# BlueFisher/Advanced-Soft-Actor-Critic

Measured on AMD Instinct MI355X. Metric: SAC train steps/sec (PER sample + grad step), batch 256, higher is better.
Workload: dtype f32; 1 GPU; cfg2: TEST vector obs(6) c_action(2) stock MLP, PER capacity 524288, n_step=4 V-trace; per_gpu_batch=256, global_batch=256, rows_resident=262144, replay_capacity=524288, n_step=4, burn_in_step=0, parallelism=single, ranks=1, hipgraph=True

## Files before the change

advanced-soft-actor-critic_amd/algorithm/fused.py:

```python
import numpy as np
import contextlib

import torch

from asac_amd import native

__all__ = ['FlatParamGroup', 'FlatAdam', 'squash_sample', 'squash_sample_ls', 'clipped_q_loss', 'DeviceNoise',
           'RecordedNoise']


class FlatParamGroup:

    def __init__(self, named_params: list[tuple[str, list[torch.nn.Parameter]]], device, with_grad=True):
        self.segments: dict[str, tuple[int, int]] = {}
        self.params: dict[str, list[torch.nn.Parameter]] = {}
        total = 0
        for name, ps in named_params:
            start = total
            for p in ps:
                total += p.numel()
            total = (total + 3) // 4 * 4
            self.segments[name] = (start, total)
            self.params[name] = list(ps)
        self.numel = total
# ... 305 lines not shown
        F.mse_loss = orig


def scaled_mse(pred: torch.Tensor, target: torch.Tensor, divisor: float) -> torch.Tensor:
    from asac_amd import native
    if (pred.is_cuda and pred.dim() == 3 and pred.dtype == torch.float32 and pred.is_contiguous() and target.shape == pred.shape
            and target.dtype == torch.float32 and target.stride(-1) == 1 and not target.requires_grad
            and 0 < pred.numel() <= native.MASKED_MSE_MAX):
        return _ScaledMseFn.apply(pred, target, divisor)
    return torch.nn.functional.mse_loss(pred, target) / divisor


class DeviceNoise:

    def __init__(self, seed: int | None = None):
        self.seed = torch.initial_seed() if seed is None else seed
        self._prefilled = []

    def _covered(self, buf: torch.Tensor) -> bool:
        return any(lo <= buf.data_ptr() < hi for lo, hi in self._prefilled)

    def begin_step(self, step_counter: torch.Tensor, u: torch.Tensor | None, flat: torch.Tensor | None,
                   subsets: torch.Tensor | None = None, ensemble: int = 0, polyak=None, zero=None) -> None:
        if subsets is not None and subsets.shape[1] == ensemble:
            subsets = None
        if polyak is not None or zero is not None:
            native.step_prologue(polyak, zero, self.seed, step_counter, u, flat, subsets, ensemble)
        else:
            native.noise_fill(self.seed, step_counter, u, flat, subsets, ensemble)
        self._prefilled = [(t.data_ptr(), t.data_ptr() + t.numel() * t.element_size())
                           for t in (u, flat, subsets) if t is not None]

    def begin_step_with_sample(self, step_counter, rb, flat, subsets=None, ensemble: int = 0, polyak=None,
                               zero=None, defer_weights: bool = False) -> int:
        if (rb.uniform_source is not self or rb.sharded is not None
                or rb.batch_size > native.PROLOGUE_SAMPLE_MAX_BATCH):
            return 0
        if subsets is not None and subsets.shape[1] == ensemble:
            subsets = None
        if defer_weights and rb.min_ratio_reducer is None and rb.batch_size > 256 and rb._gather_keys is not None:
            native.step_prologue_sample_partial(polyak, zero, self.seed, step_counter, rb._u, flat, subsets, ensemble, rb._tree,
                                                rb.capacity, rb.batch_size, rb._slot_ids, rb._leaf, rb._p, rb._ids, rb._min_p)
            self._prefilled = [(t.data_ptr(), t.data_ptr() + t.numel() * t.element_size())
                               for t in (rb._u, flat, subsets) if t is not None]
            return 3
        native.step_prologue_sample(polyak, zero, self.seed, step_counter, rb._u, flat, subsets, ensemble, rb._tree,
                                    rb.capacity, rb.batch_size, rb._slot_ids, rb._beta, rb.beta_increment_per_sampling,
                                    rb._leaf, rb._p, rb._ids, rb._w if rb.min_ratio_reducer is None else None,
                                    rb._min_p)
        self._prefilled = [(t.data_ptr(), t.data_ptr() + t.numel() * t.element_size())
                           for t in (rb._u, flat, subsets) if t is not None]
        return 1

    def uniform_(self, buf: torch.Tensor) -> None:
        if not self._covered(buf):
            buf.uniform_()

    def prefill(self, flat: torch.Tensor) -> None:
        if not self._covered(flat):
            flat.normal_()
            self._prefilled.append((flat.data_ptr(), flat.data_ptr() + flat.numel() * flat.element_size()))

    def normal_(self, buf: torch.Tensor) -> None:
        if not self._covered(buf):
            buf.normal_()

    def subset_(self, buf: torch.Tensor, ensemble: int) -> None:
        k = buf.numel()
        if k == ensemble or self._covered(buf):
            return
        keys = torch.rand(ensemble, device=buf.device)
        buf.copy_(torch.topk(keys, k).indices.to(torch.int32))

# ... 40 lines not shown
```

advanced-soft-actor-critic_amd/algorithm/replay_buffer.py:

```python
import logging
import math
from pathlib import Path

import numpy as np
import torch

from asac_amd import native

_NP_DTYPES = {torch.float32: np.dtype(np.float32), torch.float64: np.dtype(np.float64), torch.float16: np.dtype(np.float16),
              torch.int64: np.dtype(np.int64), torch.int32: np.dtype(np.int32), torch.int16: np.dtype(np.int16),
              torch.int8: np.dtype(np.int8), torch.uint8: np.dtype(np.uint8), torch.bool: np.dtype(np.bool_)}

__all__ = ['PrioritizedReplayBuffer']


def _f32_bits(x: float) -> int:
    return int(np.float32(x).view(np.uint32))


class _DeviceUniform:

    def fill(self, u: torch.Tensor) -> None:
        u.uniform_()

# ... 35 lines not shown

        C, dev = self.capacity, self.device
        with torch.cuda.device(dev):
            self._tree = torch.zeros(2 * C - 1, dtype=torch.float32, device=dev)
            self._slot_ids = torch.zeros(C, dtype=torch.int64, device=dev)
            self._winner = torch.full((C + 2 * max(4096, batch_size),), -1, dtype=torch.int32, device=dev)
            self._winner_rows = torch.full((C,), -1, dtype=torch.int32, device=dev)
            self._winner_rows_side = None
            self._nan_flag = torch.zeros(1, dtype=torch.int32, device=dev)
            self._beta = torch.tensor([beta], dtype=torch.float64, device=dev)
            self._max_p = torch.zeros(1, dtype=torch.float32, device=dev)
            self._min_p = torch.zeros(528, dtype=torch.float32, device=dev)
            B = batch_size
            self._u = torch.zeros(B, dtype=torch.float64, device=dev)
            self._leaf = torch.zeros(B, dtype=torch.int32, device=dev)
            self._p = torch.zeros(B, dtype=torch.float32, device=dev)
            self._ids = torch.zeros(B, dtype=torch.int64, device=dev)
            self._w = torch.ones(B, dtype=torch.float32, device=dev)
        self._init_beta = beta

        self._columns: dict[str, torch.Tensor] | None = None
        self._batch: dict[str, torch.Tensor] | None = None
        self._gather_keys = None
        self._join_action_width, self.joint_pre_action, self.derived = None, None, None
        self._size = 0
        self._next_id = 0

        self._pad_action: torch.Tensor | None = None
        self.uniform_source = _DeviceUniform()
        self.min_ratio_reducer = None
        self.sharded = None
        self.lookahead, self.next_valid, self.parity, self._alt = False, False, 0, None
        self._gather_sidecar = None
        self._closed = False

    def set_window_padding(self, padding_action: torch.Tensor) -> None:
        self._pad_action = padding_action.to(self.device, torch.float32).contiguous()
        self._gather_keys = None

    @property
    def beta(self) -> float:
        return float(self._beta.item())

    def _to_device(self, v) -> torch.Tensor:
        if isinstance(v, torch.Tensor):
            return v.to(self.device, non_blocking=True)
        return torch.from_numpy(np.ascontiguousarray(v)).to(self.device, non_blocking=True)

    def _store_rows(self, transitions: dict) -> tuple[int, int]:
        if (self.packed_ingress and len(transitions) <= native.MAX_GATHER_KEYS
                and all(isinstance(v, np.ndarray) for v in transitions.values())):
            return self._store_rows_packed(transitions)
        rows = {k: self._to_device(v) for k, v in transitions.items()}
        count = next(iter(rows.values())).shape[0]
        C = self.capacity
        if self._columns is None:
            self._columns = {k: torch.zeros((C, *v.shape[1:]), dtype=v.dtype, device=self.device)
                             for k, v in rows.items()}
            self._batch, self._gather_keys = None, None
        first_id = self._next_id
        skip = max(0, count - C)
        start = (first_id + skip) % C
        n1 = min(count - skip, C - start)
        for k, v in rows.items():
            col = self._columns[k]
            col[start:start + n1].copy_(v[skip:skip + n1], non_blocking=True)
# ... 173 lines not shown
    def _build_batch(self) -> None:
        self._batch, specs = self._window_specs(self.batch_size, joined=True)
        self._gather_keys = native.make_gather_keys(specs)
        self._gather_refs = specs
        if self.lookahead:
            self._build_second_set()

    _SET_ATTRS = ('_u', '_leaf', '_p', '_ids', '_w', '_min_p', '_batch', '_gather_keys', '_gather_refs',
                  'joint_pre_action', 'derived', '_gather_sidecar')

    def enable_lookahead(self) -> None:
        assert self.sharded is None and self.min_ratio_reducer is None, 'one batch in flight: single-shard replay only'
        self.lookahead, self.next_valid, self.parity = True, False, 0
        self._alt = None
        if self._gather_keys is not None:
            self._build_second_set()

    def _build_second_set(self) -> None:
        first = {a: getattr(self, a) for a in self._SET_ATTRS}
        with torch.cuda.device(self.device):
            for a in ('_u', '_leaf', '_p', '_ids', '_w', '_min_p'):
                setattr(self, a, first[a].clone())
            self._batch, specs = self._window_specs(self.batch_size, joined=True)
            self._gather_keys = native.make_gather_keys(specs)
            self._gather_refs = specs
            self._gather_sidecar = self._make_gather_sidecar()
        self._alt = {a: getattr(self, a) for a in self._SET_ATTRS}
        for a, v in first.items():
            setattr(self, a, v)
        with torch.cuda.device(self.device):
            self._gather_sidecar = self._make_gather_sidecar()
        self.next_valid = False

    def _make_gather_sidecar(self):
        return native.sidecar_window_gather(self._gather_keys, self._ids, self.batch_size, self.prev_n, self.post_n,
                                            self.capacity, self._index_ring())

    def next_gather_sidecar(self):
        self.next_valid = True
        return self._alt['_gather_sidecar']

    def gather_next_now(self) -> None:
        self.swap_sets()
        try:
            self.sample_into_static(sampled=True)
        finally:
            self.swap_sets()

    def swap_sets(self) -> None:
        for a in self._SET_ATTRS:
            mine = getattr(self, a)
            setattr(self, a, self._alt[a])
            self._alt[a] = mine
        self.parity ^= 1

    def next_uniforms(self) -> torch.Tensor:
        return self._alt['_u']

    def sample_next_into_static(self, sampled: bool = False) -> None:
        self.swap_sets()
        try:
            self.sample_into_static(sampled=sampled)
        finally:
            self.swap_sets()
        self.next_valid = True

    def _index_ring(self):
        index_ring = self._columns.get('index') if self._pad_action is not None else None
        if self._pad_action is not None and index_ring is None:
            raise KeyError("window padding needs an 'index' column")
        return self._leaf if index_ring is None else index_ring

    def gather_windows(self, ids: torch.Tensor) -> dict:
        ids = ids.reshape(-1).to(self.device, torch.int64).contiguous()
        out, specs = self._window_specs(ids.numel())
        if ids.numel():
            with torch.cuda.device(self.device):
                native.window_gather_pad(native.make_gather_keys(specs), ids, ids.numel(), self.prev_n, self.post_n,
                                         self.capacity, self._index_ring())
        return out

    def sample(self):
        if not self.is_lg_batch_size:
            return None
        if self._gather_keys is None:
            self._build_batch()
        self.sample_into_static()
        return self._ids, self._batch, self._w.unsqueeze(-1)

    def sample_into_static(self, sampled: int = 0) -> None:
        B, C = self.batch_size, self.capacity
        if self.sharded is not None:
            self.sharded.sample_into(self)
            return
        reducer = self.min_ratio_reducer
        if not sampled:
            self.uniform_source.fill(self._u)
            native.sumtree_sample(self._tree, C, B, self._u, self._slot_ids, self._beta,
                                  self.beta_increment_per_sampling, self._leaf, self._p, self._ids,
                                  self._w if reducer is None else None, self._min_p)
        if reducer is not None:
            if not sampled:
                torch.div(self._min_p[0:1], self._tree[0:1], out=self._min_p[1:2])
            reducer(self._min_p[1:2])
            native.per_is_weights(self._p, B, self._tree, self._min_p[1:2], self._beta,
                                  self.beta_increment_per_sampling, self._w)
        if sampled == 3:
            native.window_gather_pad_w(self._gather_keys, self._ids, B, self.prev_n, self.post_n, C, self._index_ring(),
                                       self._p, self._tree, self._beta, self.beta_increment_per_sampling, self._w, self._min_p)
        elif sampled != 2:
            native.window_gather_pad(self._gather_keys, self._ids, B, self.prev_n, self.post_n, C, self._index_ring())

    def _update_ids(self, ids: torch.Tensor, td: torch.Tensor, stale_check=True, mode=0, sidecars=None) -> None:
        k = ids.numel()
        if k == 0:
            return
        piece = (self._winner.numel() - self.capacity) // 2
        for s in range(0, k, piece):
            native.sumtree_update(self._tree, self.capacity, ids[s:s + piece], self._slot_ids if stale_check else None,
                                  td[s:s + piece], self.alpha, self.td_error_min, self.td_error_max, mode,
                                  self._winner, self._nan_flag, sidecars=sidecars if s == 0 else None)

    def update(self, data_ids, td_error, sidecars=None) -> None:
# ... 163 lines not shown
```

advanced-soft-actor-critic_amd/algorithm/sac_base.py:

```python
import contextlib
import logging
import random
from collections import defaultdict, namedtuple
from pathlib import Path

import numpy as np
import torch
from torch import distributions, nn
from torch.nn import functional

from asac_amd import native

from . import fused_gru, fused_linear
from .fused import DeviceNoise, FlatAdam, FlatParamGroup, squash_sample, squash_sample_ls, time_slice
from .fused_mlp import DeferredPartialSums, StockMLP, describe_policy, describe_q, direct_param_grads
from .nn_models import *
from .nn_models.layers.seq_layers import step_mask_cache
from .nn_models.representation import ModelSimpleRep
from .batch_buffer import BatchBuffer
from .captured_step import CapturedStep
from .replay_buffer import PrioritizedReplayBuffer
from .sac_aux import AuxHeadsMixin
from .utils import *
from .utils.enums import CURIOSITY, SEQ_ENCODER, SIAMESE
# ... 182 lines not shown

        hip_config = dict(hip_config or {})
        self._use_graph = bool(hip_config.get('use_graph', True))
        self._graph_warmup = int(hip_config.get('graph_warmup', 3))
        self._direct_graph_launch = bool(hip_config.get('direct_graph_launch', True))
        self._dist = hip_config.get('dist')
        self._use_fused_mlp = bool(hip_config.get('fused_mlp', True))
        self._graph_collectives = bool(hip_config.get('graph_collectives', True))
        self._twin_rep = bool(hip_config.get('twin_rep', True))
        self._fuse_linear_tanh = bool(hip_config.get('fused_linear_tanh', True))
        self._use_sidecars = bool(hip_config.get('sidecars', True))
        self._defer_is_weights = bool(hip_config.get('defer_is_weights', True))
        self._fused_policy_step = bool(hip_config.get('fused_policy_step', True))
        self._fused_forward_chain = bool(hip_config.get('fused_forward_chain', True))
        self._fused_td_chain = bool(hip_config.get('fused_td_chain', True))
        self._fused_td_update = bool(hip_config.get('fused_td_update', True))
        self._fused_q_return = bool(hip_config.get('fused_q_return', True))
        self._fused_q_state_grads = bool(hip_config.get('fused_q_state_grads', True))
        self._gru_backward_at = bool(hip_config.get('gru_backward_at', True))
        self._adjacent_cat = bool(hip_config.get('adjacent_cat', True))
        self._fold_rep_q_adam = bool(hip_config.get('fold_rep_q_adam', True))
        self._rep_grad_one_position = bool(hip_config.get('rep_grad_one_position', True))
        self._deferred_cat = bool(hip_config.get('deferred_cat', True))
        self._rep_from_burn_in = bool(hip_config.get('rep_from_burn_in', True))
        self._fused_curiosity = bool(hip_config.get('fused_curiosity', True))
        self._fused_discrete = bool(hip_config.get('fused_discrete', True))
        self._fused_rpm_loss = bool(hip_config.get('fused_rpm_loss', True))
        self._rpm_single_backward = bool(hip_config.get('rpm_single_backward', True))
        self._fused_gating = bool(hip_config.get('fused_gating', True))
        self._rpm_conv_one_launch = bool(hip_config.get('rpm_conv_one_launch', True))
        self._lookahead = int(hip_config.get('lookahead', 0))
        assert self._lookahead in (0, 1), 'hip_config lookahead: 0 (synchronous sampling) or 1 (one batch in flight)'
        self._la_gather_sidecar = bool(hip_config.get('lookahead_gather_sidecar', True)) and self._use_sidecars
        self._la_gather = None
        self._fuse_prediction_dense = bool(hip_config.get('fuse_prediction_dense', True))
        self._fused_q_loss_with_aux = bool(hip_config.get('fused_q_loss_with_aux', True))
        self._head_sums_members = bool(hip_config.get('head_sums_members', True))
        self._rep_epilogue, self._rep_epilogue_hp = False, None
        self._cat_mode = None
        self._g_state_base = None
        self._dist_sampling = hip_config.get('dist_sampling', 'throughput')
        self._dist_ready = False
        assert self._dist_sampling in ('throughput', 'parity')

        self._set_logger()

        if not use_replay_buffer:
            if self._dist is not None:
                raise ValueError('use_replay_buffer=False (the episode batch queue) is single-GPU: a data-parallel '
                                 "context (hip_config['dist']) is not supported with it")
            if self._lookahead:
                self._logger.info("hip_config['lookahead'] does not apply without a replay buffer: forced to 0")
                self._lookahead = 0

        if self.use_n_step_is and c_action_size == 0 and len(d_action_sizes) != 0 and discrete_dqn_like:
            self.use_n_step_is = False

        if device is None:
            if not torch.cuda.is_available():
                raise native.AsacNativeError('SAC_Base needs an MI355X (cuda/ROCm device); there is no CPU path')
            self.device = torch.device(f'cuda:{random.randint(0, torch.cuda.device_count() - 1)}')
        else:
            self.device = torch.device(device)
        if self.device.type != 'cuda':
            raise native.AsacNativeError(f'SAC_Base needs a cuda/ROCm device, got {self.device}; no CPU fallback')
        if self.device.index is None:
# ... 854 lines not shown
        else:
            self._launch_return(ret)
            g0 = self._fq.backward_qloss(x0, a0, t_q, c_y.reshape(-1), w, self.clip_epsilon, self._loss_q_e,
                                         defer=fold, state_grads=state_grads)
        if fold:
            self._fq.adam_partials(self.optimizer_q_list[0], loss_out=self._loss_q_e)
        return g0

    @torch.no_grad()
    def _train_rep_q_stock(self, n_last_masks, n_padding_masks, nx_obses_list, nx_states, nx_actions, n_rewards,
                           n_dones, n_mu_probs, priority_is, policy_sample):
        E, B = self.ensemble_q_num, nx_states.shape[0]
        x0 = StockMLP._rows(nx_states[:, 0], self.state_size)
        a0 = StockMLP._rows(nx_actions[:, 0], self.c_action_size)
        xs = StockMLP._rows(nx_states, self.state_size)
        job_tq, _ = self._ftq.job(x0, a0, out=self._tq_buf)
        job_pi, ls = self._fpi.job(xs, None)
        T, A = nx_states.shape[1], self.c_action_size
        window = (n_last_masks, n_padding_masks, nx_obses_list, nx_states, nx_actions, n_rewards, n_dones,
                  n_mu_probs if self.use_n_step_is else None)
        fused = None
        if self._fused_forward_chain and self.curiosity is None:
            f32 = dict(dtype=torch.float32, device=self.device)
            a_y, logp_y = torch.empty((B, T, A), **f32), torch.empty((B, T), **f32)
            c_pi = torch.empty((B, T, A), **f32) if self.use_n_step_is else None
            job_q, q_tab = self._ftq.job(xs, a_y.view(-1, A))
            fused = native.pi_q_job(job_pi, job_q, self._eps_y, a_y, logp_y, T,
                                    action=nx_actions if self.use_n_step_is else None,
                                    action_offset=self.d_action_summed_size, prob_out=c_pi,
                                    eps2=self._eps_pi if policy_sample else None, t2=0,
                                    a2_out=self._pi_a, logp2_out=self._pi_logp)
            if not native.policy_sample_q_forward_ok(fused):
                fused = None
        if fused is not None:
            self.noise.normal_(self._eps_y)
            if policy_sample:
                self.noise.normal_(self._eps_pi)
                self._pi_sampled = True
            native.policy_sample_q_forward(fused, [job_tq], sidecars=self._take_la_gather())
            _, c_y, ret = self._get_y(*window, eps_buf=self._eps_y, subset_prefix='y', y_out=self._y_buf,
                                      ls=ls[0].view(B, T, 2 * A), sample=(a_y, logp_y), stored_pi=c_pi,
                                      q_table=q_tab.view(E, B, T), launch=False)
        else:
            c_y, ret = self._stock_q_targets(job_tq, job_pi, ls, window, policy_sample)
        opt = self.optimizer_q_list[0]
        fold = self._dist is None and opt.start == self._fq._start and self._params.span('rep')[0] == self._params.span('rep')[1]
        self._stock_q_backward(x0, a0, ret, c_y, priority_is, fold, fused_return=fused is not None and self._fused_q_return)
        if not fold:
            self._finish_rep_q(None, None)

    def _train_rep_q(self, n_last_masks, n_padding_masks, nx_obses_list, nx_states, nx_actions, n_rewards,
                     n_dones, n_mu_probs, priority_is, aux=None, policy_sample=False, state_base=None):
        if (self._stock_c_only() and aux is None and self.clip_epsilon > 0 and not nx_states.requires_grad
                and self.optimizer_rep is None):
            return self._train_rep_q_stock(n_last_masks, n_padding_masks, nx_obses_list, nx_states, nx_actions,
                                           n_rewards, n_dones, n_mu_probs, priority_is, policy_sample)
        dsum = self.d_action_summed_size
        obs_list = [o[:, 0] for o in nx_obses_list]
        state, action = nx_states[:, 0], nx_actions[:, 0]
        if state_base is not None and not nx_states.requires_grad:
            state = state_base[0][:, state_base[1]]
        d_action, c_action = action[..., :dsum], action[..., dsum:]

        if (self._fused_q_state_grads and self._fq is not None and self._ftq is not None and not self.d_action_sizes
                and self.c_action_size and self.clip_epsilon > 0 and aux is None and state_base is not None
                and state_base[0].dim() == 3 and state.requires_grad):
            base, t = state_base
            with torch.no_grad():
                x0 = StockMLP._rows(base.detach()[:, t], self.state_size)
                a0 = StockMLP._rows(c_action, self.c_action_size)
                states_y = nx_states.detach()
                job_tq, _ = self._ftq.job(x0, a0, out=self._tq_buf)
                job_pi, ls_y = self._fpi.job(StockMLP._rows_in_place(states_y, self.state_size), None)
                c_y, ret = self._stock_q_targets(
                    job_tq, job_pi, ls_y, (n_last_masks, n_padding_masks, nx_obses_list, states_y, nx_actions, n_rewards,
                                           n_dones, n_mu_probs if self.use_n_step_is else None), policy_sample)
                fold = self._dist is None and self._fold_rep_q_adam and self._rep_q_adam_alike()
                g0 = self._stock_q_backward(x0, a0, ret, c_y, priority_is, fold, fused_return=self._fused_q_return,
                                            state_grads=True)
                g_base = self._g_state_base
                if g_base is None or g_base.shape != base.shape:
                    g_base = self._g_state_base = torch.zeros_like(base)
                at_position = self._gru_backward_at and fused_gru.is_fused_top(base)
                from_head = not at_position and self._head_sums_members and fused_linear.is_fused_head_output(base)
                if not (at_position or from_head):
                    torch.sum(g0, dim=0, out=g_base[:, t])
            rep_stepped = False
            with direct_param_grads(), DeferredPartialSums() as sums_later:
                if at_position:
# ... 411 lines not shown
            return
        if isinstance(ep_indexes, torch.Tensor):
            assert ep_indexes.dtype == torch.int32
            last = ep_indexes == -1
            last[:, -1] = True
            obs_dev = [o[0] for o in ep_obses_list]
        else:
            assert ep_indexes.dtype == np.int32
            last = np.zeros_like(ep_indexes, dtype=bool)
            last[:, -1] = True
            last[ep_indexes == -1] = True
            obs_dev = None
        if not self.use_replay_buffer:
            self.batch_buffer.put_episode(ep_indexes, last, ep_obses_list, ep_actions, ep_rewards, ep_dones, ep_probs,
                                          ep_pre_seq_hidden_states)
            return
        rows = {'index': ep_indexes[0], 'last_mask': last[0],
                **{f'obs_{name}': o[0] for name, o in zip(self.obs_names, ep_obses_list)},
                'action': ep_actions[0], 'reward': ep_rewards[0], 'done': ep_dones[0],
                'mu_prob': ep_probs[0], 'pre_seq_hidden_state': ep_pre_seq_hidden_states[0]}
        if self.use_normalization:
            self._update_normalizer(obs_dev if obs_dev is not None
                                    else [torch.from_numpy(o[0]).to(self.device) for o in ep_obses_list])
        self.replay_buffer.add(rows, ignore_size=1)

    def _device_step(self) -> None:
        with step_mask_cache() if self.seq_encoder == SEQ_ENCODER.ATTN else contextlib.nullcontext():
            self._device_step_body()

    def _device_step_body(self) -> None:
        self._counter_advanced = False
        w = self._step_sample()
        self._step_rep_and_q(w)
        self._step_policy(w)
        post = _AfterPolicy()
        if not self.use_replay_buffer:
            self._step_temperature_and_aux(w, post)
            if not self._counter_advanced:
                self._opt_steps.add_(1)
            self.batch_buffer.advance_head()
            return
        self._join_lookahead()
        if w.stock and self.use_n_step_is:
            with torch.no_grad():
                if not self._step_after_policy_one_launch(w, post):
                    self._step_after_policy_chain(w, post)
        self._step_temperature_and_aux(w, post)
        self._step_write_backs(w, post)
        if not self._counter_advanced:
            self._opt_steps.add_(1)

    def _join_lookahead(self) -> None:
        if self._la_gather is not None:
            self._la_gather = None
            self.replay_buffer.gather_next_now()

    def _take_la_gather(self):
        sc, self._la_gather = self._la_gather, None
        return None if sc is None else [sc]

    def _step_sample(self):
        rb, b = getattr(self, 'replay_buffer', None), self.burn_in_step
        polyak = None
        if self.update_target_per_step == 1 and self._polyak_len > 0:
            polyak = (self._target_params.flat[:self._polyak_len], self._params.flat[:self._polyak_len], self.tau)
        zero = None if self._grads_overwrite else self._params.grad
        if not self.use_replay_buffer:
            self.noise.begin_step(self._opt_steps, None, self._eps_all, self._subsets_all, self.ensemble_q_num,
                                  polyak=polyak, zero=zero)
            self.batch_buffer.gather_into_static()
            return self._window_views(self.batch_buffer._batch, None, None, None)
        if self._lookahead:
            sampled = False
            if self._use_sidecars:
                rb.swap_sets()
                try:
                    sampled = self.noise.begin_step_with_sample(self._opt_steps, rb, self._eps_all, self._subsets_all,
                                                                self.ensemble_q_num, polyak=polyak, zero=zero)
                finally:
                    rb.swap_sets()
            if not sampled:
                self.noise.begin_step(self._opt_steps, rb.next_uniforms() if rb.uniform_source is self.noise else None,
                                      self._eps_all, self._subsets_all, self.ensemble_q_num, polyak=polyak, zero=zero)
            if sampled and self._la_gather_sidecar:
                self._la_gather = rb.next_gather_sidecar()
            else:
                rb.sample_next_into_static(sampled=sampled)
        else:
            sampled = self._use_sidecars and self.noise.begin_step_with_sample(
                self._opt_steps, rb, self._eps_all, self._subsets_all, self.ensemble_q_num, polyak=polyak, zero=zero,
                defer_weights=self._defer_is_weights)
            if not sampled:
                self.noise.begin_step(self._opt_steps, rb._u if rb.uniform_source is self.noise else None, self._eps_all,
                                      self._subsets_all, self.ensemble_q_num, polyak=polyak, zero=zero)
            rb.sample_into_static(sampled=sampled)
        derived = rb.derived if rb.derived is not None and rb.sharded is None else None
        return self._window_views(rb._batch, rb._ids, rb._w.unsqueeze(-1) if self.use_priority else None, derived,
                                  rb.joint_pre_action)

    def _window_views(self, batch, ids, priority_is, derived, joint_pre_action=None):
        b = self.burn_in_step
        w = _Window()
        w.ids = ids
        w.priority_is = priority_is
        w.bnx_obses_list = [batch[f'obs_{name}'] for name in self.obs_names]
        w.bnx_actions, w.bnx_pad = batch['action'], batch['padding_mask']
        w.bn_indexes, w.bn_last, w.bn_pad = batch['index'][:, :-1], batch['last_mask'][:, :-1], w.bnx_pad[:, :-1]
        w.bn_actions, w.bn_rewards, w.bn_dones = w.bnx_actions[:, :-1], batch['reward'][:, :-1], batch['done'][:, :-1]
        w.bn_mu_probs = batch['mu_prob'][:, :-1]
        w.bnx_hidden = batch['pre_seq_hidden_state']
        w.nx_obs = [o[:, b:] for o in w.bnx_obses_list]
        w.obs_b = [o[:, b] for o in w.bnx_obses_list]
        w.stock = self._stock_c_only()
        w.rep_trainable = self.optimizer_rep is not None
        self.noise.prefill(self._eps_all)
        if type(self.model_rep) is ModelSimpleRep:
            w.rep_in = (None, None, w.bnx_obses_list, None, w.bnx_hidden)
        else:
            if derived is not None:
                d = derived
                bnx_indexes, bnx_padding_masks, bnx_pre_actions = d['index_x'], d['padding_mask_x'], d['pre_action']
            else:
                bnx_indexes, bnx_padding_masks, bnx_pre_actions = self.get_bnx_data(
                    w.bn_indexes, w.bn_pad, w.bn_actions, pre_action_out=joint_pre_action)
            w.rep_in = (bnx_indexes, bnx_padding_masks, w.bnx_obses_list, bnx_pre_actions, w.bnx_hidden)
        return w

    def _step_rep_and_q(self, w) -> None:
# ... 269 lines not shown
    def _optimizer_hp(self) -> tuple:
        opts = self._all_optimizers
        if opts is None:
            opts = self._all_optimizers = [o for o in vars(self).values() if isinstance(o, FlatAdam)] + \
                [o for o in self.optimizer_q_list if o is not None]
        return tuple((o.lr, o.betas, o.eps) for o in opts)

    def _drop_graphs(self) -> None:
        self._graph, self._la_graphs, self._graph_runs = None, {}, {}

    def _drop_graphs_if_hp_changed(self) -> None:
        hp = self._optimizer_hp()
        if hp != self._graph_hp:
            if self._graph_hp is not None and (self._graph is not None or self._la_graphs or self._graph_runs):
                self._logger.info('optimizer hyper-parameters changed: the captured step is dropped and captured again')
                self._drop_graphs()
            self._graph_hp = hp

    @unified_elapsed_timer('train a step', 10)
    def train(self) -> int:
        step = self.get_global_step()
        rb = getattr(self, 'replay_buffer', None)
        if not self._ready_to_train():
            self._profiler('train a step').ignore()
            return step
        self._drop_graphs_if_hp_changed()
        if rb is None:
            if self.batch_buffer._batch is None:
                self.batch_buffer.build_static()
                self._drop_graphs()
        elif rb._gather_keys is None:
            rb._build_batch()
            self._drop_graphs()

        if self._lookahead:
            if not rb.lookahead:
                rb.enable_lookahead()
            if not rb.next_valid:
                with torch.cuda.device(self.device):
                    rb.sample_next_into_static()
            rb.swap_sets()
            self._graph = self._la_graphs.get(rb.parity)
            rb.next_valid = False

        with self._profiler('train', repeat=10):
            if self.update_target_per_step != 1 and step % self.update_target_per_step == 0:
                self._update_target_variables(tau=self.tau)
            graph_ok = (self._use_graph and not self._graph_failed and isinstance(self.noise, DeviceNoise)
                        and (self._dist is None or self._graph_collectives))
            if graph_ok and self._graph is None and self._eager_steps >= self._graph_warmup:
                self._try_capture()
            if graph_ok and self._graph is not None:
                self._replay_graph()
            else:
                self._device_step()
                self._eager_steps += 1
        if rb is None:
            self.batch_buffer.pop_host()
        if self._lookahead:
            self._la_graphs[rb.parity] = self._graph
            rb.next_valid = True

        if step % self.write_summary_per_step == 0:
            if rb is not None:
                rb.check_health()
            if self.summary_writer is not None:
# ... 89 lines not shown
```

advanced-soft-actor-critic_amd/csrc/asac_gather.h:

```cpp
#pragma once
#include "asac_common.h"

namespace asac {

constexpr int kGatherBlock = 256;
#ifndef ASAC_GATHER_UNROLL
#define ASAC_GATHER_UNROLL 2
#endif
constexpr int kUnrollLarge = ASAC_GATHER_UNROLL;
constexpr int64_t kSmallGatherBlocks = 8192;

struct GatherKeyDev {
    const uint8_t* src;
    uint8_t* dst;
    const uint8_t* pad_row;
    int32_t row_bytes;
    int32_t pad_mode;
    uint32_t pad_word;
    int32_t convert;
    int32_t unit_log2;
    int32_t units_per_row;
    uint32_t first_block;
    int32_t dst_pitch;
    int32_t derive;
};

struct GatherArgs {
    int32_t n_keys;
    const int64_t* ids;
    const int32_t* index_ring;
    int32_t batch, prev_n, L, capacity;
};
template <int NK>
struct GatherLaunch {
    GatherKeyDev key[NK];
    GatherArgs c;
};

__device__ __forceinline__ int64_t load_id(const int64_t* ids, int s) { return ids[s]; }

__device__ __forceinline__ bool row_valid(const GatherArgs& a, int64_t id, int j) {
    if (j == a.prev_n) return true;
    const int idx_j = a.index_ring[ring_slot(id + (j - a.prev_n), a.capacity)];
    const int idx_c = a.index_ring[ring_slot(id, a.capacity)];
    return (idx_j - idx_c) == (j - a.prev_n);
}

template <typename Unit>
__device__ __forceinline__ Unit pad_value(const GatherKeyDev& k, int w);

template <>
__device__ __forceinline__ uint4 pad_value<uint4>(const GatherKeyDev& k, int w) {
    if (k.pad_mode == ASAC_PAD_ROW) return reinterpret_cast<const uint4*>(k.pad_row)[w];
    uint32_t x = k.pad_word;
    if (k.pad_mode == ASAC_PAD_BYTE) x = (x & 0xff) * 0x01010101u;
    return make_uint4(x, x, x, x);
}
template <>
__device__ __forceinline__ uint32_t pad_value<uint32_t>(const GatherKeyDev& k, int w) {
    if (k.pad_mode == ASAC_PAD_ROW) return reinterpret_cast<const uint32_t*>(k.pad_row)[w];
    uint32_t x = k.pad_word;
    if (k.pad_mode == ASAC_PAD_BYTE) x = (x & 0xff) * 0x01010101u;
    return x;
}
template <>
__device__ __forceinline__ uint8_t pad_value<uint8_t>(const GatherKeyDev& k, int w) {
    if (k.pad_mode == ASAC_PAD_ROW) return k.pad_row[w];
    if (k.pad_mode == ASAC_PAD_WORD) return (uint8_t)(k.pad_word >> (8 * (w & 3)));
    return (uint8_t)(k.pad_word & 0xff);
}

__device__ __forceinline__ int derived_row(int derive, int j, int L) {
    if (derive == ASAC_DERIVE_PREVIOUS) return j > 0 ? j - 1 : 0;
    if (derive >= ASAC_DERIVE_HOLD_LAST) return min(j, L - 2);
    return j;
}
template <typename Unit> __device__ __forceinline__ Unit zero_unit() { return Unit(0); }
template <> __device__ __forceinline__ uint4 zero_unit<uint4>() { return make_uint4(0, 0, 0, 0); }
template <typename Unit> __device__ __forceinline__ Unit next_index(Unit v) { return v; }
template <> __device__ __forceinline__ uint32_t next_index<uint32_t>(uint32_t v) { return v + (v != 0xffffffffu ? 1u : 0u); }

template <typename Unit, int kUnroll>
__device__ __forceinline__ void copy_units(const GatherArgs& a, const GatherKeyDev& k, int64_t g0,
                                           int64_t total_units) {
    int64_t g[kUnroll], at[kUnroll];
    Unit val[kUnroll];
    bool live[kUnroll];
#pragma unroll
    for (int r = 0; r < kUnroll; ++r) {
        g[r] = g0 + (int64_t)r * kGatherBlock;
        live[r] = g[r] < total_units;
        if (!live[r]) continue;
        const int64_t row = g[r] / k.units_per_row;
        const int w = (int)(g[r] - row * k.units_per_row);
        at[r] = row * k.dst_pitch + (int64_t)w * (int)sizeof(Unit);
        const int sample = (int)(row / a.L);
        const int j = (int)(row - (int64_t)sample * a.L);
        const int64_t id = load_id(a.ids, sample);
        const int js = derived_row(k.derive, j, a.L);
        const int slot = ring_slot(id + (js - a.prev_n), a.capacity);
        const Unit data = reinterpret_cast<const Unit*>(k.src + (int64_t)slot * k.row_bytes)[w];
        const bool valid = (k.pad_mode == ASAC_PAD_KEEP) || row_valid(a, id, js);
// ... 83 lines not shown
```

advanced-soft-actor-critic_amd/csrc/asac_sidecar.h:

```cpp
#pragma once
#include "asac_common.h"
#include "asac_gather.h"

#include <cmath>

namespace asac {

struct AdamScalars {
    float w1, b2, one_m_b2, eps;
    double lr, b1, b2d;
};

inline AdamScalars adam_scalars(float lr, float beta1, float beta2, float eps) {
    AdamScalars c;
    c.w1 = (float)(1.0 - (double)beta1);
    c.b2 = beta2;
    c.one_m_b2 = (float)(1.0 - (double)beta2);
    c.eps = eps;
    c.lr = (double)lr;
    c.b1 = (double)beta1;
    c.b2d = (double)beta2;
    return c;
}

// ... 115 lines not shown
    if (a.padding_mask && a.padding_mask[(int64_t)s * a.mask_sample_stride + j]) return false;
    if (a.ids[s] < 0) return false;
    const int64_t tid = a.ids[s] + a.first_off + j;
    const int slot = ring_slot(tid, a.capacity);
    *slot_out = slot;
    return a.slot_ids[slot] == tid;
}

__device__ __forceinline__ void scatter_elect_row(const ScatterArgs& a, int flat) {
    if (flat >= a.batch * a.count) return;
    int slot;
    if (scatter_target(a, flat, &slot)) atomicMax(&a.winner[slot], flat);
}

__device__ __forceinline__ void scatter_write_row(const ScatterArgs& a, int flat, int lane, int lanes) {
    if (flat >= a.batch * a.count) return;
    int slot;
    if (!scatter_target(a, flat, &slot)) return;
    if (__hip_atomic_load(&a.winner[slot], __ATOMIC_RELAXED, __HIP_MEMORY_SCOPE_AGENT) != flat) return;
    const int s = flat / a.count;
    const int j = flat - s * a.count;
    const uint8_t* src = a.rows + (int64_t)s * a.rows_sample_stride + (int64_t)j * a.rows_row_stride;
    uint8_t* dst = a.ring + (int64_t)slot * a.row_bytes;
    if (((a.row_bytes | (int)(reinterpret_cast<uintptr_t>(src) & 3) |
          (int)(reinterpret_cast<uintptr_t>(dst) & 3)) & 3) == 0) {
        for (int w = lane; w < a.row_bytes / 4; w += lanes)
            reinterpret_cast<uint32_t*>(dst)[w] = reinterpret_cast<const uint32_t*>(src)[w];
    } else {
        for (int w = lane; w < a.row_bytes; w += lanes) dst[w] = src[w];
    }
    if (lane == 0) __hip_atomic_store(&a.winner[slot], -1, __ATOMIC_RELAXED, __HIP_MEMORY_SCOPE_AGENT);
}

struct SidecarDev {
    int32_t kind, first_block;
    AlphaAdamArgs alpha;
    ScatterArgs scatter;
    const void* gather;
};
template <int NSC>
struct SidecarsT {
    SidecarDev j[NSC];
    int32_t n, blocks;
};
using SidecarsDev = SidecarsT<ASAC_MAX_SIDECARS>;

template <int NSC>
inline SidecarsT<NSC> sidecars_first(const SidecarsDev& full) {
    SidecarsT<NSC> out{};
    for (int k = 0; k < NSC && k < full.n; ++k) out.j[k] = full.j[k];
    out.n = full.n < NSC ? full.n : NSC;
    out.blocks = full.blocks;
    return out;
}

constexpr int kSidecarRowsPerWg = 256;
inline int scatter_write_rows_per_wg(int row_bytes) { return row_bytes <= 32 ? kSidecarRowsPerWg : 4; }

inline int sidecars_prepare(const asac_sidecar_t* jobs, int n, SidecarsDev& out) {
    out.n = 0;
    out.blocks = 0;
    if (n < 0 || n > ASAC_MAX_SIDECARS || (n > 0 && !jobs)) return 1;
    for (int k = 0; k < n; ++k) {
        const asac_sidecar_t& h = jobs[k];
        SidecarDev& d = out.j[k];
        d.kind = h.kind;
        d.first_block = out.blocks;
        if (h.kind == ASAC_SIDECAR_ALPHA_ADAM) {
            if (h.B <= 0 || h.n <= 0 || h.slot < 0 || h.slot >= h.n || !h.logp || !h.steps_done) return 1;
            d.alpha = AlphaAdamArgs{h.logp, h.B, h.target, h.slot, h.param, h.grad, h.exp_avg, h.exp_avg_sq, h.n,
                                    adam_scalars(h.lr, h.beta1, h.beta2, h.eps), h.steps_done, h.advance_counter};
            out.blocks += 1;
        } else if (h.kind == ASAC_SIDECAR_SCATTER_ELECT || h.kind == ASAC_SIDECAR_SCATTER_WRITE) {
            if (h.row_bytes <= 0 || h.capacity <= 0 || h.batch <= 0 || h.count <= 0 || !h.winner || !h.slot_ids) return 1;
            d.scatter = ScatterArgs{static_cast<uint8_t*>(h.ring), h.row_bytes, h.capacity, h.ids, h.batch, h.first_off,
                                    h.count, h.slot_ids, h.padding_mask, h.mask_sample_stride,
                                    static_cast<const uint8_t*>(h.rows), h.rows_sample_stride_bytes,
                                    h.rows_row_stride_bytes, h.winner};
            const int total = h.batch * h.count;
            const int per = h.kind == ASAC_SIDECAR_SCATTER_ELECT ? kSidecarRowsPerWg : scatter_write_rows_per_wg(h.row_bytes);
            out.blocks += (total + per - 1) / per;
        } else if (h.kind == ASAC_SIDECAR_WINDOW_GATHER) {
            if (!h.gather_plan || h.gather_blocks <= 0) return 1;
            d.gather = h.gather_plan;
            out.blocks += h.gather_blocks;
        } else {
            return 1;
        }
    }
    out.n = n;
    return 0;
}

template <int NSC, bool GATHER = false>
__device__ __forceinline__ void sidecar_run(const SidecarsT<NSC>& sc, int block, float* lds256) {
    int k = 0;
#pragma unroll
    for (int q = 1; q < NSC; ++q)
        if (q < sc.n && block >= sc.j[q].first_block) k = q;
    const SidecarDev& job = sc.j[k];
    const int local = block - job.first_block;
    if (job.kind == ASAC_SIDECAR_ALPHA_ADAM) {
        alpha_adam_block(job.alpha, lds256);
    } else if (GATHER && job.kind == ASAC_SIDECAR_WINDOW_GATHER) {
        if (threadIdx.x < kGatherBlock)
            gather_block<ASAC_MAX_GATHER_KEYS, 1>(*static_cast<const GatherLaunch<ASAC_MAX_GATHER_KEYS>*>(job.gather),
                                                  (unsigned)local);
    } else if (threadIdx.x < 256) {
        if (job.kind == ASAC_SIDECAR_SCATTER_ELECT) {
            scatter_elect_row(job.scatter, local * kSidecarRowsPerWg + (int)threadIdx.x);
        } else if (job.scatter.row_bytes <= 32) {
            scatter_write_row(job.scatter, local * kSidecarRowsPerWg + (int)threadIdx.x, 0, 1);
        } else {
            scatter_write_row(job.scatter, local * 4 + (int)(threadIdx.x >> 6), (int)(threadIdx.x & 63), kWave);
        }
    }
}

}
```

advanced-soft-actor-critic_amd/csrc/gather.hip:

```cpp
#include "asac_common.h"
#include "asac_gather.h"
#include "asac_sidecar.h"

namespace asac {

template <int NK, int kUnroll>
__global__ __launch_bounds__(kGatherBlock) void k_window_gather_pad(const GatherLaunch<NK> m) {
    gather_block<NK, kUnroll>(m, blockIdx.x);
}

struct WeightsJob {
    const float* p;
    const float* tree;
    double* beta_state;
    double beta_increment;
    float* w_out;
    float* min_p_out;
    int32_t batch, parts;
};

__device__ __forceinline__ void weights_job(const WeightsJob& j) {
    float bm = j.min_p_out[2];
    for (int k = 1; k < j.parts; ++k) bm = fminf(bm, j.min_p_out[2 + k]);
    const float root = j.tree[0];
    const double b = fmin(1.0, *j.beta_state + j.beta_increment);
    const float min_ratio = bm / root;
    __syncthreads();
    for (int i = threadIdx.x; i < j.batch; i += kGatherBlock) j.w_out[i] = is_weight(j.p[i], root, min_ratio, b);
    if (threadIdx.x == 0) {
        *j.beta_state = b;
        j.min_p_out[0] = bm;
    }
}

template <int NK, int kUnroll>
__global__ __launch_bounds__(kGatherBlock) void k_window_gather_pad_w(const GatherLaunch<NK> m, unsigned gather_blocks,
                                                                      const WeightsJob j) {
    if (blockIdx.x == 0) {
        weights_job(j);
        return;
    }
    gather_block<NK, kUnroll>(m, blockIdx.x - 1);
}

__global__ __launch_bounds__(256) void k_scatter_elect(const ScatterArgs a) {
    scatter_elect_row(a, blockIdx.x * blockDim.x + threadIdx.x);
}

__global__ __launch_bounds__(256) void k_scatter_write(const ScatterArgs a) {
    scatter_write_row(a, blockIdx.x * (blockDim.x / kWave) + threadIdx.x / kWave, threadIdx.x & (kWave - 1), kWave);
}

__global__ __launch_bounds__(256) void k_window_aux(const int32_t* __restrict__ index, int64_t index_sb,
                                                    const uint8_t* __restrict__ pad, int64_t pad_sb,
                                                    const float* __restrict__ action, int64_t action_sb,
                                                    int64_t action_st, int B, int L, int A,
                                                    int32_t* __restrict__ index_x, uint8_t* __restrict__ pad_x,
                                                    float* __restrict__ pre_action, int64_t pre_action_st) {
    const int i = blockIdx.x * blockDim.x + threadIdx.x;
    if (i >= B * L) return;
    const int b = i / L, t = i - b * L;
    const int ts = t < L - 1 ? t : L - 2;
    const int32_t iv = index[(int64_t)b * index_sb + ts];
    index_x[i] = t < L - 1 ? iv : iv + (iv != -1 ? 1 : 0);
    pad_x[i] = pad[(int64_t)b * pad_sb + ts];
// ... 101 lines not shown
    return finish_launch("asac_window_aux");
}

int asac_window_gather_pad(const asac_gather_key_t* keys_host, int n_keys, const int64_t* ids,
                           int batch, int prev_n, int post_n, int capacity,
                           const int32_t* index_ring, void* stream) {
    GatherLaunch<ASAC_MAX_GATHER_KEYS> m{};
    uint64_t blocks = 0;
    int unroll = 0;
    if (const int rc = gather_fill(keys_host, n_keys, ids, batch, prev_n, post_n, capacity, index_ring, 0, m, &blocks, &unroll))
        return rc;
    if (n_keys <= 8) {
        GatherLaunch<8> m8{};
        for (int q = 0; q < n_keys; ++q) m8.key[q] = m.key[q];
        m8.c = m.c;
        if (unroll == 1)
            ASAC_LAUNCH((k_window_gather_pad<8, 1>), dim3((unsigned)blocks), dim3(kGatherBlock), 0, as_stream(stream), m8);
        else
            ASAC_LAUNCH((k_window_gather_pad<8, kUnrollLarge>), dim3((unsigned)blocks), dim3(kGatherBlock), 0, as_stream(stream), m8);
    } else if (unroll == 1) {
        ASAC_LAUNCH((k_window_gather_pad<ASAC_MAX_GATHER_KEYS, 1>), dim3((unsigned)blocks), dim3(kGatherBlock), 0,
                    as_stream(stream), m);
    } else {
        ASAC_LAUNCH((k_window_gather_pad<ASAC_MAX_GATHER_KEYS, kUnrollLarge>), dim3((unsigned)blocks), dim3(kGatherBlock), 0,
                    as_stream(stream), m);
    }
    return finish_launch("asac_window_gather_pad");
}

int asac_window_gather_pad_w(const asac_gather_key_t* keys_host, int n_keys, const int64_t* ids, int batch, int prev_n,
                             int post_n, int capacity, const int32_t* index_ring, const float* p, const float* tree,
                             double* beta_state, double beta_increment, float* is_weights_out, float* min_p_out,
                             void* stream) {
    if (!p || !tree || !beta_state || !is_weights_out || !min_p_out || batch <= 256 || batch > 1024)
        return bad_arg("asac_window_gather_pad_w");
    GatherLaunch<ASAC_MAX_GATHER_KEYS> m{};
    uint64_t blocks = 0;
    int unroll = 0;
    if (const int rc = gather_fill(keys_host, n_keys, ids, batch, prev_n, post_n, capacity, index_ring, 0, m, &blocks, &unroll))
        return rc;
    const dim3 grid((unsigned)blocks + 1u);
    for (int rep = 0; rep < g_launch_repeat; ++rep) {
        const WeightsJob j{p, tree, beta_state, rep == 0 ? beta_increment : 0.0, is_weights_out, min_p_out, batch,
                           (batch + 255) / 256};
        if (n_keys <= 8) {
            GatherLaunch<8> m8{};
            for (int q = 0; q < n_keys; ++q) m8.key[q] = m.key[q];
            m8.c = m.c;
            if (unroll == 1)
                hipLaunchKernelGGL((k_window_gather_pad_w<8, 1>), grid, dim3(kGatherBlock), 0, as_stream(stream), m8,
                                   (unsigned)blocks, j);
            else
                hipLaunchKernelGGL((k_window_gather_pad_w<8, kUnrollLarge>), grid, dim3(kGatherBlock), 0, as_stream(stream),
                                   m8, (unsigned)blocks, j);
        } else if (unroll == 1) {
            hipLaunchKernelGGL((k_window_gather_pad_w<ASAC_MAX_GATHER_KEYS, 1>), grid, dim3(kGatherBlock), 0,
                               as_stream(stream), m, (unsigned)blocks, j);
        } else {
            hipLaunchKernelGGL((k_window_gather_pad_w<ASAC_MAX_GATHER_KEYS, kUnrollLarge>), grid, dim3(kGatherBlock), 0,
                               as_stream(stream), m, (unsigned)blocks, j);
        }
    }
    return finish_launch("asac_window_gather_pad_w");
}

int64_t asac_window_gather_plan_bytes(void) { return (int64_t)sizeof(GatherLaunch<ASAC_MAX_GATHER_KEYS>); }

int asac_window_gather_plan(const asac_gather_key_t* keys_host, int n_keys, const int64_t* ids, int batch, int prev_n,
                            int post_n, int capacity, const int32_t* index_ring, void* plan_dev, int* blocks_out) {
    if (!plan_dev || !blocks_out) return bad_arg("asac_window_gather_plan");
    GatherLaunch<ASAC_MAX_GATHER_KEYS> m{};
    uint64_t blocks = 0;
    int unroll = 0;
    if (const int rc = gather_fill(keys_host, n_keys, ids, batch, prev_n, post_n, capacity, index_ring, 1, m, &blocks, &unroll))
        return rc;
    const hipError_t e = hipMemcpy(plan_dev, &m, sizeof(m), hipMemcpyHostToDevice);
    if (e != hipSuccess) {
        set_error(e, "asac_window_gather_plan");
        return (int)e;
    }
    *blocks_out = (int)blocks;
    return 0;
}

int asac_gather_rows(const asac_gather_key_t* keys_host, int n_keys, const int64_t* ids, int n_rows, int capacity,
                     void* stream) {
    if (n_keys <= 0 || n_keys > ASAC_MAX_GATHER_KEYS || !keys_host) return bad_arg("asac_gather_rows");
    for (int q = 0; q < n_keys; ++q)
        if (keys_host[q].pad_mode != ASAC_PAD_KEEP || keys_host[q].convert != ASAC_CVT_NONE)
            return bad_arg("asac_gather_rows: key");
    return asac_window_gather_pad(keys_host, n_keys, ids, n_rows, 0, 0, capacity, nullptr, stream);
}

int asac_scatter_rows_if_id_match(void* ring, int row_bytes, int capacity, const int64_t* ids,
                                  int batch, int first_off, int count, const int64_t* slot_ids,
                                  const uint8_t* padding_mask, int mask_sample_stride,
                                  const void* rows, int64_t rows_sample_stride_bytes,
                                  int64_t rows_row_stride_bytes, int32_t* winner, void* stream) {
    if (row_bytes <= 0 || capacity <= 0 || batch <= 0 || count <= 0 || !winner || !slot_ids)
        return bad_arg("asac_scatter_rows_if_id_match");
    ScatterArgs a{static_cast<uint8_t*>(ring), row_bytes, capacity, ids, batch, first_off, count,
                  slot_ids, padding_mask, mask_sample_stride, static_cast<const uint8_t*>(rows),
                  rows_sample_stride_bytes, rows_row_stride_bytes, winner};
    const int total = batch * count;
    hipStream_t s = as_stream(stream);
    ASAC_LAUNCH(k_scatter_elect, dim3((total + 255) / 256), dim3(256), 0, s, a);
    ASAC_LAUNCH(k_scatter_write, dim3((total + 3) / 4), dim3(256), 0, s, a);
    return finish_launch("asac_scatter_rows_if_id_match");
}

}
```

advanced-soft-actor-critic_amd/csrc/mlp.hip:

```cpp
#include "asac_common.h"
#include "asac_gelu.h"
#include "asac_sidecar.h"
#include "asac_squash.h"
#include "asac_vtrace.h"

#include <cmath>

namespace asac {

constexpr int kP = 66;
constexpr int kMaxW = 64;
constexpr int kMaxB = ASAC_MLP_MAX_BLOCKS;
constexpr int kHeadPad = 16;
#ifndef ASAC_PS_WAVES
#define ASAC_PS_WAVES 16
#endif
#ifndef ASAC_PIQ_WAVES
#define ASAC_PIQ_WAVES 8
#endif
constexpr int kPiQThreads = 64 * ASAC_PIQ_WAVES;
template <int TM> constexpr int threads_of() { return TM * 16; }

inline int mlp_tile_rows(int64_t N, int E) { return ((N + 15) / 16) * (int64_t)(E > 0 ? E : 1) <= 256 ? 16 : 32; }

// ... 364 lines not shown
}

using rsrc_t = __amdgpu_buffer_rsrc_t;
constexpr unsigned kOob = 0x80000000u;
__device__ __forceinline__ rsrc_t make_rsrc(const void* p, unsigned bytes = 0x7fffffffu) {
    return __builtin_amdgcn_make_buffer_rsrc(const_cast<void*>(p), 0, (int)bytes, 0x00020000);
}
__device__ __forceinline__ int buf_ld(rsrc_t r, unsigned byte_off) {
    return __builtin_amdgcn_raw_buffer_load_b32(r, (int)byte_off, 0, 0);
}

template <int THREADS, bool WINDOW, int SLOTS = 4>
__device__ __forceinline__ void fetch_input_tile_fixed(const StageScalars& q, int e, int64_t row0, float (&v)[SLOTS]) {
    const int in0 = q.in0, in1 = q.in1;
    const rsrc_t r0 = make_rsrc(q.x0 + e * q.x0_ms);
    const rsrc_t r1 = make_rsrc(q.x1 + e * q.x1_ms, in1 > 0 ? 0x7fffffffu : 0u);
#pragma unroll
    for (int u = 0; u < SLOTS; ++u) {
        const int i = threadIdx.x + u * THREADS;
        const int r = i >> 6, c = i & 63;
        const uint32_t row = (uint32_t)row0 + (uint32_t)r;
        const bool live = (int64_t)row0 + r < q.N;
        uint32_t off = row * (uint32_t)q.x0_rs;
        if (WINDOW) {
            const uint32_t smp = row / (uint32_t)q.x0_T;
            off = smp * (uint32_t)q.x0_sb + (row - smp * (uint32_t)q.x0_T) * (uint32_t)q.x0_rs;
        }
        const unsigned o0 = (live && c < in0) ? (off + (uint32_t)c) * 4u : kOob;
        const unsigned o1 = (live && c >= in0 && c < in0 + in1) ? (row * (uint32_t)q.x1_rs + (uint32_t)(c - in0)) * 4u : kOob;
        v[u] = __builtin_bit_cast(float, buf_ld(r0, o0) | buf_ld(r1, o1));
    }
}

template <int THREADS, int NB>
__device__ __forceinline__ void net_fetch_fixed(const StageScalars& q, StagedNet<THREADS>& r) {
    constexpr int U = 4096 / THREADS;
    const rsrc_t rp = make_rsrc(q.P);
    const int K0 = q.in0 + q.in1;
#pragma unroll
    for (int u = 0; u < U; ++u) {
        const int i = threadIdx.x + u * THREADS;
        const int rr = i >> 6, c = i & 63;
        r.w[0][u] = __builtin_bit_cast(float, buf_ld(rp, c < K0 ? (unsigned)(q.w_off[0] + rr * K0 + c) * 4u : kOob));
    }
#pragma unroll
    for (int l = 1; l < NB; ++l) {
#pragma unroll
        for (int u = 0; u < U / 4; ++u) {
            const auto t = __builtin_amdgcn_raw_buffer_load_b128(rp, (q.w_off[l] + 4 * (int)(threadIdx.x + u * THREADS)) * 4, 0, 0);
#pragma unroll
            for (int k = 0; k < 4; ++k) r.w[l][4 * u + k] = __builtin_bit_cast(float, (int)t[k]);
        }
    }
#pragma unroll
    for (int l = 0; l < NB; ++l) r.bias[l] = __builtin_bit_cast(float, buf_ld(rp, (unsigned)(q.b_off[l] + (threadIdx.x & 63)) * 4u));
    const int h0 = q.h0, h1 = q.h1;
#pragma unroll
    for (int u = 0; u < 1024 / THREADS; ++u) {
        const int i = threadIdx.x + u * THREADS;
        const int o = i >> 6, c = i & 63;
        const bool first = o < h0, second = !first && o < h0 + h1;
        const int idx = second ? q.hw1 + (o - h0) * kMaxW + c : q.hw0 + o * kMaxW + c;
        r.head[u] = __builtin_bit_cast(float, buf_ld(rp, (first || second) ? (unsigned)idx * 4u : kOob));
    }
    {
        const int o = threadIdx.x & 15;
// ... 18 lines not shown
            const int q = threadIdx.x + u * THREADS;
            float2* o2 = reinterpret_cast<float2*>(L.w[l] + (q >> 4) * kP + ((q & 15) << 2));
            o2[0] = make_float2(r.w[l][4 * u], r.w[l][4 * u + 1]);
            o2[1] = make_float2(r.w[l][4 * u + 2], r.w[l][4 * u + 3]);
        }
    }
    if (threadIdx.x < kMaxW) {
#pragma unroll
        for (int l = 0; l < NB; ++l) L.bias[l][threadIdx.x] = r.bias[l];
    }
#pragma unroll
    for (int u = 0; u < 1024 / THREADS; ++u) {
        const int i = threadIdx.x + u * THREADS;
        L.head[(i >> 6) * kP + (i & 63)] = r.head[u];
    }
    if (threadIdx.x < kHeadPad) L.head_bias[threadIdx.x] = r.head_bias;
}

template <int TM>
struct MlpLds {
    float head[kHeadPad * kP];
    float bias[kMaxB][kMaxW];
    float head_bias[kHeadPad];
    float xs[2][TM * kP];
    float w[kMaxB][kMaxW * kP];
};

inline size_t mlp_fwd_lds_bytes(int n_blocks, bool wide = false, int TM = 32) {
    const size_t head = TM == 16 ? offsetof(MlpLds<16>, w) : offsetof(MlpLds<32>, w);
    return head + (size_t)(n_blocks + (wide ? 1 : 0)) * kMaxW * kP * sizeof(float) +
           (wide ? (size_t)TM * kP * sizeof(float) : 0);
}

template <int TM, bool WINDOW, bool WIDE = false, int NB = 0, bool EPI = false>
__device__ __forceinline__ void mlp_fwd_tiles(const MlpFwdArgs& a, const int e, const int tile0, const int tile_stride,
                                              MlpLds<TM>& L, const SampleEpi* epi = nullptr) {
    constexpr int THREADS = threads_of<TM>();
    constexpr int RT = TM / 16;
    constexpr bool fixed = NB > 0;
    static_assert(!(fixed && WIDE), "the fixed-shape path has a first layer of <= 64 inputs");
    const float* P = a.params + e * a.member_stride;
    const int wave = threadIdx.x >> 6, lane = threadIdx.x & 63;
    const int rt = wave % RT, ct = wave / RT;
    const int nb = fixed ? NB : a.d.n_blocks;
    const int K0 = a.d.in0 + a.d.in1;
    const int n_tiles = (int)((a.N + TM - 1) / TM);

    constexpr bool wide = WIDE;
    float* w_hi = &L.w[0][0] + nb * kMaxW * kP;
    float* x_hi = w_hi + kMaxW * kP;
    StageScalars q;
    if constexpr (fixed) {
        q = stage_scalars<NB>(a, e);
        float in_lo[4];
        fetch_input_tile_fixed<THREADS, WINDOW>(q, e, (int64_t)tile0 * TM, in_lo);
        StagedNet<THREADS> regs;
        net_fetch_fixed<THREADS, NB>(q, regs);
        put_input_tile<THREADS>(in_lo, L.xs[0]);
        net_put_fixed<THREADS, NB>(regs, L);
    } else {
        float in_lo[4], in_hi[4];
        fetch_input_tile<THREADS, WINDOW>(a, e, (int64_t)tile0 * TM, in_lo);
        if (wide) fetch_input_tile<THREADS, WINDOW>(a, e, (int64_t)tile0 * TM, in_hi, kMaxW);
        StagedNet<THREADS> regs;
        net_fetch<THREADS>(a.d, P, K0, wide, regs);
        put_input_tile<THREADS>(in_lo, L.xs[0]);
        if (wide) {
            put_input_tile<THREADS>(in_hi, x_hi);
            stage_matrix_part<THREADS>(L.w[0], P + a.d.w_off[0], a.d.width[0], K0, 0, kMaxW);
            stage_matrix_part<THREADS>(w_hi, P + a.d.w_off[0], a.d.width[0], K0, kMaxW, K0 - kMaxW);
        }
        net_put<THREADS>(a.d, P, K0, wide, regs, L);
    }
    const int K_last = fixed ? kMaxW : a.d.width[nb - 1];
    __syncthreads();

    const int O = a.d.head_cols[0] + a.d.head_cols[1];
    int cur = 0;
    for (int tile = tile0; tile < n_tiles; tile += tile_stride) {
        const int64_t row0 = (int64_t)tile * TM;
        const bool more = tile + tile_stride < n_tiles;
        float nxt[4], nxt_hi[4];
        if (more) {
            if constexpr (fixed) fetch_input_tile_fixed<THREADS, WINDOW>(q, e, (int64_t)(tile + tile_stride) * TM, nxt);
            else fetch_input_tile<THREADS, WINDOW>(a, e, (int64_t)(tile + tile_stride) * TM, nxt);
        }
        if (more && wide) fetch_input_tile<THREADS, WINDOW>(a, e, (int64_t)(tile + tile_stride) * TM, nxt_hi, kMaxW);
        SampleEpiIn epi_in{};
        bool epi_on = false;
        if constexpr (EPI) {
            epi_on = epi->on != 0;
            if (epi_on)
                epi_in = sample_epilogue_fetch(*epi, row0 + (wave % RT) * 16 + 4 * (lane >> 4) + wave / RT, a.N, lane & 15);
        }
        int K = K0;
#pragma unroll
        for (int l = 0; l < (fixed ? NB : kMaxB); ++l) {
            if (l >= nb) break;
            const int W = fixed ? kMaxW : a.d.width[l];
            const float* xin = L.xs[cur];
            float* xout = L.xs[cur ^ 1];
            f32x4 acc = (fixed && l > 0) ? gemm_tile(xin, L.w[l], kMaxW, rt, ct)
                                         : gemm_tile(xin, L.w[l], (l == 0 && wide) ? kMaxW : round4(K), rt, ct);
            if (l == 0 && wide) acc += gemm_tile(x_hi, w_hi, round4(K0 - kMaxW), rt, ct);
            const int col = ct * 16 + (lane & 15);
            const float bias = L.bias[l][col];
            const bool res = a.d.residual[l] != 0;
            f32x2_g ya, yb, unused;
            gelu_parts2((f32x2_g){acc[0] + bias, acc[1] + bias}, ya, unused);
            gelu_parts2((f32x2_g){acc[2] + bias, acc[3] + bias}, yb, unused);
            const float yv[4] = {ya.x, ya.y, yb.x, yb.y};
#pragma unroll
            for (int r = 0; r < 4; ++r) {
                const int row = rt * 16 + 4 * (lane >> 4) + r;
                float y = yv[r];
                if (res) y += xin[row * kP + col];
                xout[row * kP + col] = col < W ? y : 0.f;
// ... 948 lines not shown
    q.in0 = j.in0, q.in1 = j.in1, q.x0_T = j.x0_T;
    q.h0 = j.h0, q.h1 = j.h1;
    q.hw0 = j.hw0, q.hw1 = j.hw1, q.hb0 = j.hb0, q.hb1 = j.hb1;
#pragma unroll
    for (int l = 0; l < 3; ++l) q.w_off[l] = j.w_off[l], q.b_off[l] = j.b_off[l];
    ASAC_PIN(q.P); ASAC_PIN(q.x0); ASAC_PIN(q.x1);
    ASAC_PIN(q.N); ASAC_PIN(q.x0_rs); ASAC_PIN(q.x0_ms); ASAC_PIN(q.x1_rs); ASAC_PIN(q.x1_ms); ASAC_PIN(q.x0_sb);
    ASAC_PIN(q.in0); ASAC_PIN(q.in1); ASAC_PIN(q.x0_T); ASAC_PIN(q.h0); ASAC_PIN(q.h1);
    ASAC_PIN(q.hw0); ASAC_PIN(q.hw1); ASAC_PIN(q.hb0); ASAC_PIN(q.hb1);
#pragma unroll
    for (int l = 0; l < 3; ++l) { ASAC_PIN(q.w_off[l]); ASAC_PIN(q.b_off[l]); }
    return q;
}

__device__ __forceinline__ StageScalars stage_scalars_stock_like(const ASAC_KARG StockJobArg& j, int e, const StageScalars& rows) {
    StageScalars q = rows;
    q.P = j.P + e * j.member_stride;
    q.in1 = j.in1;
    q.h0 = j.h0, q.h1 = j.h1;
    q.hw0 = j.hw0, q.hw1 = j.hw1, q.hb0 = j.hb0, q.hb1 = j.hb1;
#pragma unroll
    for (int l = 0; l < 3; ++l) q.w_off[l] = j.w_off[l], q.b_off[l] = j.b_off[l];
    ASAC_PIN(q.P); ASAC_PIN(q.in1); ASAC_PIN(q.h0); ASAC_PIN(q.h1);
    ASAC_PIN(q.hw0); ASAC_PIN(q.hw1); ASAC_PIN(q.hb0); ASAC_PIN(q.hb1);
#pragma unroll
    for (int l = 0; l < 3; ++l) { ASAC_PIN(q.w_off[l]); ASAC_PIN(q.b_off[l]); }
    return q;
}

__device__ __forceinline__ float gauss_head_value(bool location, float raw) {
    return location ? tanhf(raw / 5.f) * 5.f : expf(fminf(fmaxf(raw, -20.f), 0.5f));
}

template <bool WINDOW>
__device__ __forceinline__ void pi_q_tiles(const ASAC_KARG PiQLaunch& a, PiQLds& L) {
    constexpr int THREADS = kPiQThreads;
    constexpr int SLOTS = 1024 / kPiQThreads;
    const bool comp = (threadIdx.x >> 6) < 4;
    const int e = (int)blockIdx.x % a.E, group = (int)blockIdx.x / a.E;
    const int wave = threadIdx.x >> 6, lane = threadIdx.x & 63;
    const int col = wave * 16 + (lane & 15);
    const int A = a.pi.h0, S = a.q.in0;
    const int K0p = a.pi.in0, K0q = a.q.in0 + a.q.in1;
    const int N = a.pi.N;
    const int n_tiles = (int)((N + 15) / 16);
    const bool writer = e == 0;
    MLP_STAMP(0);

    const StageScalars sp = stage_scalars_stock(a.pi, 0);
    const StageScalars sq = stage_scalars_stock_like(a.q, e, sp);
    float in_lo[SLOTS];
    fetch_input_tile_fixed<THREADS, WINDOW, SLOTS>(sp, 0, (int64_t)group * 16, in_lo);
    StagedNet<THREADS> rp, rq;
    net_fetch_fixed<THREADS, 3>(sp, rp);
    net_fetch_fixed<THREADS, 3>(sq, rq);
    put_input_tile<THREADS, SLOTS>(in_lo, L.xs[0]);
    net_put_fixed<THREADS, 3>(rp, L);
    PiQCritic C{L.qw, L.qhead, L.qbias, L.qhead_bias};
    __syncthreads();
    MLP_STAMP(1);

    for (int tile = group; tile < n_tiles; tile += a.tile_groups) {
        const int row0 = tile * 16;
        if (tile != group) {
            fetch_input_tile_fixed<THREADS, WINDOW, SLOTS>(sp, 0, row0, in_lo);
            __syncthreads();
            put_input_tile<THREADS, SLOTS>(in_lo, L.xs[0]);
            __syncthreads();
        }
        int cur = 0;
#pragma unroll
        for (int l = 0; l < 3; ++l) {
            if (comp) {
                const float* xin = L.xs[cur];
                float* xout = L.xs[cur ^ 1];
                const f32x4 acc = l > 0 ? gemm_tile(xin, L.w[l], kMaxW, 0, wave) : gemm_tile(xin, L.w[l], round4(K0p), 0, wave);
                const float bias = L.bias[l][col];
                const bool res = (a.pi.residual_bits >> l) & 1;
                f32x2_g ya, yb, unused;
                gelu_parts2((f32x2_g){acc[0] + bias, acc[1] + bias}, ya, unused);
                gelu_parts2((f32x2_g){acc[2] + bias, acc[3] + bias}, yb, unused);
                const float yv[4] = {ya.x, ya.y, yb.x, yb.y};
#pragma unroll
                for (int r = 0; r < 4; ++r) {
                    const int row = 4 * (lane >> 4) + r;
                    float y = yv[r];
                    if (res) y += xin[row * kP + col];
                    xout[row * kP + col] = y;
                }
            }
            __syncthreads();
            cur ^= 1;
        }
        MLP_STAMP(2);
        if (comp) {
            const f32x4 acc = gemm_tile(L.xs[cur], L.head, kMaxW, 0, 0);
            const int hc = lane & 15;
            const float mine = wave == 0 ? acc[0] : wave == 1 ? acc[1] : wave == 2 ? acc[2] : acc[3];
            const int lrow = 4 * (lane >> 4) + wave;
            const float v = gauss_head_value(hc < A, mine + L.head_bias[hc]);
            L.ls[lrow * 2 * kHeadPad + hc] = v;
            if (writer && a.pi.out && row0 + lrow < N && hc < 2 * A) a.pi.out[(row0 + lrow) * (2 * A) + hc] = v;
        }
        __syncthreads();
        MLP_STAMP(3);
        {
            float* scr = L.xs[1];
            const int job = wave;
            const bool job_on = job == 0 || (writer && ((job == 1 && a.sp.action) || (job == 2 && a.eps2)));
            float* s0 = scr + job * 256;
            float* s1 = s0 + 128;
            if (job < 3 && job_on) {
                for (int it = lane; it < 16 * A; it += 64) {
                    const int lrow = it / A, d = it - lrow * A;
                    const int r = row0 + lrow;
                    if (r >= N) continue;
                    const float l = L.ls[lrow * 2 * kHeadPad + d], sc = L.ls[lrow * 2 * kHeadPad + A + d];
                    if (job == 1) {
                        const int spT = a.sp.T;
                        const int sb = (int)((unsigned)r / (unsigned)spT), st = r - sb * spT;
                        const float av = a.sp.action[sb * a.sp.a_sb + st * a.sp.a_st + a.sp.a_off + d];
                        const float x = atanhf(fminf(fmaxf(av, -0.999f), 0.999f));
                        s0[lrow * 8 + d] = squash_jac(x);
                        s1[lrow * 8 + d] = expf(normal_log_prob(x, l, sc));
                    } else {
                        float ev;
                        const int smp = (int)((unsigned)r / (unsigned)a.T);
                        if (job == 0) {
                            ev = a.eps[r * A + d];
                        } else {
                            if (r - smp * a.T != a.t2) continue;
                            ev = a.eps2[smp * A + d];
                        }
                        const float x = l + ev * sc;
                        const float t = tanhf(x);
                        s0[lrow * 8 + d] = logf(fmaxf(1.f - t * t, kSquashFloor));
                        s1[lrow * 8 + d] = normal_log_prob(x, l, sc);
                        if (job == 0) {
                            L.act[lrow * kHeadPad + d] = t;
                            if (writer) a.a_out[r * A + d] = t;
                        } else {
                            a.a2_out[smp * A + d] = t;
                        }
                    }
                }
                __builtin_amdgcn_fence(__ATOMIC_RELEASE, "wavefront");
                __builtin_amdgcn_wave_barrier();
                __builtin_amdgcn_fence(__ATOMIC_ACQUIRE, "wavefront");
                if (lane < 16) {
                    const int lrow = lane;
                    const int r = row0 + lrow;
                    if (r < N) {
                        if (job == 1) {
                            float jac = 1.f;
// ... 77 lines not shown

template <int NSC>
__global__ __launch_bounds__(kPiQThreads) void k_pi_sample_q(const PiQLaunch m_by_value, const SidecarsT<NSC> sc) {
    extern __shared__ __attribute__((aligned(16))) unsigned char smem_raw[];
    const ASAC_KARG PiQLaunch& m = *static_cast<const ASAC_KARG PiQLaunch*>(kernarg_base());
    const int blk = (int)blockIdx.x;
    const int fused_blocks = m.blocks;
    if (blk >= fused_blocks && threadIdx.x >= 256) return;
    if (blk < fused_blocks) {
        PiQLds& L = *reinterpret_cast<PiQLds*>(smem_raw);
        if (m.pi.x0_T > 0) pi_q_tiles<true>(m, L);
        else pi_q_tiles<false>(m, L);
        return;
    }
    const int xb = blk - fused_blocks;
    if (xb >= m.x_blocks) {
        sidecar_run<NSC, true>(sc, xb - m.x_blocks, reinterpret_cast<float*>(smem_raw));
        return;
    }
    int k = 0;
#pragma unroll
    for (int q = 1; q < ASAC_MLP_MAX_JOBS; ++q)
        if (q < m.x_n && xb >= m.x_first_block[q]) k = q;
    const int local = xb - m.x_first_block[k];
    const int E = m.x_E[k];
    MlpLds<16>& L = *reinterpret_cast<MlpLds<16>*>(smem_raw);
    const MlpFwdArgs job = expand_stock(m.x_job[k]);
    if (job.x0_T > 0)
        mlp_fwd_tiles<16, true, false, 3>(job, local % E, local / E, m.x_tile_stride[k], L);
    else
        mlp_fwd_tiles<16, false, false, 3>(job, local % E, local / E, m.x_tile_stride[k], L);
}

__global__ __launch_bounds__(256) void k_mlp_reduce_partials(const float* __restrict__ partial, int tiles, int E,
                                                             int64_t member_stride, int64_t used,
                                                             float* __restrict__ grad, int accumulate,
                                                             const float* __restrict__ loss_partial,
                                                             float* __restrict__ loss_out, float inv_n) {
    const int64_t i = (int64_t)blockIdx.x * blockDim.x + threadIdx.x;
    const int e = blockIdx.y;
    if (loss_partial && i == 0) {
        float l = 0.f;
        for (int t = 0; t < tiles; ++t) l += loss_partial[(int64_t)t * E + e];
        loss_out[e] = l * inv_n;
    }
    if (i >= used) return;
    float s = 0.f;
    for (int t0 = 0; t0 < tiles; t0 += 8) {
        float v[8];
#pragma unroll
        for (int w = 0; w < 8; ++w) {
            const int t = t0 + w < tiles ? t0 + w : tiles - 1;
            v[w] = partial[((int64_t)t * E + e) * member_stride + i];
        }
#pragma unroll
        for (int w = 0; w < 8; ++w) s += t0 + w < tiles ? v[w] : 0.f;
    }
    grad[e * member_stride + i] = accumulate ? grad[e * member_stride + i] + s : s;
}

constexpr int kReduceSlices = 16;
constexpr int kSlicedFrom = 64;
__global__ __launch_bounds__(64 * kReduceSlices) void k_mlp_reduce_partials_sliced(
    const float* __restrict__ partial, int tiles, int E, int64_t member_stride, int64_t used, float* __restrict__ grad,
    int accumulate, const float* __restrict__ loss_partial, float* __restrict__ loss_out, float inv_n) {
    __shared__ float part[kReduceSlices][64];
// ... 443 lines not shown
    ASAC_LAUNCH(k_policy_step, dim3((unsigned)tiles), dim3(kPsThreads), sizeof(PsLds), s, a);
    if (reduce_mode != ASAC_MLP_REDUCE_DEFER)
        reduce_partials(pi_desc, workspace, tiles, 1, pi_member_stride, pi_grad_params, reduce_mode, nullptr, nullptr, 0.f, s);
    return finish_launch("asac_policy_step_fused");
}

static bool fits32(int64_t v) { return v >= 0 && v < 0x1fffffffLL; }

static StockJobArg stock_job_arg(const asac_mlp_job_t& p) {
    const asac_mlp_desc_t* d = p.desc;
    StockJobArg j{};
    j.P = p.params, j.x0 = p.x0, j.x1 = p.x1, j.out = p.out;
    j.member_stride = (int32_t)p.member_stride, j.N = (int32_t)p.N;
    j.x0_rs = (int32_t)p.x0_row_stride, j.x0_ms = (int32_t)p.x0_member_stride;
    j.x1_rs = (int32_t)p.x1_row_stride, j.x1_ms = (int32_t)p.x1_member_stride;
    j.x0_sb = (int32_t)p.x0_sample_stride, j.x0_T = (int32_t)p.x0_window_T;
    j.in0 = d->in0, j.in1 = d->in1, j.h0 = d->head_cols[0], j.h1 = d->head_cols[1];
    j.hw0 = (int32_t)d->head_w_off[0], j.hw1 = (int32_t)d->head_w_off[1];
    j.hb0 = (int32_t)d->head_b_off[0], j.hb1 = (int32_t)d->head_b_off[1];
    for (int l = 0; l < 3; ++l) {
        j.w_off[l] = (int32_t)d->w_off[l], j.b_off[l] = (int32_t)d->b_off[l];
        j.residual_bits |= (d->residual[l] ? 1 : 0) << l;
    }
    j.head_transform = d->head_transform;
    return j;
}

static asac_mlp_job_t pi_rows(const asac_mlp_job_t& p) {
    asac_mlp_job_t r = p;
    r.x1 = nullptr, r.x1_row_stride = r.x1_member_stride = 0;
    return r;
}

static bool pi_q_job_ok(const asac_pi_q_job_t& j) {
    const asac_mlp_job_t &p = j.pi, &q = j.q;
    if (!p.desc || !q.desc || !desc_ok(*p.desc) || !desc_ok(*q.desc) || p.N <= 0 || q.N != p.N || p.E != 1 || q.E < 1) return false;
    if (!stock3(*p.desc, p.params, p.member_stride) || !stock3(*q.desc, q.params, q.member_stride)) return false;
    if (!scalar_head(*q.desc) || !gauss_head(*p.desc) || p.desc->in1 != 0) return false;
    const int A = p.desc->head_cols[0];
    if (q.desc->in0 != p.desc->in0 || q.desc->in1 != A || 2 * A > kHeadPad || A > 8) return false;
    if (!p.x0 || q.x0 != p.x0 || q.x0_row_stride != p.x0_row_stride || q.x0_window_T != p.x0_window_T ||
        q.x0_sample_stride != p.x0_sample_stride || p.x0_member_stride != 0 || q.x0_member_stride != 0 || !q.out)
        return false;
    const asac_squash_job_t& s = j.sample;
    if (!s.eps || !s.a_tanh_out || !s.logp_out || s.A != A || s.rows != p.N) return false;
    if (s.action && (!s.prob_out || s.T <= 0)) return false;
    if (j.eps2 && (!j.a2_out || !j.logp2_out || s.T <= 0 || j.t2 < 0 || j.t2 >= s.T)) return false;
    if (!fits32(p.member_stride) || !fits32(q.member_stride * q.E)) return false;
    if (s.action && (!fits32((p.N / s.T + 1) * s.action_stride_b) || !fits32((p.N / s.T + 1) * s.prob_stride_b) ||
                     !fits32(s.T * s.action_stride_t) || !fits32(s.T * s.prob_stride_t)))
        return false;
    return job_fits32(pi_rows(p));
}

int asac_policy_sample_q_forward_ok(const asac_pi_q_job_t* job) { return job && pi_q_job_ok(*job) ? 1 : 0; }

int asac_policy_sample_q_forward(const asac_pi_q_job_t* job, const asac_mlp_job_t* extra_jobs, int n_extra,
                                 const asac_sidecar_t* sidecars_host, int n_sidecars, void* stream) {
    if (!job || !pi_q_job_ok(*job) || n_extra < 0 || n_extra > ASAC_MLP_MAX_JOBS || (n_extra > 0 && !extra_jobs))
        return bad_arg("asac_policy_sample_q_forward");
    SidecarsDev sc{};
    if (sidecars_prepare(sidecars_host, n_sidecars, sc)) return bad_arg("asac_policy_sample_q_forward: sidecar");
    PiQLaunch m{};
    const asac_mlp_job_t p = pi_rows(job->pi);
    asac_mlp_job_t q = pi_rows(job->q);
    q.x1 = p.x0;
    m.pi = stock_job_arg(p);
    m.q = stock_job_arg(q);
    m.E = q.E;
    const int tiles = (int)((p.N + 15) / 16);
    const int cap = 256 / q.E > 0 ? 256 / q.E : 1;
    m.tile_groups = tiles <= cap ? tiles : cap;
    m.blocks = m.tile_groups * q.E;
    const asac_squash_job_t& sj = job->sample;
    m.eps = sj.eps;
    m.a_out = sj.a_tanh_out;
    m.logp_out = sj.logp_out;
    m.sp = StoredProbArg{sj.action, sj.prob_out, sj.T, (int32_t)sj.action_stride_b, (int32_t)sj.action_stride_t, sj.action_offset,
                         (int32_t)sj.prob_stride_b, (int32_t)sj.prob_stride_t, sj.prob_offset, 0};
    m.eps2 = job->eps2;
    m.T = sj.T > 0 ? sj.T : 1;
    m.t2 = job->t2;
    m.a2_out = job->a2_out;
    m.logp2_out = job->logp2_out;
    m.x_n = n_extra;
    int blocks = 0;
    for (int k = 0; k < n_extra; ++k) {
        const asac_mlp_job_t& j = extra_jobs[k];
        if (!job_ok(j, true) || !stock3(*j.desc, j.params, j.member_stride) || j.x0_window_T < 0 || !job_fits32(j) ||
            !fits32(j.member_stride) || !fits32(j.x0_member_stride) || !fits32(j.x1_member_stride))
            return bad_arg("asac_policy_sample_q_forward: extra job");
        m.x_job[k] = stock_job_arg(j);
        m.x_E[k] = j.E;
        m.x_first_block[k] = blocks;
        m.x_tile_stride[k] = mlp_tile_groups(j.N, j.E, 1, 16);
        blocks += m.x_tile_stride[k] * j.E;
    }
    m.x_blocks = blocks;
    static bool attr_done = false;
    static bool attr_done1 = false;
    if (int rc = set_lds_limit(reinterpret_cast<const void*>(k_pi_sample_q<ASAC_MAX_SIDECARS>), sizeof(PiQLds), attr_done,
                               "asac_policy_sample_q_forward: hipFuncSetAttribute"))
        return rc;
    if (int rc = set_lds_limit(reinterpret_cast<const void*>(k_pi_sample_q<1>), sizeof(PiQLds), attr_done1,
                               "asac_policy_sample_q_forward: hipFuncSetAttribute"))
        return rc;
    const SidecarsDev none{};
    for (int rep = 0; rep < g_launch_repeat; ++rep) {
        const bool last = rep == g_launch_repeat - 1;
        const dim3 grid((unsigned)(m.blocks + blocks + (last ? sc.blocks : 0)));
        if (sc.n <= 1)
            hipLaunchKernelGGL(k_pi_sample_q<1>, grid, dim3(kPiQThreads), sizeof(PiQLds), as_stream(stream), m,
                               sidecars_first<1>(last ? sc : none));
        else
            hipLaunchKernelGGL(k_pi_sample_q<ASAC_MAX_SIDECARS>, grid, dim3(kPiQThreads), sizeof(PiQLds), as_stream(stream), m,
                               last ? sc : none);
    }
    return finish_launch("asac_policy_sample_q_forward");
}

int asac_mlp_backward_qloss_return_ok(const asac_mlp_job_t* job, const asac_vtrace_args_t* ret) {
    if (!job || !job->desc || !desc_ok(*job->desc) || !ret || job->E <= 0 || job->N <= 0 || ret->B != job->N || ret->n <= 0 ||
        !ret->q || !ret->y_out || ret->E_sample <= 0 || ret->E_sample > ASAC_MAX_ENSEMBLE || ret->td_error_out)
        return 0;
    if (wide_input(*job->desc) || !stock3(*job->desc, job->params, job->member_stride)) return 0;
    const int tm = mlp_tile_rows(job->N, job->E);
    const size_t lds = (tm == 16 ? sizeof(MlpBwdLds<16>) : sizeof(MlpBwdLds<32>)) +
                       (size_t)(2 * ((ret->n + 1) | 1) + 2) * tm * sizeof(float);
    const int threads = tm == 16 ? 64 * ASAC_BWD_WAVES : 32 * 16;
    return tm * ret->n <= threads && lds <= 128 * 1024;
}
// ... 41 lines not shown
```

advanced-soft-actor-critic_amd/csrc/sumtree.hip:

```cpp
#include "asac_common.h"
#include "asac_gather.h"
#include "asac_noise.h"
#include "asac_sidecar.h"
#include "asac_tree_update.h"

#include <cmath>
#include <cstdio>
#include <cstring>
#include <mutex>

namespace asac {

int g_launch_repeat = 1;
static char g_err[256] = "";
static std::mutex g_err_mu;

void set_error(hipError_t e, const char* where) {
    std::lock_guard<std::mutex> lk(g_err_mu);
    snprintf(g_err, sizeof(g_err), "%s: %s", where, hipGetErrorString(e));
}

constexpr int kSampleBlock = 256;
constexpr int kLdsLevels = 12;
constexpr int kLdsNodes = (1 << kLdsLevels) - 1;
// ... 148 lines not shown
            node_[t] = 4 * node_[t] + 3 + 2 * i1 + step(t, i1 ? a2[t].z : a2[t].x, i1 ? a2[t].w : a2[t].y);
        }
    }
    for (; l < levels; ++l) {
        float ab[kTrips][2];
#pragma unroll
        for (int t = 0; t < kTrips; ++t) {
            const int left = live_[t] ? 2 * node_[t] + 1 : 1;
            ab[t][0] = tree[left], ab[t][1] = tree[left + 1];
        }
#pragma unroll
        for (int t = 0; t < kTrips; ++t) node_[t] = 2 * node_[t] + 1 + step(t, ab[t][0], ab[t][1]);
    }
    int64_t id_reg[kTrips];
#pragma unroll
    for (int trip = 0; trip < kTrips; ++trip) {
        const int i = first + trip * kSampleBlock;
        id_reg[trip] = -1;
        if (!live_[trip]) {
            p_reg[trip] = 0.f;
            continue;
        }
        const float p = levels == 0 ? tree[0] : p_reg[trip];
        leaf_out[i] = node_[trip];
        p_out[i] = p;
        id_reg[trip] = slot_ids[node_[trip] - (capacity - 1)];
        pmin = fminf(pmin, p);
        p_reg[trip] = p;
    }

    float m = wave_min(pmin);
    if ((threadIdx.x & (kWave - 1)) == 0) red[threadIdx.x / kWave] = m;
    __syncthreads();
    SampleSync* const sync = MULTI ? reinterpret_cast<SampleSync*>(min_p_out + 2) : nullptr;
    const unsigned n_wg = MULTI ? (unsigned)((batch + kSampleBlock - 1) / kSampleBlock) : 1u;
    if (PARTIAL) {
        if (threadIdx.x == 0) {
            float bm = red[0];
            for (int w = 1; w < kSampleBlock / kWave; ++w) bm = fminf(bm, red[w]);
            sync->part[blockIdx.x] = bm;
        }
#pragma unroll
        for (int trip = 0; trip < kTrips; ++trip) {
            const int i = first + trip * kSampleBlock;
            if (live_[trip]) ids_out[i] = id_reg[trip];
        }
        return;
    }
    if (MULTI) {
        if (threadIdx.x == 0) {
            float bm = red[0];
            for (int w = 1; w < kSampleBlock / kWave; ++w) bm = fminf(bm, red[w]);
            sync_store(&sync->part[blockIdx.x], bm);
            sync_complete();
            __hip_atomic_fetch_add(&sync->arrived, 1u, __ATOMIC_RELAXED, __HIP_MEMORY_SCOPE_AGENT);
            while (__hip_atomic_load(&sync->arrived, __ATOMIC_RELAXED, __HIP_MEMORY_SCOPE_AGENT) < n_wg)
                __builtin_amdgcn_s_sleep(1);
            bm = sync_load(&sync->part[0]);
            for (unsigned w = 1; w < n_wg; ++w) bm = fminf(bm, sync_load(&sync->part[w]));
            red[0] = bm;
        }
    } else if (threadIdx.x == 0) {
        float bm = red[0];
        for (int w = 1; w < kSampleBlock / kWave; ++w) bm = fminf(bm, red[w]);
        red[0] = bm;
        if (FUSE_WEIGHTS && !w_out) {
            min_p_out[0] = bm;
// ... 27 lines not shown
        const double b = fmin(1.0, beta_old + beta_increment);
#pragma unroll
        for (int trip = 0; trip < kTrips; ++trip) {
            const int i = first + trip * kSampleBlock;
            if (i < batch) w_out[i] = is_weight(p_reg[trip], root, min_ratio, b);
        }
    }
#pragma unroll
    for (int trip = 0; trip < kTrips; ++trip) {
        const int i = first + trip * kSampleBlock;
        if (live_[trip]) ids_out[i] = id_reg[trip];
    }
}

template <bool FUSE_WEIGHTS, bool STAGE_TOP>
__global__ __launch_bounds__(kSampleBlock) void k_sumtree_sample(
    const float* __restrict__ tree, int capacity, int levels, int batch,
    const double* __restrict__ u, const int64_t* __restrict__ slot_ids, double* beta_state,
    double beta_increment, int32_t* __restrict__ leaf_out, float* __restrict__ p_out,
    int64_t* __restrict__ ids_out, float* __restrict__ w_out, float* min_p_out) {
    sumtree_sample_body<FUSE_WEIGHTS, STAGE_TOP>(tree, capacity, levels, batch, const_cast<double*>(u), slot_ids, beta_state,
                                                 beta_increment, leaf_out, p_out, ids_out, w_out, min_p_out);
}

template <bool PARTIAL>
__global__ __launch_bounds__(kSampleBlock) void k_prologue_sample(
    const PrologueArgs pa, const float* __restrict__ tree, int capacity, int levels, int batch,
    const int64_t* __restrict__ slot_ids, double* beta_state, double beta_increment, int32_t* __restrict__ leaf_out,
    float* __restrict__ p_out, int64_t* __restrict__ ids_out, float* __restrict__ w_out, float* min_p_out) {
    const int n_s = (batch + kSampleBlock - 1) / kSampleBlock;
    if ((int)blockIdx.x < n_s) {
        const SampleDraw dr{pa.seed, pa.step, pa.n_normal};
        if (n_s == 1)
            sumtree_sample_body<true, true, true, false, 1, false, 13>(
                tree, capacity, levels, batch, pa.u, slot_ids, beta_state, beta_increment, leaf_out, p_out, ids_out, w_out,
                min_p_out, dr);
        else
            sumtree_sample_body<true, true, true, false, 1, true, 13, PARTIAL>(
                tree, capacity, levels, batch, pa.u, slot_ids, beta_state, beta_increment, leaf_out, p_out, ids_out, w_out,
                min_p_out, dr);
    } else {
        prologue_block(pa, (int)blockIdx.x - n_s, true);
    }
}

__global__ __launch_bounds__(kSampleBlock) void k_sumtree_descend(
    const float* __restrict__ tree, int capacity, int levels, int n, const double* __restrict__ v,
    const int64_t* __restrict__ slot_ids, int32_t* __restrict__ leaf_out, float* __restrict__ p_out,
    int64_t* __restrict__ ids_out, float* scratch_min) {
    sumtree_sample_body<false, false, false, true>(tree, capacity, levels, n, const_cast<double*>(v), slot_ids, nullptr, 0.0,
                                                   leaf_out, p_out, ids_out, nullptr, scratch_min);
}

__global__ __launch_bounds__(kSampleBlock) void k_sumtree_descend_owned(
    const float* __restrict__ tree, int capacity, int levels, int n, const double* __restrict__ v,
    const int32_t* __restrict__ owner, int rank, const int64_t* __restrict__ slot_ids, int32_t* __restrict__ leaf_out,
    float* __restrict__ p_out, int64_t* __restrict__ ids_out, float* scratch_min) {
    sumtree_sample_body<false, false, false, true>(tree, capacity, levels, n, const_cast<double*>(v), slot_ids, nullptr, 0.0,
                                                   leaf_out, p_out, ids_out, nullptr, scratch_min, SampleDraw{}, owner, rank);
}

constexpr int kMaxShards = 64;
__global__ __launch_bounds__(kSampleBlock) void k_sumtree_plan_top(const float* __restrict__ roots, int G, int levels_top,
                                                                   int batch, const double* __restrict__ u,
                                                                   int32_t* __restrict__ owner_out, double* __restrict__ v_out,
                                                                   float* __restrict__ total_out) {
    __shared__ float heap[2 * kMaxShards];
// ... 305 lines not shown
    for (int rep = 0; rep < g_launch_repeat; ++rep) {
        const int blocks_p = rep == 0 ? (int)pb : 0;
        const PrologueArgs a{seed, step_counter, uniform_out, batch, normal_out, n_normal, subsets_out, n_subsets, E_sample,
                             E, blocks_p, target, source, n_polyak, one_m_tau, tau, (int)zb, zero_out, n_zero};
        const dim3 grid((unsigned)((batch + kSampleBlock - 1) / kSampleBlock + blocks_p + zb + (lanes + 255) / 256));
        if (partial)
            hipLaunchKernelGGL(k_prologue_sample<true>, grid, dim3(kSampleBlock), 0, as_stream(stream), a, tree, capacity,
                               ilog2(capacity), batch, slot_ids, beta_state, 0.0, leaf_out, p_out, ids_out, is_weights_out,
                               min_p_out);
        else
            hipLaunchKernelGGL(k_prologue_sample<false>, grid, dim3(kSampleBlock), 0, as_stream(stream), a, tree, capacity,
                               ilog2(capacity), batch, slot_ids, beta_state, rep == 0 ? beta_increment : 0.0, leaf_out, p_out,
                               ids_out, is_weights_out, min_p_out);
    }
    return finish_launch("asac_step_prologue_sample");
}

int asac_step_prologue_sample(float* target, const float* source, int64_t n_polyak, float tau, float* zero_out,
                              int64_t n_zero, uint64_t seed, const int64_t* step_counter, double* uniform_out,
                              float* normal_out, int64_t n_normal, int32_t* subsets_out, int n_subsets, int E_sample,
                              int E, const float* tree, int capacity, int batch, const int64_t* slot_ids,
                              double* beta_state, double beta_increment, int32_t* leaf_out, float* p_out,
                              int64_t* ids_out, float* is_weights_out, float* min_p_out, void* stream) {
    return prologue_sample_launch(target, source, n_polyak, tau, zero_out, n_zero, seed, step_counter, uniform_out, normal_out,
                                  n_normal, subsets_out, n_subsets, E_sample, E, tree, capacity, batch, slot_ids, beta_state,
                                  beta_increment, leaf_out, p_out, ids_out, is_weights_out, min_p_out, false, stream);
}

int asac_step_prologue_sample_partial(float* target, const float* source, int64_t n_polyak, float tau, float* zero_out,
                                      int64_t n_zero, uint64_t seed, const int64_t* step_counter, double* uniform_out,
                                      float* normal_out, int64_t n_normal, int32_t* subsets_out, int n_subsets, int E_sample,
                                      int E, const float* tree, int capacity, int batch, const int64_t* slot_ids,
                                      int32_t* leaf_out, float* p_out, int64_t* ids_out, float* min_p_out, void* stream) {
    if (batch <= kSampleBlock) return bad_arg("asac_step_prologue_sample_partial: one workgroup samples such a batch whole");
    static double unused_beta = 0.0;
    return prologue_sample_launch(target, source, n_polyak, tau, zero_out, n_zero, seed, step_counter, uniform_out, normal_out,
                                  n_normal, subsets_out, n_subsets, E_sample, E, tree, capacity, batch, slot_ids, &unused_beta,
                                  0.0, leaf_out, p_out, ids_out, nullptr, min_p_out, true, stream);
}

int asac_per_is_weights(const float* p, int batch, const float* total, const float* min_ratio,
                        double* beta_state, double beta_increment, float* is_weights_out,
                        void* stream) {
    if (batch <= 0) return bad_arg("asac_per_is_weights");
    hipStream_t s = as_stream(stream);
    const int blocks = (batch + 255) / 256;
    if (batch <= kFusedSampleMax && g_launch_repeat == 1) {
        ASAC_LAUNCH(k_is_weights_advance, dim3(1), dim3(256), 0, s, p, batch, total, min_ratio, beta_state, beta_increment,
                    is_weights_out);
        return finish_launch("asac_per_is_weights");
    }
    ASAC_LAUNCH(k_is_weights, dim3(blocks), dim3(256), 0, s, p, batch, total, min_ratio,
                       beta_state, beta_increment, is_weights_out, 1);
    ASAC_LAUNCH(k_advance_beta, dim3(1), dim3(1), 0, s, beta_state, beta_increment);
    return finish_launch("asac_per_is_weights");
}

int asac_sumtree_update(float* tree, int capacity, int k, const int64_t* ids,
                        const int64_t* slot_ids, const float* td_error, float alpha, float td_min,
                        float td_max, int mode, int32_t* winner, int32_t* nan_flag, void* stream) {
    return asac_sumtree_update_sc(tree, capacity, k, ids, slot_ids, td_error, alpha, td_min, td_max, mode, winner, nan_flag,
                                  nullptr, 0, stream);
}

int asac_sumtree_update_sc(float* tree, int capacity, int k, const int64_t* ids,
                           const int64_t* slot_ids, const float* td_error, float alpha, float td_min,
                           float td_max, int mode, int32_t* winner, int32_t* nan_flag,
// ... 59 lines not shown
```

advanced-soft-actor-critic_amd/native.py:

```python
import ctypes as C
from pathlib import Path

import torch

PKG_DIR = Path(__file__).resolve().parent
import os as _os

LIB_PATH = Path(_os.environ.get('ASAC_HIP_LIB', PKG_DIR / 'lib' / 'libasac_hip.so'))
ABI_VERSION = 88

MAX_GATHER_KEYS = 16
PAD_KEEP, PAD_WORD, PAD_BYTE, PAD_ROW, PAD_EMIT_MASK = 0, 1, 2, 3, 4
CVT_NONE, CVT_U8_TO_F32_UNIT, CVT_BOOL_TO_F32 = 0, 1, 2


class AsacNativeError(RuntimeError):
    pass


class GatherKey(C.Structure):
    _fields_ = [('src', C.c_void_p), ('dst', C.c_void_p), ('pad_row', C.c_void_p),
                ('row_bytes', C.c_int32), ('pad_mode', C.c_int32), ('pad_word', C.c_uint32),
                ('convert', C.c_int32), ('dst_row_pitch', C.c_int32), ('derive', C.c_int32)]


class AdamEpilogue(C.Structure):
    _fields_ = [('param_base', C.c_void_p), ('grad_base', C.c_void_p), ('exp_avg_base', C.c_void_p),
                ('exp_avg_sq_base', C.c_void_p), ('lr', C.c_float), ('beta1', C.c_float), ('beta2', C.c_float),
                ('eps', C.c_float), ('steps_done', C.c_void_p)]


def adam_epilogue(param_flat, grad_flat, exp_avg, exp_avg_sq, lr, beta1, beta2, eps, steps_done) -> AdamEpilogue:
    for t in (param_flat, grad_flat, exp_avg, exp_avg_sq):
        assert t.is_cuda and t.is_contiguous() and t.dtype == torch.float32 and t.numel() == param_flat.numel()
    assert steps_done.dtype == torch.int64 and steps_done.is_cuda
    ep = AdamEpilogue(param_flat.data_ptr(), grad_flat.data_ptr(), exp_avg.data_ptr(), exp_avg_sq.data_ptr(),
                      float(lr), float(beta1), float(beta2), float(eps), steps_done.data_ptr())
    ep._keep = (param_flat, grad_flat, exp_avg, exp_avg_sq, steps_done)
    ep._span = (grad_flat.data_ptr(), grad_flat.data_ptr() + 4 * grad_flat.numel())
    return ep


# ... 56 lines not shown
    _fields_ = [('in0', C.c_int32), ('in1', C.c_int32), ('n_blocks', C.c_int32),
                ('width', C.c_int32 * 4), ('residual', C.c_int32 * 4), ('head_cols', C.c_int32 * 2),
                ('w_off', C.c_int64 * 4), ('b_off', C.c_int64 * 4),
                ('head_w_off', C.c_int64 * 2), ('head_b_off', C.c_int64 * 2),
                ('head_transform', C.c_int32), ('reserved_', C.c_int32)]


class MlpJob(C.Structure):
    _fields_ = [('desc', C.POINTER(MlpDesc)), ('params', C.c_void_p), ('member_stride', C.c_int64),
                ('x0', C.c_void_p), ('x0_row_stride', C.c_int64), ('x0_member_stride', C.c_int64),
                ('x1', C.c_void_p), ('x1_row_stride', C.c_int64), ('x1_member_stride', C.c_int64),
                ('N', C.c_int64), ('out', C.c_void_p), ('E', C.c_int32), ('x0_window_T', C.c_int32),
                ('x0_sample_stride', C.c_int64)]


MLP_MAX_JOBS = 2
SAMPLE_EPILOGUE = _os.environ.get('ASAC_SAMPLE_EPILOGUE', '1') != '0'


class Sidecar(C.Structure):
    _fields_ = [('kind', C.c_int32),
                ('logp', C.c_void_p), ('B', C.c_int32), ('target', C.c_float), ('slot', C.c_int32),
                ('param', C.c_void_p), ('grad', C.c_void_p), ('exp_avg', C.c_void_p), ('exp_avg_sq', C.c_void_p),
                ('n', C.c_int32), ('lr', C.c_float), ('beta1', C.c_float), ('beta2', C.c_float), ('eps', C.c_float),
                ('steps_done', C.c_void_p), ('advance_counter', C.c_int32),
                ('ring', C.c_void_p), ('row_bytes', C.c_int32), ('capacity', C.c_int32), ('ids', C.c_void_p),
                ('batch', C.c_int32), ('first_off', C.c_int32), ('count', C.c_int32), ('slot_ids', C.c_void_p),
                ('padding_mask', C.c_void_p), ('mask_sample_stride', C.c_int32), ('rows', C.c_void_p),
                ('rows_sample_stride_bytes', C.c_int64), ('rows_row_stride_bytes', C.c_int64), ('winner', C.c_void_p),
                ('gather_plan', C.c_void_p), ('gather_blocks', C.c_int32)]


SIDECAR_ALPHA_ADAM, SIDECAR_SCATTER_ELECT, SIDECAR_SCATTER_WRITE, SIDECAR_WINDOW_GATHER, MAX_SIDECARS = 1, 2, 3, 4, 4


class SquashJob(C.Structure):
    _fields_ = [('loc', C.c_void_p), ('scale', C.c_void_p), ('ls_row_stride', C.c_int64), ('eps', C.c_void_p),
                ('rows', C.c_int64), ('A', C.c_int32), ('T', C.c_int32), ('a_tanh_out', C.c_void_p),
                ('logp_out', C.c_void_p), ('x_out', C.c_void_p), ('action', C.c_void_p),
                ('action_stride_b', C.c_int64), ('action_stride_t', C.c_int64), ('prob_out', C.c_void_p),
                ('prob_stride_b', C.c_int64), ('prob_stride_t', C.c_int64), ('action_offset', C.c_int32),
                ('prob_offset', C.c_int32)]


SQUASH_MAX_JOBS = 4


class PiQJob(C.Structure):
    _fields_ = [('pi', MlpJob), ('sample', SquashJob), ('eps2', C.c_void_p), ('t2', C.c_int32), ('reserved_', C.c_int32),
                ('a2_out', C.c_void_p), ('logp2_out', C.c_void_p), ('q', MlpJob)]


class SampleEpilogue(C.Structure):
    _fields_ = [('sample', SquashJob), ('eps2', C.c_void_p), ('t2', C.c_int32), ('reserved_', C.c_int32),
                ('a2_out', C.c_void_p), ('logp2_out', C.c_void_p)]


class PartialSum(C.Structure):
    _fields_ = [('partial', C.c_void_p), ('out', C.c_void_p), ('slab_stride', C.c_int64), ('n', C.c_int64),
                ('slabs', C.c_int32), ('slices', C.c_int32), ('accumulate', C.c_int32), ('pad_', C.c_int32)]


class GruDesc(C.Structure):
    _fields_ = [('input', C.c_int32), ('hidden', C.c_int32), ('hidden_pow2', C.c_int32), ('layers', C.c_int32)]


class Conv2Desc(C.Structure):
    _fields_ = [(n, C.c_int32) for n in ('channels', 'height', 'width', 'out1', 'kernel1', 'stride1',
                                         'out2', 'kernel2', 'stride2')]


GRU_MAX_LAYERS, GRU_MAX_DIM = 2, 16
_PtrArray = C.c_void_p * GRU_MAX_LAYERS

class ObsDecoderParams(C.Structure):
    _fields_ = [(n, C.c_void_p) for n in ('dense1_w', 'dense1_b', 'dense2_w', 'dense2_b', 'ct1_w', 'ct1_b', 'ct2_w',
                                          'ct2_b', 'ct3_w', 'ct3_b')]


_SIGNATURES = {
    'asac_version': (C.c_int, []),
    'asac_last_error': (C.c_char_p, []),
    'asac_set_launch_repeat': (C.c_int, [C.c_int]),
    'asac_sumtree_sample': (C.c_int, [C.c_void_p, C.c_int, C.c_int, C.c_void_p, C.c_void_p, C.c_void_p,
                                      C.c_double, C.c_void_p, C.c_void_p, C.c_void_p, C.c_void_p,
                                      C.c_void_p, C.c_void_p]),
    'asac_per_is_weights': (C.c_int, [C.c_void_p, C.c_int, C.c_void_p, C.c_void_p, C.c_void_p, C.c_double,
                                      C.c_void_p, C.c_void_p]),
    'asac_sumtree_update': (C.c_int, [C.c_void_p, C.c_int, C.c_int, C.c_void_p, C.c_void_p, C.c_void_p,
                                      C.c_float, C.c_float, C.c_float, C.c_int, C.c_void_p, C.c_void_p,
                                      C.c_void_p]),
    'asac_per_add': (C.c_int, [C.c_void_p, C.c_int, C.c_int64, C.c_int, C.c_int, C.c_void_p, C.c_float,
                               C.c_void_p, C.c_void_p]),
    'asac_sumtree_leaf_max': (C.c_int, [C.c_void_p, C.c_int, C.c_void_p, C.c_void_p]),
    'asac_sumtree_check': (C.c_int, [C.c_void_p, C.c_int, C.c_void_p, C.c_void_p]),
    'asac_gelu_eval': (C.c_int, [C.c_void_p, C.c_void_p, C.c_void_p, C.c_int64, C.c_void_p]),
    'asac_sumtree_plan_top': (C.c_int, [C.c_void_p, C.c_int, C.c_int, C.c_void_p, C.c_void_p, C.c_void_p, C.c_void_p, C.c_void_p]),
    'asac_sumtree_descend_owned': (C.c_int, [C.c_void_p, C.c_int, C.c_int, C.c_void_p, C.c_void_p, C.c_int, C.c_void_p,
                                             C.c_void_p, C.c_void_p, C.c_void_p, C.c_void_p]),
    'asac_per_is_weights_slice': (C.c_int, [C.c_void_p, C.c_int, C.c_int, C.c_int, C.c_void_p, C.c_void_p, C.c_double,
                                            C.c_void_p, C.c_void_p]),
    'asac_window_gather_pad': (C.c_int, [C.POINTER(GatherKey), C.c_int, C.c_void_p, C.c_int, C.c_int,
                                         C.c_int, C.c_int, C.c_void_p, C.c_void_p]),
    'asac_window_gather_plan_bytes': (C.c_int64, []),
    'asac_window_gather_plan': (C.c_int, [C.POINTER(GatherKey), C.c_int, C.c_void_p, C.c_int, C.c_int, C.c_int, C.c_int,
                                          C.c_void_p, C.c_void_p, C.POINTER(C.c_int)]),
    'asac_sumtree_descend': (C.c_int, [C.c_void_p, C.c_int, C.c_int, C.c_void_p, C.c_void_p, C.c_void_p, C.c_void_p,
                                       C.c_void_p, C.c_void_p]),
    'asac_gather_rows': (C.c_int, [C.POINTER(GatherKey), C.c_int, C.c_void_p, C.c_int, C.c_int, C.c_void_p]),
    'asac_rows_move': (C.c_int, [C.POINTER(RowMove), C.c_int, C.c_void_p, C.c_void_p, C.c_void_p, C.c_int,
                                 C.c_void_p]),
    'asac_batch_put': (C.c_int, [C.POINTER(BatchPutKey), C.c_int, C.c_int, C.c_int, C.c_int, C.c_void_p, C.c_void_p,
                                 C.c_int, C.c_int, C.c_void_p, C.c_void_p, C.c_int, C.c_int, C.c_void_p, C.c_int,
                                 C.c_void_p, C.c_int32, C.c_void_p]),
    'asac_batch_pop_gather': (C.c_int, [C.POINTER(BatchGatherKey), C.c_int, C.c_void_p, C.c_void_p, C.c_int, C.c_int,
                                        C.c_int, C.c_int, C.c_void_p]),
    'asac_window_aux': (C.c_int, [C.c_void_p, C.c_int64, C.c_void_p, C.c_int64, C.c_void_p, C.c_int64, C.c_int64,
                                  C.c_int, C.c_int, C.c_int, C.c_void_p, C.c_void_p, C.c_void_p, C.c_int64, C.c_void_p]),
    'asac_scatter_rows_if_id_match': (C.c_int, [C.c_void_p, C.c_int, C.c_int, C.c_void_p, C.c_int, C.c_int,
                                                C.c_int, C.c_void_p, C.c_void_p, C.c_int, C.c_void_p,
                                                C.c_int64, C.c_int64, C.c_void_p, C.c_void_p]),
    'asac_squash_sample_fwd': (C.c_int, [C.c_void_p, C.c_void_p, C.c_int64, C.c_void_p, C.c_int64, C.c_int,
                                         C.c_void_p, C.c_void_p, C.c_void_p,
                                         C.c_void_p, C.c_int, C.c_int64, C.c_int64, C.c_int,
                                         C.c_void_p, C.c_int64, C.c_int64, C.c_int, C.c_void_p]),
    'asac_squash_sample_bwd': (C.c_int, [C.c_void_p, C.c_void_p, C.c_int64, C.c_void_p, C.c_void_p, C.c_int,
                                         C.c_int64, C.c_void_p, C.c_void_p, C.c_int64, C.c_int, C.c_void_p,
                                         C.c_void_p, C.c_int64, C.c_void_p]),
    'asac_squash_multi': (C.c_int, [C.POINTER(SquashJob), C.c_int, C.POINTER(Sidecar), C.c_int, C.c_void_p]),
    'asac_squash_prob': (C.c_int, [C.c_void_p, C.c_void_p, C.c_int64, C.c_void_p, C.c_int, C.c_int64, C.c_int64,
                                   C.c_int, C.c_int64, C.c_int, C.c_void_p, C.c_int64, C.c_int64, C.c_int,
                                   C.c_void_p]),
    'asac_vtrace_return_min': (C.c_int, [C.POINTER(VtraceArgs), C.c_void_p]),
    'asac_vtrace_return_min_sc': (C.c_int, [C.POINTER(VtraceArgs), C.POINTER(Sidecar), C.c_int, C.POINTER(Sidecar),
                                            C.c_void_p]),
    'asac_td_update': (C.c_int, [C.POINTER(VtraceArgs), C.c_void_p, C.c_int, C.c_void_p, C.c_void_p, C.c_float, C.c_float,
                                 C.c_float, C.c_void_p, C.c_void_p, C.POINTER(Sidecar), C.c_int, C.POINTER(Sidecar),
                                 C.c_void_p]),
    'asac_sumtree_update_sc': (C.c_int, [C.c_void_p, C.c_int, C.c_int, C.c_void_p, C.c_void_p, C.c_void_p, C.c_float,
                                         C.c_float, C.c_float, C.c_int, C.c_void_p, C.c_void_p, C.POINTER(Sidecar), C.c_int,
                                         C.c_void_p]),
    'asac_vtrace_return_direct': (C.c_int, [C.POINTER(VtraceArgs), C.c_void_p, C.c_void_p, C.c_void_p,
                                            C.c_void_p, C.c_void_p]),
    'asac_q_loss_fwd_bwd': (C.c_int, [C.c_void_p, C.c_void_p, C.c_void_p, C.c_void_p, C.c_int, C.c_int,
                                      C.c_float, C.c_void_p, C.c_void_p, C.c_void_p]),
    'asac_mlp_forward': (C.c_int, [C.POINTER(MlpJob), C.c_void_p]),
    'asac_mlp_forward_multi': (C.c_int, [C.POINTER(MlpJob), C.c_int, C.POINTER(Sidecar), C.c_int, C.c_void_p]),
    'asac_mlp_forward_multi_sampled_ok': (C.c_int, [C.POINTER(MlpJob), C.c_int, C.POINTER(SampleEpilogue)]),
    'asac_mlp_forward_multi_sampled': (C.c_int, [C.POINTER(MlpJob), C.c_int, C.POINTER(SampleEpilogue), C.POINTER(Sidecar),
                                                 C.c_int, C.c_void_p]),
    'asac_mlp_backward_workspace': (C.c_int64, [C.c_int64, C.c_int, C.c_int64]),
    'asac_mlp_backward_tiles': (C.c_int64, [C.c_int64, C.c_int]),
    'asac_mlp_backward': (C.c_int, [C.POINTER(MlpJob), C.c_void_p, C.c_void_p, C.c_void_p, C.c_void_p, C.c_void_p, C.c_int,
                                    C.c_void_p]),
    'asac_mlp_backward_qloss': (C.c_int, [C.POINTER(MlpJob), C.c_void_p, C.c_void_p, C.c_void_p, C.c_float, C.c_void_p,
                                          C.c_void_p, C.c_void_p, C.c_void_p, C.c_int, C.c_void_p]),
    'asac_mlp_backward_qloss_return_ok': (C.c_int, [C.POINTER(MlpJob), C.POINTER(VtraceArgs)]),
    'asac_mlp_backward_qloss_return': (C.c_int, [C.POINTER(MlpJob), C.c_void_p, C.POINTER(VtraceArgs), C.c_void_p, C.c_float,
                                                 C.c_void_p, C.c_void_p, C.c_void_p, C.c_void_p, C.c_int, C.c_void_p]),
    'asac_mlp_backward_policy_q': (C.c_int, [C.POINTER(MlpJob), C.c_void_p, C.c_void_p, C.c_int, C.c_void_p, C.c_void_p]),
    'asac_mlp_backward_policy_sample': (C.c_int, [C.POINTER(MlpJob), C.c_void_p, C.c_void_p, C.c_int, C.c_void_p,
                                                  C.c_void_p, C.c_void_p, C.c_int, C.c_void_p]),
    'asac_struct_size': (C.c_int64, [C.c_char_p]),
    'asac_policy_sample_q_forward_ok': (C.c_int, [C.POINTER(PiQJob)]),
    'asac_policy_sample_q_forward': (C.c_int, [C.POINTER(PiQJob), C.POINTER(MlpJob), C.c_int, C.POINTER(Sidecar), C.c_int,
                                               C.c_void_p]),
    'asac_policy_step_fused_ok': (C.c_int, [C.POINTER(MlpDesc), C.c_void_p, C.c_int64, C.POINTER(MlpDesc), C.c_void_p,
                                            C.c_int64, C.c_int64]),
    'asac_policy_step_fused': (C.c_int, [C.POINTER(MlpDesc), C.c_void_p, C.c_int64, C.POINTER(MlpDesc), C.c_void_p,
                                         C.c_int64, C.c_void_p, C.c_int64, C.c_int64, C.c_void_p, C.c_void_p,
                                         C.c_void_p, C.c_void_p, C.c_void_p, C.c_void_p, C.c_void_p, C.c_void_p,
                                         C.c_void_p, C.c_void_p, C.c_int, C.c_void_p]),
    'asac_mlp_param_extent': (C.c_int64, [C.POINTER(MlpDesc)]),
    'asac_adam_step_partials': (C.c_int, [C.c_void_p, C.c_void_p, C.c_void_p, C.c_void_p, C.c_float, C.c_float,
                                          C.c_float, C.c_float, C.c_void_p, C.c_void_p, C.c_int64, C.c_int,
                                          C.c_int64, C.c_int64, C.c_int, C.c_void_p, C.c_int64, C.c_void_p]),
    'asac_gauss_head_fwd': (C.c_int, [C.c_void_p, C.c_int64, C.c_int, C.c_void_p, C.c_void_p, C.c_void_p]),
    'asac_gauss_head_bwd': (C.c_int, [C.c_void_p, C.c_void_p, C.c_void_p, C.c_int64, C.c_int, C.c_void_p,
                                      C.c_void_p]),
    'asac_attention_supported': (C.c_int, [C.c_int, C.c_int, C.c_int]),
    'asac_attention_forward': (C.c_int, [C.c_void_p, C.c_void_p, C.c_void_p, C.c_void_p, C.c_int64, C.c_int64, C.c_int64,
                                         C.c_int, C.c_int, C.c_int, C.c_int, C.c_void_p, C.c_void_p, C.c_void_p,
                                         C.c_void_p]),
    'asac_attention_backward': (C.c_int, [C.c_void_p, C.c_void_p, C.c_void_p, C.c_void_p, C.c_void_p, C.c_void_p, C.c_int,
                                          C.c_int, C.c_int, C.c_int, C.c_void_p, C.c_void_p, C.c_void_p, C.c_void_p]),
    'asac_attention_proj_workspace': (C.c_int64, [C.c_int, C.c_int, C.c_int, C.c_int]),
    'asac_attention_proj_forward': (C.c_int, [C.c_void_p, C.c_int64, C.c_int64, C.c_void_p, C.c_int64, C.c_int64,
                                              C.c_void_p * 8, C.c_void_p, C.c_int64, C.c_int64, C.c_int64, C.c_int,
                                              C.c_int, C.c_int, C.c_int, C.c_void_p, C.c_void_p, C.c_void_p, C.c_void_p,
                                              C.c_void_p, C.c_int64, C.c_int64, C.c_void_p]),
    'asac_attention_proj_backward': (C.c_int, [C.c_void_p, C.c_int64, C.c_int64, C.c_void_p, C.c_int64, C.c_int64,
                                               C.c_void_p * 8, C.c_void_p, C.c_void_p, C.c_void_p, C.c_void_p, C.c_int64,
                                               C.c_int64, C.c_void_p, C.c_void_p, C.c_int64, C.c_int64,
                                               C.c_int, C.c_int, C.c_int, C.c_int, C.c_void_p, C.c_void_p, C.c_void_p,
                                               C.c_int, C.c_void_p, C.c_void_p]),
    'asac_linear_tanh_workspace': (C.c_int64, [C.c_int64, C.c_int, C.c_int]),
    'asac_linear_tanh_forward': (C.c_int, [C.c_void_p, C.c_int64, C.c_void_p, C.c_void_p, C.c_int64, C.c_int, C.c_int,
# ... 360 lines not shown
def sumtree_descend_owned(tree, capacity, values, owner, rank, slot_ids, leaf_out, p_out, ids_out):
    assert values.dtype == torch.float64 and owner.dtype == torch.int32 and ids_out.dtype == torch.int64
    _check(load().asac_sumtree_descend_owned(_p(tree), capacity, values.numel(), _p(values), _p(owner), int(rank),
                                             _p(slot_ids), _p(leaf_out), _p(p_out), _p(ids_out), _stream()),
           'asac_sumtree_descend_owned')


def per_is_weights_slice(p_all, first, count, total, beta_state, beta_increment, w_out):
    _check(load().asac_per_is_weights_slice(_p(p_all), p_all.numel(), first, count, _p(total), _p(beta_state),
                                            float(beta_increment), _p(w_out), _stream()), 'asac_per_is_weights_slice')


def gelu_eval(z, value, deriv):
    _check(load().asac_gelu_eval(_p(z), _p(value), _p(deriv), z.numel(), _stream()), 'asac_gelu_eval')


@_profiled
def window_gather_pad(keys, ids, batch, prev_n, post_n, capacity, index_ring):
    _check(load().asac_window_gather_pad(keys, len(keys), _p(ids), batch, prev_n, post_n, capacity,
                                         _p(index_ring), _stream()), 'asac_window_gather_pad')


def sidecar_window_gather(keys, ids, batch, prev_n, post_n, capacity, index_ring) -> Sidecar:
    import torch
    plan = torch.empty(int(load().asac_window_gather_plan_bytes()), dtype=torch.uint8, device=ids.device)
    blocks = C.c_int(0)
    _check(load().asac_window_gather_plan(keys, len(keys), _p(ids), batch, prev_n, post_n, capacity, _p(index_ring), _p(plan),
                                          C.byref(blocks)), 'asac_window_gather_plan')
    sc = Sidecar(kind=SIDECAR_WINDOW_GATHER, gather_plan=_p(plan), gather_blocks=blocks.value)
    sc._keep = (plan, keys, ids, index_ring)
    return sc


@_profiled
def gather_rows(keys, ids, capacity):
    _check(load().asac_gather_rows(keys, len(keys), _p(ids), ids.numel(), capacity, _stream()), 'asac_gather_rows')


def make_row_moves(specs):
    assert 0 < len(specs) <= MAX_GATHER_KEYS
    arr = (RowMove * len(specs))()
    for k, s in zip(arr, specs):
        k.src, k.dst = s['src'].data_ptr(), s['dst'].data_ptr()
        k.row_bytes = int(s['row_bytes'])
        k.src_mode, k.dst_mode = int(s['src_mode']), int(s['dst_mode'])
        k.src_stride0, k.src_stride1 = int(s.get('src_stride0', 0)), int(s.get('src_stride1', 0))
        k.dst_stride0, k.dst_stride1 = int(s.get('dst_stride0', 0)), int(s.get('dst_stride1', 0))
        k.src_row_offset = int(s.get('src_row_offset', 0))
        k.pad_word = int(s.get('pad_word', 0)) & 0xffffffff
    return arr


@_profiled
def rows_move(keys, slot, src_row, dst_row, n_items):
    _check(load().asac_rows_move(keys, len(keys), _p(slot), _p(src_row), _p(dst_row), int(n_items), _stream()),
           'asac_rows_move')


def make_batch_put_keys(specs):
    assert 0 < len(specs) <= MAX_GATHER_KEYS
    arr = (BatchPutKey * len(specs))()
    for k, s in zip(arr, specs):
        k.src = s['src'].data_ptr() if s.get('src') is not None else None
        k.pool = s['pool'].data_ptr()
        k.pad_row = s['pad_row'].data_ptr() if s.get('pad_row') is not None else None
        k.src_stride = int(s.get('src_stride', 0))
# ... 308 lines not shown
    assert len(jobs) == len(epilogues) and 1 <= len(jobs) <= MLP_MAX_JOBS
    return bool(load().asac_mlp_forward_multi_sampled_ok((MlpJob * len(jobs))(*jobs), len(jobs),
                                                         (SampleEpilogue * len(jobs))(*epilogues)))


@_profiled
def mlp_forward_multi_sampled(jobs, epilogues, sidecars=None):
    global _last_work
    _last_work = sum(mlp_flops(j.desc.contents, j.E, j.N) for j in jobs)
    assert len(jobs) == len(epilogues) and 1 <= len(jobs) <= MLP_MAX_JOBS
    arr = (MlpJob * len(jobs))(*jobs)
    epi = (SampleEpilogue * len(jobs))(*epilogues)
    sc, n_sc = _sidecar_array(sidecars)
    _check(load().asac_mlp_forward_multi_sampled(arr, len(jobs), epi, sc, n_sc, _stream()), 'asac_mlp_forward_multi_sampled')


def pi_q_job(pi_job: MlpJob, q_job: MlpJob, eps, a_out, logp_out, T, action=None, action_offset=0, prob_out=None,
             prob_offset=0, eps2=None, t2=0, a2_out=None, logp2_out=None) -> PiQJob:
    j = PiQJob()
    j.pi, j.q = pi_job, q_job
    A = pi_job.desc.contents.head_cols[0]
    N = pi_job.N
    assert eps.is_contiguous() and a_out.is_contiguous() and eps.numel() == N * A and logp_out.numel() == N
    s = j.sample
    s.eps, s.a_tanh_out, s.logp_out, s.rows, s.A, s.T = eps.data_ptr(), a_out.data_ptr(), logp_out.data_ptr(), N, A, T
    if action is not None:
        assert action.dim() == 3 and action.shape[1] == T
        _stored_action(s, N, action, action_offset, prob_out, prob_offset)
    if eps2 is not None:
        _second_sample(j, N // T, A, eps2, t2, a2_out, logp2_out)
    return j


def policy_sample_q_forward_ok(job: PiQJob) -> bool:
    return bool(load().asac_policy_sample_q_forward_ok(C.byref(job)))


@_profiled
def policy_sample_q_forward(job: PiQJob, extra_jobs=(), sidecars=None):
    global _last_work
    _last_work = (mlp_flops(job.pi.desc.contents, 1, job.pi.N) + mlp_flops(job.q.desc.contents, job.q.E, job.q.N)
                  + sum(mlp_flops(j.desc.contents, j.E, j.N) for j in extra_jobs))
    extra_jobs = list(extra_jobs)
    assert len(extra_jobs) <= MLP_MAX_JOBS
    arr = (MlpJob * len(extra_jobs))(*extra_jobs) if extra_jobs else None
    sc, n_sc = _sidecar_array(sidecars)
    _check(load().asac_policy_sample_q_forward(C.byref(job), arr, len(extra_jobs), sc, n_sc, _stream()),
           'asac_policy_sample_q_forward')


def mlp_backward_workspace(member_stride, E, N) -> int:
    return int(load().asac_mlp_backward_workspace(member_stride, E, N))


def mlp_backward_tiles(N, E) -> int:
    return int(load().asac_mlp_backward_tiles(N, E))


MLP_REDUCE_OVERWRITE, MLP_REDUCE_ACCUMULATE, MLP_REDUCE_DEFER = 0, 1, 2


def mlp_param_extent(desc) -> int:
    return int(load().asac_mlp_param_extent(C.byref(desc)))


@_profiled
def mlp_backward_qloss(job: MlpJob, target_q, y, weights, clip_eps, loss_out, grad_params, workspace, reduce_mode,
                       grad_x0=None):
# ... 643 lines not shown
                                     C.c_uint64(int(seed) & (2 ** 64 - 1)), _p(step_counter), _p(uniform_out), nu,
                                     _p(normal_out), nn_, _p(subsets_out), ns, es, int(ensemble), _stream()),
           'asac_step_prologue')


PROLOGUE_SAMPLE_MAX_BATCH = 1024


@_profiled
def step_prologue_sample(polyak, zero, seed, step_counter, uniform_out, normal_out, subsets_out, ensemble, tree,
                         capacity, batch, slot_ids, beta_state, beta_increment, leaf_out, p_out, ids_out, is_weights_out,
                         min_p_out):
    target_flat, source_flat, tau = polyak if polyak is not None else (None, None, 0.0)
    assert uniform_out.numel() == batch and uniform_out.dtype == torch.float64 and batch <= PROLOGUE_SAMPLE_MAX_BATCH
    assert min_p_out.numel() >= 528 and min_p_out.dtype == torch.float32
    assert zero is None or (zero.is_contiguous() and zero.dtype == torch.float32)
    nn_ = 0 if normal_out is None else normal_out.numel()
    ns = es = 0
    if subsets_out is not None:
        assert subsets_out.dtype == torch.int32 and subsets_out.is_contiguous() and subsets_out.dim() == 2
        ns, es = subsets_out.shape
    _check(load().asac_step_prologue_sample(
        _p(target_flat), _p(source_flat), 0 if polyak is None else target_flat.numel(), float(tau), _p(zero),
        0 if zero is None else zero.numel(), C.c_uint64(int(seed) & (2 ** 64 - 1)), _p(step_counter), _p(uniform_out),
        _p(normal_out), nn_, _p(subsets_out), ns, es, int(ensemble), _p(tree), capacity, batch, _p(slot_ids),
        _p(beta_state), float(beta_increment), _p(leaf_out), _p(p_out), _p(ids_out), _p(is_weights_out), _p(min_p_out),
        _stream()), 'asac_step_prologue_sample')


@_profiled
def step_prologue_sample_partial(polyak, zero, seed, step_counter, uniform_out, normal_out, subsets_out, ensemble, tree,
                                 capacity, batch, slot_ids, leaf_out, p_out, ids_out, min_p_out):
    target_flat, source_flat, tau = polyak if polyak is not None else (None, None, 0.0)
    assert uniform_out.numel() == batch and uniform_out.dtype == torch.float64 and 256 < batch <= PROLOGUE_SAMPLE_MAX_BATCH
    assert min_p_out.numel() >= 528 and min_p_out.dtype == torch.float32
    assert zero is None or (zero.is_contiguous() and zero.dtype == torch.float32)
    nn_ = 0 if normal_out is None else normal_out.numel()
    ns = es = 0
    if subsets_out is not None:
        assert subsets_out.dtype == torch.int32 and subsets_out.is_contiguous() and subsets_out.dim() == 2
        ns, es = subsets_out.shape
    _check(load().asac_step_prologue_sample_partial(
        _p(target_flat), _p(source_flat), 0 if polyak is None else target_flat.numel(), float(tau), _p(zero),
        0 if zero is None else zero.numel(), C.c_uint64(int(seed) & (2 ** 64 - 1)), _p(step_counter), _p(uniform_out),
        _p(normal_out), nn_, _p(subsets_out), ns, es, int(ensemble), _p(tree), capacity, batch, _p(slot_ids),
        _p(leaf_out), _p(p_out), _p(ids_out), _p(min_p_out), _stream()), 'asac_step_prologue_sample_partial')


@_profiled
def window_gather_pad_w(keys, ids, batch, prev_n, post_n, capacity, index_ring, p, tree, beta_state, beta_increment,
                        is_weights_out, min_p_out):
    _check(load().asac_window_gather_pad_w(keys, len(keys), _p(ids), batch, prev_n, post_n, capacity, _p(index_ring), _p(p),
                                           _p(tree), _p(beta_state), float(beta_increment), _p(is_weights_out),
                                           _p(min_p_out), _stream()), 'asac_window_gather_pad_w')


def graph_launch(graph_exec: int):
    _check(load().asac_graph_launch(C.c_void_p(int(graph_exec)), _stream()), 'asac_graph_launch')


def graph_replace_memset_nodes(graph: int):
    rep, kept = C.c_int(0), C.c_int(0)
    _check(load().asac_graph_replace_memset_nodes(C.c_void_p(int(graph)), C.byref(rep), C.byref(kept)),
           'asac_graph_replace_memset_nodes')
    return rep.value, kept.value


# ... 684 lines not shown
```

include/asac_hip.h:

```cpp
#ifndef ASAC_HIP_H
#define ASAC_HIP_H

#include <stdint.h>

#ifdef __cplusplus
extern "C" {
#endif

#define ASAC_ABI_VERSION 88
#define ASAC_MAX_GATHER_KEYS 16
#define ASAC_MAX_ENSEMBLE 16
#define ASAC_MAX_ACTION 64
#define ASAC_MLP_MAX_BLOCKS 4

int asac_version(void);
int64_t asac_struct_size(const char* name);
const char* asac_last_error(void);

int asac_set_launch_repeat(int repeat);


int asac_sumtree_sample(const float* tree, int capacity, int batch, const double* u,
                        const int64_t* slot_ids, double* beta_state, double beta_increment,
                        int32_t* leaf_out, float* p_out, int64_t* ids_out, float* is_weights_out,
                        float* min_p_out, void* stream);

int asac_sumtree_descend(const float* tree, int capacity, int n, const double* values, const int64_t* slot_ids,
                         int32_t* leaf_out, float* p_out, int64_t* ids_out, void* stream);

int asac_sumtree_plan_top(const float* shard_roots, int n_shards, int batch, const double* u, int32_t* owner_out,
                          double* value_out, float* total_out, void* stream);
int asac_sumtree_descend_owned(const float* tree, int capacity, int n, const double* values, const int32_t* owner,
                               int rank, const int64_t* slot_ids, int32_t* leaf_out, float* p_out, int64_t* ids_out,
                               void* stream);
int asac_per_is_weights_slice(const float* p_all, int n_all, int first, int count, const float* total, double* beta_state,
                              double beta_increment, float* is_weights_out, void* stream);

int asac_per_is_weights(const float* p, int batch, const float* total, const float* min_ratio,
                        double* beta_state, double beta_increment, float* is_weights_out,
                        void* stream);

int asac_sumtree_update(float* tree, int capacity, int k, const int64_t* ids,
// ... 12 lines not shown
enum {
    ASAC_PAD_KEEP = 0,
    ASAC_PAD_WORD = 1,
    ASAC_PAD_BYTE = 2,
    ASAC_PAD_ROW = 3,
    ASAC_PAD_EMIT_MASK = 4
};
enum {
    ASAC_CVT_NONE = 0,
    ASAC_CVT_U8_TO_F32_UNIT = 1,
    ASAC_CVT_BOOL_TO_F32 = 2
};
enum { ASAC_DERIVE_NONE = 0, ASAC_DERIVE_PREVIOUS = 1, ASAC_DERIVE_HOLD_LAST = 2, ASAC_DERIVE_HOLD_LAST_NEXT = 3 };
typedef struct {
    const void* src;
    void* dst;
    const void* pad_row;
    int32_t row_bytes;
    int32_t pad_mode;
    uint32_t pad_word;
    int32_t convert;
    int32_t dst_row_pitch;
    int32_t derive;
} asac_gather_key_t;

int asac_window_gather_pad(const asac_gather_key_t* keys_host, int n_keys, const int64_t* ids,
                           int batch, int prev_n, int post_n, int capacity,
                           const int32_t* index_ring, void* stream);

int64_t asac_window_gather_plan_bytes(void);
int asac_window_gather_plan(const asac_gather_key_t* keys_host, int n_keys, const int64_t* ids, int batch, int prev_n,
                            int post_n, int capacity, const int32_t* index_ring, void* plan_dev, int* blocks_out);

int asac_gather_rows(const asac_gather_key_t* keys_host, int n_keys, const int64_t* ids, int n_rows, int capacity,
                     void* stream);

enum { ASAC_ROW_ITEM = 0, ASAC_ROW_SLOT = 1, ASAC_ROW_SLOT_ROW = 2, ASAC_ROW_BROADCAST = 3 };
typedef struct {
    const void* src;
    void* dst;
    int64_t src_stride0, src_stride1;
    int64_t dst_stride0, dst_stride1;
    int32_t row_bytes;
    int32_t src_mode, dst_mode;
    int32_t src_row_offset;
    uint32_t pad_word;
    int32_t reserved_;
} asac_row_move_t;

int asac_rows_move(const asac_row_move_t* keys_host, int n_keys, const int32_t* slot, const int32_t* src_row,
                   const int32_t* dst_row, int n_items, void* stream);

int asac_window_aux(const int32_t* index, int64_t index_stride_b, const uint8_t* padding_mask,
                    int64_t mask_stride_b, const float* action, int64_t action_stride_b, int64_t action_stride_t,
                    int B, int L, int A, int32_t* index_x_out, uint8_t* padding_mask_x_out,
                    float* pre_action_out, int64_t pre_action_stride_t, void* stream);

int asac_scatter_rows_if_id_match(void* ring, int row_bytes, int capacity, const int64_t* ids,
                                  int batch, int first_off, int count, const int64_t* slot_ids,
                                  const uint8_t* padding_mask, int mask_sample_stride,
                                  const void* rows, int64_t rows_sample_stride_bytes,
                                  int64_t rows_row_stride_bytes, int32_t* winner, void* stream);


int asac_squash_sample_fwd(const float* loc, const float* scale, int64_t ls_row_stride, const float* eps,
                           int64_t rows, int A, float* a_tanh_out, float* logp_out, float* x_out,
                           const float* action, int T, int64_t action_stride_b, int64_t action_stride_t,
                           int action_offset, float* prob_out, int64_t prob_stride_b, int64_t prob_stride_t,
                           int prob_offset, void* stream);

int asac_squash_sample_bwd(const float* loc, const float* scale, int64_t ls_row_stride, const float* eps,
                           const float* grad_a, int grad_a_members, int64_t grad_a_member_stride,
                           const float* grad_logp, const float* log_alpha, int64_t rows, int A,
                           float* grad_loc, float* grad_scale, int64_t grad_row_stride, void* stream);

#define ASAC_SIDECAR_ALPHA_ADAM 1
#define ASAC_SIDECAR_SCATTER_ELECT 2
#define ASAC_SIDECAR_SCATTER_WRITE 3
#define ASAC_SIDECAR_WINDOW_GATHER 4
#define ASAC_MAX_SIDECARS 4
typedef struct {
    int32_t kind;
    const float* logp;
    int32_t B;
    float target;
    int32_t slot;
    float *param, *grad, *exp_avg, *exp_avg_sq;
    int32_t n;
    float lr, beta1, beta2, eps;
    int64_t* steps_done;
    int32_t advance_counter;
    void* ring;
    int32_t row_bytes, capacity;
    const int64_t* ids;
    int32_t batch, first_off, count;
    const int64_t* slot_ids;
    const uint8_t* padding_mask;
    int32_t mask_sample_stride;
    const void* rows;
    int64_t rows_sample_stride_bytes, rows_row_stride_bytes;
    int32_t* winner;
    const void* gather_plan;
    int32_t gather_blocks;
} asac_sidecar_t;

#define ASAC_SQUASH_MAX_JOBS 4
typedef struct {
    const float* loc;
    const float* scale;
    int64_t ls_row_stride;
    const float* eps;
    int64_t rows;
// ... 87 lines not shown
    const asac_mlp_desc_t* desc;
    const float* params;
    int64_t member_stride;
    const float* x0;
    int64_t x0_row_stride, x0_member_stride;
    const float* x1;
    int64_t x1_row_stride, x1_member_stride;
    int64_t N;
    float* out;
    int32_t E;
    int32_t x0_window_T;
    int64_t x0_sample_stride;
} asac_mlp_job_t;

int asac_mlp_forward(const asac_mlp_job_t* job, void* stream);

#define ASAC_MLP_MAX_JOBS 2
int asac_mlp_forward_multi(const asac_mlp_job_t* jobs_host, int n_jobs, const asac_sidecar_t* sidecars_host,
                           int n_sidecars, void* stream);

typedef struct {
    asac_squash_job_t sample;
    const float* eps2;
    int32_t t2;
    int32_t reserved_;
    float* a2_out;
    float* logp2_out;
} asac_mlp_sample_epilogue_t;
int asac_mlp_forward_multi_sampled_ok(const asac_mlp_job_t* jobs_host, int n_jobs, const asac_mlp_sample_epilogue_t* epilogues);
int asac_mlp_forward_multi_sampled(const asac_mlp_job_t* jobs_host, int n_jobs, const asac_mlp_sample_epilogue_t* epilogues,
                                   const asac_sidecar_t* sidecars_host, int n_sidecars, void* stream);

typedef struct {
    asac_mlp_job_t pi;
    asac_squash_job_t sample;
    const float* eps2;
    int32_t t2;
    int32_t reserved_;
    float* a2_out;
    float* logp2_out;
    asac_mlp_job_t q;
} asac_pi_q_job_t;
int asac_policy_sample_q_forward_ok(const asac_pi_q_job_t* job);
int asac_policy_sample_q_forward(const asac_pi_q_job_t* job, const asac_mlp_job_t* extra_jobs, int n_extra,
                                 const asac_sidecar_t* sidecars_host, int n_sidecars, void* stream);

#define ASAC_MLP_REDUCE_OVERWRITE 0
#define ASAC_MLP_REDUCE_ACCUMULATE 1
#define ASAC_MLP_REDUCE_DEFER 2
int64_t asac_mlp_backward_workspace(int64_t member_stride, int E, int64_t N);
int64_t asac_mlp_backward_tiles(int64_t N, int E);

int asac_mlp_backward(const asac_mlp_job_t* job, const float* grad_out, float* grad_x0, float* grad_x1, float* grad_params,
                      float* workspace, int reduce_mode, void* stream);

int asac_mlp_backward_qloss(const asac_mlp_job_t* job, const float* target_q, const float* y, const float* weights,
                            float clip_eps, float* loss_out, float* grad_x0, float* grad_params, float* workspace,
                            int reduce_mode, void* stream);

int asac_mlp_backward_qloss_return_ok(const asac_mlp_job_t* job, const asac_vtrace_args_t* ret);
int asac_mlp_backward_qloss_return(const asac_mlp_job_t* job, const float* target_q, const asac_vtrace_args_t* ret,
                                   const float* weights, float clip_eps, float* loss_out, float* grad_x0, float* grad_params,
                                   float* workspace, int reduce_mode, void* stream);

int asac_mlp_backward_policy_q(const asac_mlp_job_t* job, const float* q_table, const int32_t* subset, int E_sample,
                               float* grad_x1, void* stream);

int asac_policy_step_fused_ok(const asac_mlp_desc_t* q_desc, const float* q_params, int64_t q_member_stride,
                              const asac_mlp_desc_t* pi_desc, const float* pi_params, int64_t pi_member_stride, int64_t N);
int asac_policy_step_fused(const asac_mlp_desc_t* q_desc, const float* q_params, int64_t q_member_stride,
                           const asac_mlp_desc_t* pi_desc, const float* pi_params, int64_t pi_member_stride,
                           const float* x, int64_t x_row_stride, int64_t N, const float* action, const float* eps,
                           const float* log_alpha, const int32_t* subset, float* q_out, float* a_tanh_out,
                           float* logp_out, float* ls_out, float* pi_grad_params, float* workspace, int reduce_mode,
                           void* stream);

// ... 441 lines not shown
```

Measured before the change: 11660 train_steps/s.

## Fuse replay window gather into policy-sample Q forward via ring-row reads

After: 11910 train_steps/s (median of 6 runs). 2.2% higher.

```diff
diff --git a/advanced-soft-actor-critic_amd/algorithm/fused.py b/advanced-soft-actor-critic_amd/algorithm/fused.py
--- a/advanced-soft-actor-critic_amd/algorithm/fused.py
+++ b/advanced-soft-actor-critic_amd/algorithm/fused.py
@@ -361,13 +361,14 @@
                            for t in (u, flat, subsets) if t is not None]
 
     def begin_step_with_sample(self, step_counter, rb, flat, subsets=None, ensemble: int = 0, polyak=None,
-                               zero=None, defer_weights: bool = False) -> int:
+                               zero=None, defer_weights: bool = False, defer_small: bool = False) -> int:
         if (rb.uniform_source is not self or rb.sharded is not None
                 or rb.batch_size > native.PROLOGUE_SAMPLE_MAX_BATCH):
             return 0
         if subsets is not None and subsets.shape[1] == ensemble:
             subsets = None
-        if defer_weights and rb.min_ratio_reducer is None and rb.batch_size > 256 and rb._gather_keys is not None:
+        if (defer_weights and rb.min_ratio_reducer is None and (rb.batch_size > 256 or defer_small)
+                and rb._gather_keys is not None):
             native.step_prologue_sample_partial(polyak, zero, self.seed, step_counter, rb._u, flat, subsets, ensemble, rb._tree,
                                                 rb.capacity, rb.batch_size, rb._slot_ids, rb._leaf, rb._p, rb._ids, rb._min_p)
             self._prefilled = [(t.data_ptr(), t.data_ptr() + t.numel() * t.element_size())
diff --git a/advanced-soft-actor-critic_amd/algorithm/replay_buffer.py b/advanced-soft-actor-critic_amd/algorithm/replay_buffer.py
--- a/advanced-soft-actor-critic_amd/algorithm/replay_buffer.py
+++ b/advanced-soft-actor-critic_amd/algorithm/replay_buffer.py
@@ -91,6 +91,7 @@
         self.sharded = None
         self.lookahead, self.next_valid, self.parity, self._alt = False, False, 0, None
         self._gather_sidecar = None
+        self._head_plan = None
         self._closed = False
 
     def set_window_padding(self, padding_action: torch.Tensor) -> None:
@@ -330,6 +331,37 @@
             self._gather_sidecar = self._make_gather_sidecar()
         self.next_valid = False
 
+    def head_gather(self, obs_key: str, build: bool = False, weights: bool = True):
+        if self._gather_keys is None or self.sharded is not None or self.min_ratio_reducer is not None or self.lookahead:
+            return None
+        plan = self._head_plan
+        if plan is not None and plan['for'] is self._gather_keys and plan['weights'] == weights:
+            return plan['plan']
+        if not build:
+            return None
+        made = None
+        dst = {k: self._batch.get(k) for k in (obs_key, 'action')}
+        specs = {k: next((sp for sp in self._gather_refs if sp.get('dst') is t and not sp.get('derive')), None)
+                 for k, t in dst.items() if t is not None}
+        if (len(specs) == 2 and all(sp is not None and not sp.get('dst_row_pitch') for sp in specs.values())
+                and self._pad_action is not None and self.derived is None and self.joint_pre_action is None):
+            x0, action = native.ring_key(specs[obs_key]), native.ring_key(specs['action'])
+            if x0 is not None and action is not None:
+                with torch.cuda.device(self.device):
+                    made = dict(x0=x0, action=action, index_ring=self._index_ring())
+                    if weights:
+                        made['sidecar_w'] = native.sidecar_window_gather_w(
+                            self._gather_keys, self._ids, self.batch_size, self.prev_n, self.post_n, self.capacity,
+                            self._index_ring(), self._p, self._tree, self._beta, self.beta_increment_per_sampling, self._w,
+                            self._min_p)
+                    else:
+                        made['sidecar'] = self._make_gather_sidecar()
+        self._head_plan = {'for': self._gather_keys, 'weights': weights, 'plan': made}
+        return made
+
+    def gather_now(self, weights: bool = False) -> None:
+        self.sample_into_static(sampled=3 if weights else 1)
+
     def _make_gather_sidecar(self):
         return native.sidecar_window_gather(self._gather_keys, self._ids, self.batch_size, self.prev_n, self.post_n,
                                             self.capacity, self._index_ring())
@@ -386,7 +418,10 @@
         self.sample_into_static()
         return self._ids, self._batch, self._w.unsqueeze(-1)
 
-    def sample_into_static(self, sampled: int = 0) -> None:
+    def sample_into_static(self, sampled: int = 0, gather: bool = True) -> None:
+        assert gather or (sampled in (1, 3) and self.sharded is None and self.min_ratio_reducer is None)
+        if not gather:
+            return
         B, C = self.batch_size, self.capacity
         if self.sharded is not None:
             self.sharded.sample_into(self)
diff --git a/advanced-soft-actor-critic_amd/algorithm/sac_base.py b/advanced-soft-actor-critic_amd/algorithm/sac_base.py
--- a/advanced-soft-actor-critic_amd/algorithm/sac_base.py
+++ b/advanced-soft-actor-critic_amd/algorithm/sac_base.py
@@ -238,6 +238,10 @@
         self._lookahead = int(hip_config.get('lookahead', 0))
         assert self._lookahead in (0, 1), 'hip_config lookahead: 0 (synchronous sampling) or 1 (one batch in flight)'
         self._la_gather_sidecar = bool(hip_config.get('lookahead_gather_sidecar', True)) and self._use_sidecars
+        self._head_gather_sidecar = bool(hip_config.get('head_gather_sidecar', True)) and self._use_sidecars
+        self._head_gather = None
+        self._head_gather_w = False
+        self._head_plan_cache = None
         self._la_gather = None
         self._fuse_prediction_dense = bool(hip_config.get('fuse_prediction_dense', True))
         self._fused_q_loss_with_aux = bool(hip_config.get('fused_q_loss_with_aux', True))
@@ -1158,12 +1162,19 @@
                                     a2_out=self._pi_a, logp2_out=self._pi_logp)
             if not native.policy_sample_q_forward_ok(fused):
                 fused = None
+        riders = None
+        if fused is not None and self._head_gather is not None:
+            ring = self._head_ring_job(fused, job_tq, self._head_gather, nx_states, nx_actions)
+            if ring is not None:
+                fused, riders = ring, [self._head_gather['sidecar_w' if self._head_gather_w else 'sidecar']]
+                self._head_gather = None
+        self._join_head_gather()
         if fused is not None:
             self.noise.normal_(self._eps_y)
             if policy_sample:
                 self.noise.normal_(self._eps_pi)
                 self._pi_sampled = True
-            native.policy_sample_q_forward(fused, [job_tq], sidecars=self._take_la_gather())
+            native.policy_sample_q_forward(fused, [job_tq], sidecars=riders if riders is not None else self._take_la_gather())
             _, c_y, ret = self._get_y(*window, eps_buf=self._eps_y, subset_prefix='y', y_out=self._y_buf,
                                       ls=ls[0].view(B, T, 2 * A), sample=(a_y, logp_y), stored_pi=c_pi,
                                       q_table=q_tab.view(E, B, T), launch=False)
@@ -1175,12 +1186,26 @@
         if not fold:
             self._finish_rep_q(None, None)
 
+    def _head_ring_job(self, fused, job_tq, head, nx_states, nx_actions):
+        rb, b = self.replay_buffer, self.burn_in_step
+        obs, act = rb._batch[f'obs_{self.obs_names[0]}'], rb._batch['action']
+        if b != rb.prev_n or nx_states.shape[1] + b != rb.window:
+            return None
+        for view, whole in ((nx_states, obs), (nx_actions, act)):
+            at = whole[:, b:]
+            if view.data_ptr() != at.data_ptr() or view.stride() != at.stride() or view.shape != at.shape:
+                return None
+        job = native.pi_q_ring_rows(fused, rb._ids, head['index_ring'], rb.capacity, rb.prev_n, rb.window, b, head['x0'],
+                                    head['action'], x_j0=b, x_action_offset=self.d_action_summed_size)
+        return job if native.policy_sample_q_forward_ok(job, [job_tq]) else None
+
     def _train_rep_q(self, n_last_masks, n_padding_masks, nx_obses_list, nx_states, nx_actions, n_rewards,
                      n_dones, n_mu_probs, priority_is, aux=None, policy_sample=False, state_base=None):
         if (self._stock_c_only() and aux is None and self.clip_epsilon > 0 and not nx_states.requires_grad
                 and self.optimizer_rep is None):
             return self._train_rep_q_stock(n_last_masks, n_padding_masks, nx_obses_list, nx_states, nx_actions,
                                            n_rewards, n_dones, n_mu_probs, priority_is, policy_sample)
+        self._join_head_gather()
         dsum = self.d_action_summed_size
         obs_list = [o[:, 0] for o in nx_obses_list]
         state, action = nx_states[:, 0], nx_actions[:, 0]
@@ -1658,6 +1683,7 @@
         self._counter_advanced = False
         w = self._step_sample()
         self._step_rep_and_q(w)
+        self._join_head_gather()
         self._step_policy(w)
         post = _AfterPolicy()
         if not self.use_replay_buffer:
@@ -1680,6 +1706,28 @@
         if self._la_gather is not None:
             self._la_gather = None
             self.replay_buffer.gather_next_now()
+
+    def _head_gather_plan(self, rb, build=False):
+        cached = self._head_plan_cache
+        if cached is not None and cached[0] is rb._gather_keys:
+            return cached[1]
+        if not build:
+            return None
+        plan = None
+        weights = self._defer_is_weights
+        if (self._head_gather_sidecar and self._lookahead == 0 and self.burn_in_step == 0 and self._dist is None
+                and self._stock_c_only()
+                and type(self.model_rep) is ModelSimpleRep and self.optimizer_rep is None
+                and self.clip_epsilon > 0 and self.siamese is None and not self.use_prediction
+                and not self._wide_critics and len(self.obs_names) == 1 and not (weights and rb.batch_size > 256)):
+            plan = rb.head_gather(f'obs_{self.obs_names[0]}', build=True, weights=weights)
+        self._head_plan_cache = (rb._gather_keys, plan)
+        return plan
+
+    def _join_head_gather(self) -> None:
+        if self._head_gather is not None:
+            self._head_gather = None
+            self.replay_buffer.gather_now(weights=self._head_gather_w)
 
     def _take_la_gather(self):
         sc, self._la_gather = self._la_gather, None
@@ -1713,13 +1761,18 @@
             else:
                 rb.sample_next_into_static(sampled=sampled)
         else:
+            head = self._head_gather_plan(rb)
             sampled = self._use_sidecars and self.noise.begin_step_with_sample(
                 self._opt_steps, rb, self._eps_all, self._subsets_all, self.ensemble_q_num, polyak=polyak, zero=zero,
-                defer_weights=self._defer_is_weights)
+                defer_weights=self._defer_is_weights, defer_small=head is not None)
             if not sampled:
                 self.noise.begin_step(self._opt_steps, rb._u if rb.uniform_source is self.noise else None, self._eps_all,
                                       self._subsets_all, self.ensemble_q_num, polyak=polyak, zero=zero)
-            rb.sample_into_static(sampled=sampled)
+            self._head_gather_w = sampled == 3
+            self._head_gather = head if head is not None and ('sidecar_w' if sampled == 3 else 'sidecar') in head else None
+            if not sampled:
+                self._head_gather = None
+            rb.sample_into_static(sampled=sampled, gather=self._head_gather is None)
         derived = rb.derived if rb.derived is not None and rb.sharded is None else None
         return self._window_views(rb._batch, rb._ids, rb._w.unsqueeze(-1) if self.use_priority else None, derived,
                                   rb.joint_pre_action)
@@ -2055,6 +2108,8 @@
         elif rb._gather_keys is None:
             rb._build_batch()
             self._drop_graphs()
+        if rb is not None:
+            self._head_gather_plan(rb, build=True)
 
         if self._lookahead:
             if not rb.lookahead:
diff --git a/advanced-soft-actor-critic_amd/csrc/asac_gather.h b/advanced-soft-actor-critic_amd/csrc/asac_gather.h
--- a/advanced-soft-actor-critic_amd/csrc/asac_gather.h
+++ b/advanced-soft-actor-critic_amd/csrc/asac_gather.h
@@ -39,11 +39,15 @@
 
 __device__ __forceinline__ int64_t load_id(const int64_t* ids, int s) { return ids[s]; }
 
+__device__ __forceinline__ bool index_run(int idx_j, int idx_c, int j, int prev_n) {
+    return j == prev_n || (idx_j - idx_c) == (j - prev_n);
+}
+
 __device__ __forceinline__ bool row_valid(const GatherArgs& a, int64_t id, int j) {
     if (j == a.prev_n) return true;
     const int idx_j = a.index_ring[ring_slot(id + (j - a.prev_n), a.capacity)];
     const int idx_c = a.index_ring[ring_slot(id, a.capacity)];
-    return (idx_j - idx_c) == (j - a.prev_n);
+    return index_run(idx_j, idx_c, j, a.prev_n);
 }
 
 template <typename Unit>
@@ -68,6 +72,15 @@
     if (k.pad_mode == ASAC_PAD_ROW) return k.pad_row[w];
     if (k.pad_mode == ASAC_PAD_WORD) return (uint8_t)(k.pad_word >> (8 * (w & 3)));
     return (uint8_t)(k.pad_word & 0xff);
+}
+
+__device__ __forceinline__ uint32_t ring_word(const GatherArgs& a, const GatherKeyDev& k, int64_t id, int j, int w) {
+    const int slot = ring_slot(id + (j - a.prev_n), a.capacity);
+    const uint32_t data = reinterpret_cast<const uint32_t*>(k.src + (int64_t)slot * k.row_bytes)[w];
+    const int idx_j = a.index_ring[slot];
+    const int idx_c = a.index_ring[ring_slot(id, a.capacity)];
+    const uint32_t pad = pad_value<uint32_t>(k, w);
+    return (k.pad_mode == ASAC_PAD_KEEP || index_run(idx_j, idx_c, j, a.prev_n)) ? data : pad;
 }
 
 __device__ __forceinline__ int derived_row(int derive, int j, int L) {
diff --git a/advanced-soft-actor-critic_amd/csrc/asac_sidecar.h b/advanced-soft-actor-critic_amd/csrc/asac_sidecar.h
--- a/advanced-soft-actor-critic_amd/csrc/asac_sidecar.h
+++ b/advanced-soft-actor-critic_amd/csrc/asac_sidecar.h
@@ -171,6 +171,35 @@
     if (lane == 0) __hip_atomic_store(&a.winner[slot], -1, __ATOMIC_RELAXED, __HIP_MEMORY_SCOPE_AGENT);
 }
 
+struct WeightsJob {
+    const float* p;
+    const float* tree;
+    double* beta_state;
+    double beta_increment;
+    float* w_out;
+    float* min_p_out;
+    int32_t batch, parts;
+};
+
+__device__ __forceinline__ void weights_job(const WeightsJob& j) {
+    float bm = j.min_p_out[2];
+    for (int k = 1; k < j.parts; ++k) bm = fminf(bm, j.min_p_out[2 + k]);
+    const float root = j.tree[0];
+    const double b = fmin(1.0, *j.beta_state + j.beta_increment);
+    const float min_ratio = bm / root;
+    __syncthreads();
+    for (int i = threadIdx.x; i < j.batch; i += kGatherBlock) j.w_out[i] = is_weight(j.p[i], root, min_ratio, b);
+    if (threadIdx.x == 0) {
+        *j.beta_state = b;
+        j.min_p_out[0] = bm;
+    }
+}
+
+struct GatherPlanDev {
+    GatherLaunch<ASAC_MAX_GATHER_KEYS> g;
+    WeightsJob w;
+};
+
 struct SidecarDev {
     int32_t kind, first_block;
     AlphaAdamArgs alpha;
@@ -196,7 +225,7 @@
 constexpr int kSidecarRowsPerWg = 256;
 inline int scatter_write_rows_per_wg(int row_bytes) { return row_bytes <= 32 ? kSidecarRowsPerWg : 4; }
 
-inline int sidecars_prepare(const asac_sidecar_t* jobs, int n, SidecarsDev& out) {
+inline int sidecars_prepare(const asac_sidecar_t* jobs, int n, SidecarsDev& out, bool with_weights = false) {
     out.n = 0;
     out.blocks = 0;
     if (n < 0 || n > ASAC_MAX_SIDECARS || (n > 0 && !jobs)) return 1;
@@ -219,8 +248,8 @@
             const int total = h.batch * h.count;
             const int per = h.kind == ASAC_SIDECAR_SCATTER_ELECT ? kSidecarRowsPerWg : scatter_write_rows_per_wg(h.row_bytes);
             out.blocks += (total + per - 1) / per;
-        } else if (h.kind == ASAC_SIDECAR_WINDOW_GATHER) {
-            if (!h.gather_plan || h.gather_blocks <= 0) return 1;
+        } else if (h.kind == ASAC_SIDECAR_WINDOW_GATHER || h.kind == ASAC_SIDECAR_WINDOW_GATHER_W) {
+            if (!h.gather_plan || h.gather_blocks <= 0 || (h.kind == ASAC_SIDECAR_WINDOW_GATHER_W && !with_weights)) return 1;
             d.gather = h.gather_plan;
             out.blocks += h.gather_blocks;
         } else {
@@ -231,7 +260,7 @@
     return 0;
 }
 
-template <int NSC, bool GATHER = false>
+template <int NSC, bool GATHER = false, bool WEIGHTS = false>
 __device__ __forceinline__ void sidecar_run(const SidecarsT<NSC>& sc, int block, float* lds256) {
     int k = 0;
 #pragma unroll
@@ -245,6 +274,12 @@
         if (threadIdx.x < kGatherBlock)
             gather_block<ASAC_MAX_GATHER_KEYS, 1>(*static_cast<const GatherLaunch<ASAC_MAX_GATHER_KEYS>*>(job.gather),
                                                   (unsigned)local);
+    } else if (WEIGHTS && job.kind == ASAC_SIDECAR_WINDOW_GATHER_W) {
+        if (threadIdx.x < kGatherBlock) {
+            const GatherPlanDev* plan = static_cast<const GatherPlanDev*>(job.gather);
+            if (local == 0) weights_job(plan->w);
+            else gather_block<ASAC_MAX_GATHER_KEYS, 1>(plan->g, (unsigned)(local - 1));
+        }
     } else if (threadIdx.x < 256) {
         if (job.kind == ASAC_SIDECAR_SCATTER_ELECT) {
             scatter_elect_row(job.scatter, local * kSidecarRowsPerWg + (int)threadIdx.x);
diff --git a/advanced-soft-actor-critic_amd/csrc/gather.hip b/advanced-soft-actor-critic_amd/csrc/gather.hip
--- a/advanced-soft-actor-critic_amd/csrc/gather.hip
+++ b/advanced-soft-actor-critic_amd/csrc/gather.hip
@@ -7,30 +7,6 @@
 template <int NK, int kUnroll>
 __global__ __launch_bounds__(kGatherBlock) void k_window_gather_pad(const GatherLaunch<NK> m) {
     gather_block<NK, kUnroll>(m, blockIdx.x);
-}
-
-struct WeightsJob {
-    const float* p;
-    const float* tree;
-    double* beta_state;
-    double beta_increment;
-    float* w_out;
-    float* min_p_out;
-    int32_t batch, parts;
-};
-
-__device__ __forceinline__ void weights_job(const WeightsJob& j) {
-    float bm = j.min_p_out[2];
-    for (int k = 1; k < j.parts; ++k) bm = fminf(bm, j.min_p_out[2 + k]);
-    const float root = j.tree[0];
-    const double b = fmin(1.0, *j.beta_state + j.beta_increment);
-    const float min_ratio = bm / root;
-    __syncthreads();
-    for (int i = threadIdx.x; i < j.batch; i += kGatherBlock) j.w_out[i] = is_weight(j.p[i], root, min_ratio, b);
-    if (threadIdx.x == 0) {
-        *j.beta_state = b;
-        j.min_p_out[0] = bm;
-    }
 }
 
 template <int NK, int kUnroll>
@@ -198,7 +174,7 @@
                              int post_n, int capacity, const int32_t* index_ring, const float* p, const float* tree,
                              double* beta_state, double beta_increment, float* is_weights_out, float* min_p_out,
                              void* stream) {
-    if (!p || !tree || !beta_state || !is_weights_out || !min_p_out || batch <= 256 || batch > 1024)
+    if (!p || !tree || !beta_state || !is_weights_out || !min_p_out || batch <= 0 || batch > 1024)
         return bad_arg("asac_window_gather_pad_w");
     GatherLaunch<ASAC_MAX_GATHER_KEYS> m{};
     uint64_t blocks = 0;
@@ -230,7 +206,7 @@
     return finish_launch("asac_window_gather_pad_w");
 }
 
-int64_t asac_window_gather_plan_bytes(void) { return (int64_t)sizeof(GatherLaunch<ASAC_MAX_GATHER_KEYS>); }
+int64_t asac_window_gather_plan_bytes(void) { return (int64_t)sizeof(GatherPlanDev); }
 
 int asac_window_gather_plan(const asac_gather_key_t* keys_host, int n_keys, const int64_t* ids, int batch, int prev_n,
                             int post_n, int capacity, const int32_t* index_ring, void* plan_dev, int* blocks_out) {
@@ -246,6 +222,27 @@
         return (int)e;
     }
     *blocks_out = (int)blocks;
+    return 0;
+}
+
+int asac_window_gather_plan_w(const asac_gather_key_t* keys_host, int n_keys, const int64_t* ids, int batch, int prev_n,
+                              int post_n, int capacity, const int32_t* index_ring, const float* p, const float* tree,
+                              double* beta_state, double beta_increment, float* is_weights_out, float* min_p_out,
+                              void* plan_dev, int* blocks_out) {
+    if (!plan_dev || !blocks_out || !p || !tree || !beta_state || !is_weights_out || !min_p_out || batch <= 0 || batch > 1024)
+        return bad_arg("asac_window_gather_plan_w");
+    GatherPlanDev plan{};
+    uint64_t blocks = 0;
+    int unroll = 0;
+    if (const int rc = gather_fill(keys_host, n_keys, ids, batch, prev_n, post_n, capacity, index_ring, 1, plan.g, &blocks, &unroll))
+        return rc;
+    plan.w = WeightsJob{p, tree, beta_state, beta_increment, is_weights_out, min_p_out, batch, (batch + 255) / 256};
+    const hipError_t e = hipMemcpy(plan_dev, &plan, sizeof(plan), hipMemcpyHostToDevice);
+    if (e != hipSuccess) {
+        set_error(e, "asac_window_gather_plan_w");
+        return (int)e;
+    }
+    *blocks_out = (int)blocks + 1;
     return 0;
 }
 
diff --git a/advanced-soft-actor-critic_amd/csrc/mlp.hip b/advanced-soft-actor-critic_amd/csrc/mlp.hip
--- a/advanced-soft-actor-critic_amd/csrc/mlp.hip
+++ b/advanced-soft-actor-critic_amd/csrc/mlp.hip
@@ -420,6 +420,77 @@
     }
 }
 
+struct RingKeyArg {
+    const uint8_t *src, *pad_row;
+    int32_t row_bytes;
+    uint32_t pad_word;
+};
+struct RingArg {
+    const int64_t* ids;
+    const int32_t* index_ring;
+    int32_t capacity, prev_n, L, j0, x_j0, x_a_off;
+    int32_t pad_mode0, pad_mode1;
+    RingKeyArg x0, action;
+};
+static_assert(sizeof(RingArg) == 96, "RingArg");
+
+struct RingStage {
+    GatherArgs g;
+    GatherKeyDev k0, k1;
+    int32_t j0, T, c1;
+};
+
+__device__ __forceinline__ GatherKeyDev ring_key(const ASAC_KARG RingKeyArg& k, int pad_mode) {
+    GatherKeyDev d{};
+    d.src = k.src, d.pad_row = k.pad_row, d.row_bytes = k.row_bytes, d.pad_word = k.pad_word, d.pad_mode = pad_mode;
+    return d;
+}
+
+template <bool X1>
+__device__ __forceinline__ RingStage ring_stage(const ASAC_KARG RingArg& r, int j0, int T, int c1) {
+    RingStage R{};
+    R.g.ids = r.ids, R.g.index_ring = r.index_ring, R.g.prev_n = r.prev_n, R.g.L = r.L, R.g.capacity = r.capacity;
+    R.k0 = ring_key(r.x0, r.pad_mode0);
+    if (X1) R.k1 = ring_key(r.action, r.pad_mode1);
+    R.j0 = j0, R.T = T, R.c1 = c1;
+    return R;
+}
+
+template <int THREADS, int SLOTS>
+__device__ __forceinline__ void ring_tile_ids(const StageScalars& q, const RingStage& R, int64_t row0, int64_t (&id)[SLOTS]) {
+#pragma unroll
+    for (int u = 0; u < SLOTS; ++u) {
+        const int r = (threadIdx.x + u * THREADS) >> 6;
+        const uint32_t row = (uint32_t)row0 + (uint32_t)r;
+        const bool live = (int64_t)row0 + r < q.N;
+        id[u] = load_id(R.g.ids, live ? (int)(row / (uint32_t)R.T) : 0);
+    }
+}
+
+template <int THREADS, int SLOTS, bool X1>
+__device__ __forceinline__ void ring_tile_rows(const StageScalars& q, const RingStage& R, int64_t row0,
+                                               const int64_t (&id)[SLOTS], float (&v)[SLOTS]) {
+    const int in0 = q.in0, in1 = X1 ? q.in1 : 0;
+#pragma unroll
+    for (int u = 0; u < SLOTS; ++u) {
+        const int i = threadIdx.x + u * THREADS;
+        const int r = i >> 6, c = i & 63;
+        const uint32_t row = (uint32_t)row0 + (uint32_t)r;
+        const bool live = (int64_t)row0 + r < q.N;
+        const uint32_t smp = row / (uint32_t)R.T;
+        const int j = live ? R.j0 + (int)(row - smp * (uint32_t)R.T) : R.g.prev_n;
+        const bool first = c < in0;
+        uint32_t x = ring_word(R.g, R.k0, id[u], j, first ? c : 0);
+        x = (live && first) ? x : 0u;
+        if (X1) {
+            const bool second = !first && c < in0 + in1;
+            const uint32_t x1 = ring_word(R.g, R.k1, id[u], j, second ? R.c1 + (c - in0) : R.c1);
+            x = (live && second) ? x1 : x;
+        }
+        v[u] = __builtin_bit_cast(float, x);
+    }
+}
+
 template <int THREADS, int NB>
 __device__ __forceinline__ void net_fetch_fixed(const StageScalars& q, StagedNet<THREADS>& r) {
     constexpr int U = 4096 / THREADS;
@@ -504,9 +575,10 @@
            (wide ? (size_t)TM * kP * sizeof(float) : 0);
 }
 
-template <int TM, bool WINDOW, bool WIDE = false, int NB = 0, bool EPI = false>
+template <int TM, bool WINDOW, bool WIDE = false, int NB = 0, bool EPI = false, bool RING = false>
 __device__ __forceinline__ void mlp_fwd_tiles(const MlpFwdArgs& a, const int e, const int tile0, const int tile_stride,
-                                              MlpLds<TM>& L, const SampleEpi* epi = nullptr) {
+                                              MlpLds<TM>& L, const SampleEpi* epi = nullptr, const RingStage* ring = nullptr) {
+    static_assert(!RING || (NB > 0 && !WINDOW && !EPI), "ring-addressed rows: the fixed-shape path");
     constexpr int THREADS = threads_of<TM>();
     constexpr int RT = TM / 16;
     constexpr bool fixed = NB > 0;
@@ -525,9 +597,12 @@
     if constexpr (fixed) {
         q = stage_scalars<NB>(a, e);
         float in_lo[4];
-        fetch_input_tile_fixed<THREADS, WINDOW>(q, e, (int64_t)tile0 * TM, in_lo);
+        int64_t id_lo[4];
+        if constexpr (RING) ring_tile_ids<THREADS, 4>(q, *ring, (int64_t)tile0 * TM, id_lo);
+        else fetch_input_tile_fixed<THREADS, WINDOW>(q, e, (int64_t)tile0 * TM, in_lo);
         StagedNet<THREADS> regs;
         net_fetch_fixed<THREADS, NB>(q, regs);
+        if constexpr (RING) ring_tile_rows<THREADS, 4, true>(q, *ring, (int64_t)tile0 * TM, id_lo, in_lo);
         put_input_tile<THREADS>(in_lo, L.xs[0]);
         net_put_fixed<THREADS, NB>(regs, L);
     } else {
@@ -554,7 +629,11 @@
         const bool more = tile + tile_stride < n_tiles;
         float nxt[4], nxt_hi[4];
         if (more) {
-            if constexpr (fixed) fetch_input_tile_fixed<THREADS, WINDOW>(q, e, (int64_t)(tile + tile_stride) * TM, nxt);
+            if constexpr (RING) {
+                int64_t id_nxt[4];
+                ring_tile_ids<THREADS, 4>(q, *ring, (int64_t)(tile + tile_stride) * TM, id_nxt);
+                ring_tile_rows<THREADS, 4, true>(q, *ring, (int64_t)(tile + tile_stride) * TM, id_nxt, nxt);
+            } else if constexpr (fixed) fetch_input_tile_fixed<THREADS, WINDOW>(q, e, (int64_t)(tile + tile_stride) * TM, nxt);
             else fetch_input_tile<THREADS, WINDOW>(a, e, (int64_t)(tile + tile_stride) * TM, nxt);
         }
         if (more && wide) fetch_input_tile<THREADS, WINDOW>(a, e, (int64_t)(tile + tile_stride) * TM, nxt_hi, kMaxW);
@@ -1569,8 +1648,9 @@
     return location ? tanhf(raw / 5.f) * 5.f : expf(fminf(fmaxf(raw, -20.f), 0.5f));
 }
 
-template <bool WINDOW>
-__device__ __forceinline__ void pi_q_tiles(const ASAC_KARG PiQLaunch& a, PiQLds& L) {
+template <bool WINDOW, bool RING = false>
+__device__ __forceinline__ void pi_q_tiles(const ASAC_KARG PiQLaunch& a, PiQLds& L, const ASAC_KARG RingArg* ring = nullptr) {
+    static_assert(!(RING && WINDOW), "ring-addressed rows have their own (sample, row) addressing");
     constexpr int THREADS = kPiQThreads;
     constexpr int SLOTS = 1024 / kPiQThreads;
     const bool comp = (threadIdx.x >> 6) < 4;
@@ -1587,10 +1667,18 @@
     const StageScalars sp = stage_scalars_stock(a.pi, 0);
     const StageScalars sq = stage_scalars_stock_like(a.q, e, sp);
     float in_lo[SLOTS];
-    fetch_input_tile_fixed<THREADS, WINDOW, SLOTS>(sp, 0, (int64_t)group * 16, in_lo);
+    int64_t id_lo[SLOTS];
+    RingStage R{};
+    if constexpr (RING) {
+        R = ring_stage<false>(*ring, ring->j0, a.T, 0);
+        ring_tile_ids<THREADS, SLOTS>(sp, R, (int64_t)group * 16, id_lo);
+    } else {
+        fetch_input_tile_fixed<THREADS, WINDOW, SLOTS>(sp, 0, (int64_t)group * 16, in_lo);
+    }
     StagedNet<THREADS> rp, rq;
     net_fetch_fixed<THREADS, 3>(sp, rp);
     net_fetch_fixed<THREADS, 3>(sq, rq);
+    if constexpr (RING) ring_tile_rows<THREADS, SLOTS, false>(sp, R, (int64_t)group * 16, id_lo, in_lo);
     put_input_tile<THREADS, SLOTS>(in_lo, L.xs[0]);
     net_put_fixed<THREADS, 3>(rp, L);
     PiQCritic C{L.qw, L.qhead, L.qbias, L.qhead_bias};
@@ -1600,10 +1688,28 @@
     for (int tile = group; tile < n_tiles; tile += a.tile_groups) {
         const int row0 = tile * 16;
         if (tile != group) {
-            fetch_input_tile_fixed<THREADS, WINDOW, SLOTS>(sp, 0, row0, in_lo);
+            if constexpr (RING) {
+                ring_tile_ids<THREADS, SLOTS>(sp, R, row0, id_lo);
+                ring_tile_rows<THREADS, SLOTS, false>(sp, R, row0, id_lo, in_lo);
+            } else {
+                fetch_input_tile_fixed<THREADS, WINDOW, SLOTS>(sp, 0, row0, in_lo);
+            }
             __syncthreads();
             put_input_tile<THREADS, SLOTS>(in_lo, L.xs[0]);
             __syncthreads();
+        }
+        float av_ring[2] = {0.f, 0.f};
+        if constexpr (RING) {
+            const RingStage Ra = ring_stage<true>(*ring, ring->j0, a.sp.T, a.sp.action ? a.sp.a_off : 0);
+#pragma unroll
+            for (int h = 0; h < 2; ++h) {
+                const int it = min(lane + 64 * h, 16 * A - 1);
+                const int lrow = it / A, d = it - lrow * A;
+                const int r = min(row0 + lrow, N - 1);
+                const int sb = (int)((unsigned)r / (unsigned)Ra.T), st = r - sb * Ra.T;
+                av_ring[h] = __builtin_bit_cast(float, ring_word(Ra.g, Ra.k1, load_id(Ra.g.ids, sb), Ra.j0 + st,
+                                                                 a.sp.action ? Ra.c1 + d : 0));
+            }
         }
         int cur = 0;
 #pragma unroll
@@ -1656,7 +1762,9 @@
                     if (job == 1) {
                         const int spT = a.sp.T;
                         const int sb = (int)((unsigned)r / (unsigned)spT), st = r - sb * spT;
-                        const float av = a.sp.action[sb * a.sp.a_sb + st * a.sp.a_st + a.sp.a_off + d];
+                        float av;
+                        if constexpr (RING) av = it < 64 ? av_ring[0] : av_ring[1];
+                        else av = a.sp.action[sb * a.sp.a_sb + st * a.sp.a_st + a.sp.a_off + d];
                         const float x = atanhf(fminf(fmaxf(av, -0.999f), 0.999f));
                         s0[lrow * 8 + d] = squash_jac(x);
                         s1[lrow * 8 + d] = expf(normal_log_prob(x, l, sc));
@@ -1800,6 +1908,47 @@
         mlp_fwd_tiles<16, false, false, 3>(job, local % E, local / E, m.x_tile_stride[k], L);
 }
 
+struct PiQLaunchRing {
+    PiQLaunch m;
+    RingArg ring;
+};
+static_assert(offsetof(PiQLaunchRing, m) == 0 && sizeof(PiQLaunchRing) <= 768, "kernel arguments of k_pi_sample_q_ring");
+
+template <int NSC>
+__global__ __launch_bounds__(kPiQThreads) void k_pi_sample_q_ring(const PiQLaunchRing m_by_value, const SidecarsT<NSC> sc) {
+    extern __shared__ __attribute__((aligned(16))) unsigned char smem_raw[];
+    const ASAC_KARG PiQLaunchRing& mr = *static_cast<const ASAC_KARG PiQLaunchRing*>(kernarg_base());
+    const ASAC_KARG PiQLaunch& m = mr.m;
+    const int blk = (int)blockIdx.x;
+    const int fused_blocks = m.blocks;
+    if (blk >= fused_blocks && threadIdx.x >= 256) return;
+    if (blk < fused_blocks) {
+        pi_q_tiles<false, true>(m, *reinterpret_cast<PiQLds*>(smem_raw), &mr.ring);
+        return;
+    }
+    const int xb = blk - fused_blocks;
+    if (xb >= m.x_blocks) {
+        sidecar_run<NSC, true, true>(sc, xb - m.x_blocks, reinterpret_cast<float*>(smem_raw));
+        return;
+    }
+    int k = 0;
+#pragma unroll
+    for (int q = 1; q < ASAC_MLP_MAX_JOBS; ++q)
+        if (q < m.x_n && xb >= m.x_first_block[q]) k = q;
+    const int local = xb - m.x_first_block[k];
+    const int E = m.x_E[k];
+    MlpLds<16>& L = *reinterpret_cast<MlpLds<16>*>(smem_raw);
+    const MlpFwdArgs job = expand_stock(m.x_job[k]);
+    if (k == 0 && mr.ring.x_j0 >= 0) {
+        const RingStage R = ring_stage<true>(mr.ring, mr.ring.x_j0, 1, mr.ring.x_a_off);
+        mlp_fwd_tiles<16, false, false, 3, false, true>(job, local % E, local / E, m.x_tile_stride[k], L, nullptr, &R);
+    } else if (job.x0_T > 0) {
+        mlp_fwd_tiles<16, true, false, 3>(job, local % E, local / E, m.x_tile_stride[k], L);
+    } else {
+        mlp_fwd_tiles<16, false, false, 3>(job, local % E, local / E, m.x_tile_stride[k], L);
+    }
+}
+
 __global__ __launch_bounds__(256) void k_mlp_reduce_partials(const float* __restrict__ partial, int tiles, int E,
                                                              int64_t member_stride, int64_t used,
                                                              float* __restrict__ grad, int accumulate,
@@ -2309,6 +2458,27 @@
     return r;
 }
 
+static bool ring_key_ok(const asac_ring_key_t& k, int first_col, int cols) {
+    if (!k.src || k.row_bytes <= 0 || k.row_bytes % 4 != 0 || k.row_bytes > (1 << 20) ||
+        reinterpret_cast<uintptr_t>(k.src) % 4 != 0)
+        return false;
+    if (first_col < 0 || cols <= 0 || (int64_t)(first_col + cols) * 4 > k.row_bytes) return false;
+    if (k.pad_mode == ASAC_PAD_ROW) return k.pad_row && reinterpret_cast<uintptr_t>(k.pad_row) % 4 == 0;
+    return k.pad_mode == ASAC_PAD_KEEP || k.pad_mode == ASAC_PAD_WORD;
+}
+
+static bool ring_rows_ok(const asac_pi_q_job_t& j) {
+    const asac_ring_rows_t& r = j.ring;
+    const asac_squash_job_t& s = j.sample;
+    if (!r.ids || !r.index_ring || r.capacity <= 0 || r.prev_n < 0 || r.L <= r.prev_n) return false;
+    if (s.T <= 0 || j.pi.N % s.T != 0 || r.j0 < 0 || r.j0 + s.T > r.L) return false;
+    if (j.pi.x0_window_T != 0 && j.pi.x0_window_T != s.T) return false;
+    if (!ring_key_ok(r.x0, 0, j.pi.desc->in0)) return false;
+    if ((s.action || r.x_j0 >= 0) && !ring_key_ok(r.action, 0, 1)) return false;
+    if (s.action && !ring_key_ok(r.action, s.action_offset, s.A)) return false;
+    return r.x_j0 < r.L;
+}
+
 static bool pi_q_job_ok(const asac_pi_q_job_t& j) {
     const asac_mlp_job_t &p = j.pi, &q = j.q;
     if (!p.desc || !q.desc || !desc_ok(*p.desc) || !desc_ok(*q.desc) || p.N <= 0 || q.N != p.N || p.E != 1 || q.E < 1) return false;
@@ -2327,17 +2497,41 @@
     if (s.action && (!fits32((p.N / s.T + 1) * s.action_stride_b) || !fits32((p.N / s.T + 1) * s.prob_stride_b) ||
                      !fits32(s.T * s.action_stride_t) || !fits32(s.T * s.prob_stride_t)))
         return false;
-    return job_fits32(pi_rows(p));
+    return job_fits32(pi_rows(p)) && (!j.ring.ids || ring_rows_ok(j));
+}
+
+static bool pi_q_extras_ok(const asac_pi_q_job_t& job, const asac_mlp_job_t* extra_jobs, int n_extra) {
+    if (n_extra < 0 || n_extra > ASAC_MLP_MAX_JOBS || (n_extra > 0 && !extra_jobs)) return false;
+    for (int k = 0; k < n_extra; ++k) {
+        const asac_mlp_job_t& j = extra_jobs[k];
+        if (!job_ok(j, true) || !stock3(*j.desc, j.params, j.member_stride) || j.x0_window_T < 0 || !job_fits32(j) ||
+            !fits32(j.member_stride) || !fits32(j.x0_member_stride) || !fits32(j.x1_member_stride))
+            return false;
+    }
+    const asac_ring_rows_t& r = job.ring;
+    if (r.ids && r.x_j0 >= 0) {
+        if (n_extra < 1) return false;
+        const asac_mlp_job_t& x = extra_jobs[0];
+        if (x.x0_window_T != 0 || x.x0_member_stride != 0 || x.x1_member_stride != 0 || x.N != job.pi.N / job.sample.T ||
+            x.desc->in1 <= 0 || !ring_key_ok(r.x0, 0, x.desc->in0) || !ring_key_ok(r.action, r.x_action_offset, x.desc->in1))
+            return false;
+    }
+    return true;
 }
 
 int asac_policy_sample_q_forward_ok(const asac_pi_q_job_t* job) { return job && pi_q_job_ok(*job) ? 1 : 0; }
+
+int asac_policy_sample_q_forward_jobs_ok(const asac_pi_q_job_t* job, const asac_mlp_job_t* extra_jobs, int n_extra) {
+    return job && pi_q_job_ok(*job) && pi_q_extras_ok(*job, extra_jobs, n_extra) ? 1 : 0;
+}
 
 int asac_policy_sample_q_forward(const asac_pi_q_job_t* job, const asac_mlp_job_t* extra_jobs, int n_extra,
                                  const asac_sidecar_t* sidecars_host, int n_sidecars, void* stream) {
-    if (!job || !pi_q_job_ok(*job) || n_extra < 0 || n_extra > ASAC_MLP_MAX_JOBS || (n_extra > 0 && !extra_jobs))
-        return bad_arg("asac_policy_sample_q_forward");
+    if (!job || !pi_q_job_ok(*job)) return bad_arg("asac_policy_sample_q_forward");
+    if (!pi_q_extras_ok(*job, extra_jobs, n_extra)) return bad_arg("asac_policy_sample_q_forward: extra job");
     SidecarsDev sc{};
-    if (sidecars_prepare(sidecars_host, n_sidecars, sc)) return bad_arg("asac_policy_sample_q_forward: sidecar");
+    if (sidecars_prepare(sidecars_host, n_sidecars, sc, job->ring.ids != nullptr))
+        return bad_arg("asac_policy_sample_q_forward: sidecar");
     PiQLaunch m{};
     const asac_mlp_job_t p = pi_rows(job->pi);
     asac_mlp_job_t q = pi_rows(job->q);
@@ -2364,9 +2558,6 @@
     int blocks = 0;
     for (int k = 0; k < n_extra; ++k) {
         const asac_mlp_job_t& j = extra_jobs[k];
-        if (!job_ok(j, true) || !stock3(*j.desc, j.params, j.member_stride) || j.x0_window_T < 0 || !job_fits32(j) ||
-            !fits32(j.member_stride) || !fits32(j.x0_member_stride) || !fits32(j.x1_member_stride))
-            return bad_arg("asac_policy_sample_q_forward: extra job");
         m.x_job[k] = stock_job_arg(j);
         m.x_E[k] = j.E;
         m.x_first_block[k] = blocks;
@@ -2374,6 +2565,38 @@
         blocks += m.x_tile_stride[k] * j.E;
     }
     m.x_blocks = blocks;
+    if (job->ring.ids) {
+        const asac_ring_rows_t& r = job->ring;
+        PiQLaunchRing mr{};
+        mr.m = m;
+        if (sj.action) mr.m.sp.action = static_cast<const float*>(r.action.src);
+        const asac_ring_key_t& ak = (sj.action || r.x_j0 >= 0) ? r.action : r.x0;
+        mr.ring = RingArg{r.ids, r.index_ring, r.capacity, r.prev_n, r.L, r.j0, r.x_j0, r.x_action_offset,
+                          r.x0.pad_mode, ak.pad_mode,
+                          RingKeyArg{static_cast<const uint8_t*>(r.x0.src), static_cast<const uint8_t*>(r.x0.pad_row),
+                                     r.x0.row_bytes, r.x0.pad_word},
+                          RingKeyArg{static_cast<const uint8_t*>(ak.src), static_cast<const uint8_t*>(ak.pad_row), ak.row_bytes,
+                                     ak.pad_word}};
+        static bool ring_attr = false, ring_attr1 = false;
+        if (int rc = set_lds_limit(reinterpret_cast<const void*>(k_pi_sample_q_ring<ASAC_MAX_SIDECARS>), sizeof(PiQLds),
+                                   ring_attr, "asac_policy_sample_q_forward: hipFuncSetAttribute"))
+            return rc;
+        if (int rc = set_lds_limit(reinterpret_cast<const void*>(k_pi_sample_q_ring<1>), sizeof(PiQLds), ring_attr1,
+                                   "asac_policy_sample_q_forward: hipFuncSetAttribute"))
+            return rc;
+        const SidecarsDev no_sc{};
+        for (int rep = 0; rep < g_launch_repeat; ++rep) {
+            const bool last = rep == g_launch_repeat - 1;
+            const dim3 grid((unsigned)(m.blocks + blocks + (last ? sc.blocks : 0)));
+            if (sc.n <= 1)
+                hipLaunchKernelGGL(k_pi_sample_q_ring<1>, grid, dim3(kPiQThreads), sizeof(PiQLds), as_stream(stream), mr,
+                                   sidecars_first<1>(last ? sc : no_sc));
+            else
+                hipLaunchKernelGGL(k_pi_sample_q_ring<ASAC_MAX_SIDECARS>, grid, dim3(kPiQThreads), sizeof(PiQLds),
+                                   as_stream(stream), mr, last ? sc : no_sc);
+        }
+        return finish_launch("asac_policy_sample_q_forward");
+    }
     static bool attr_done = false;
     static bool attr_done1 = false;
     if (int rc = set_lds_limit(reinterpret_cast<const void*>(k_pi_sample_q<ASAC_MAX_SIDECARS>), sizeof(PiQLds), attr_done,
diff --git a/advanced-soft-actor-critic_amd/csrc/sumtree.hip b/advanced-soft-actor-critic_amd/csrc/sumtree.hip
--- a/advanced-soft-actor-critic_amd/csrc/sumtree.hip
+++ b/advanced-soft-actor-critic_amd/csrc/sumtree.hip
@@ -204,7 +204,7 @@
     float m = wave_min(pmin);
     if ((threadIdx.x & (kWave - 1)) == 0) red[threadIdx.x / kWave] = m;
     __syncthreads();
-    SampleSync* const sync = MULTI ? reinterpret_cast<SampleSync*>(min_p_out + 2) : nullptr;
+    SampleSync* const sync = (MULTI || PARTIAL) ? reinterpret_cast<SampleSync*>(min_p_out + 2) : nullptr;
     const unsigned n_wg = MULTI ? (unsigned)((batch + kSampleBlock - 1) / kSampleBlock) : 1u;
     if (PARTIAL) {
         if (threadIdx.x == 0) {
@@ -298,7 +298,7 @@
     if ((int)blockIdx.x < n_s) {
         const SampleDraw dr{pa.seed, pa.step, pa.n_normal};
         if (n_s == 1)
-            sumtree_sample_body<true, true, true, false, 1, false, 13>(
+            sumtree_sample_body<true, true, true, false, 1, false, 13, PARTIAL>(
                 tree, capacity, levels, batch, pa.u, slot_ids, beta_state, beta_increment, leaf_out, p_out, ids_out, w_out,
                 min_p_out, dr);
         else
@@ -670,7 +670,6 @@
                                       float* normal_out, int64_t n_normal, int32_t* subsets_out, int n_subsets, int E_sample,
                                       int E, const float* tree, int capacity, int batch, const int64_t* slot_ids,
                                       int32_t* leaf_out, float* p_out, int64_t* ids_out, float* min_p_out, void* stream) {
-    if (batch <= kSampleBlock) return bad_arg("asac_step_prologue_sample_partial: one workgroup samples such a batch whole");
     static double unused_beta = 0.0;
     return prologue_sample_launch(target, source, n_polyak, tau, zero_out, n_zero, seed, step_counter, uniform_out, normal_out,
                                   n_normal, subsets_out, n_subsets, E_sample, E, tree, capacity, batch, slot_ids, &unused_beta,
diff --git a/advanced-soft-actor-critic_amd/native.py b/advanced-soft-actor-critic_amd/native.py
--- a/advanced-soft-actor-critic_amd/native.py
+++ b/advanced-soft-actor-critic_amd/native.py
@@ -7,7 +7,7 @@
 import os as _os
 
 LIB_PATH = Path(_os.environ.get('ASAC_HIP_LIB', PKG_DIR / 'lib' / 'libasac_hip.so'))
-ABI_VERSION = 88
+ABI_VERSION = 89
 
 MAX_GATHER_KEYS = 16
 PAD_KEEP, PAD_WORD, PAD_BYTE, PAD_ROW, PAD_EMIT_MASK = 0, 1, 2, 3, 4
@@ -130,6 +130,7 @@
 
 
 SIDECAR_ALPHA_ADAM, SIDECAR_SCATTER_ELECT, SIDECAR_SCATTER_WRITE, SIDECAR_WINDOW_GATHER, MAX_SIDECARS = 1, 2, 3, 4, 4
+SIDECAR_WINDOW_GATHER_W = 5
 
 
 class SquashJob(C.Structure):
@@ -144,9 +145,20 @@
 SQUASH_MAX_JOBS = 4
 
 
+class RingKey(C.Structure):
+    _fields_ = [('src', C.c_void_p), ('pad_row', C.c_void_p), ('row_bytes', C.c_int32), ('pad_mode', C.c_int32),
+                ('pad_word', C.c_uint32), ('reserved_', C.c_int32)]
+
+
+class RingRows(C.Structure):
+    _fields_ = [('ids', C.c_void_p), ('index_ring', C.c_void_p), ('capacity', C.c_int32), ('prev_n', C.c_int32),
+                ('L', C.c_int32), ('j0', C.c_int32), ('x_j0', C.c_int32), ('x_action_offset', C.c_int32),
+                ('x0', RingKey), ('action', RingKey)]
+
+
 class PiQJob(C.Structure):
     _fields_ = [('pi', MlpJob), ('sample', SquashJob), ('eps2', C.c_void_p), ('t2', C.c_int32), ('reserved_', C.c_int32),
-                ('a2_out', C.c_void_p), ('logp2_out', C.c_void_p), ('q', MlpJob)]
+                ('a2_out', C.c_void_p), ('logp2_out', C.c_void_p), ('q', MlpJob), ('ring', RingRows)]
 
 
 class SampleEpilogue(C.Structure):
@@ -203,6 +215,9 @@
     'asac_window_gather_plan_bytes': (C.c_int64, []),
     'asac_window_gather_plan': (C.c_int, [C.POINTER(GatherKey), C.c_int, C.c_void_p, C.c_int, C.c_int, C.c_int, C.c_int,
                                           C.c_void_p, C.c_void_p, C.POINTER(C.c_int)]),
+    'asac_window_gather_plan_w': (C.c_int, [C.POINTER(GatherKey), C.c_int, C.c_void_p, C.c_int, C.c_int, C.c_int, C.c_int,
+                                            C.c_void_p, C.c_void_p, C.c_void_p, C.c_void_p, C.c_double, C.c_void_p,
+                                            C.c_void_p, C.c_void_p, C.POINTER(C.c_int)]),
     'asac_sumtree_descend': (C.c_int, [C.c_void_p, C.c_int, C.c_int, C.c_void_p, C.c_void_p, C.c_void_p, C.c_void_p,
                                        C.c_void_p, C.c_void_p]),
     'asac_gather_rows': (C.c_int, [C.POINTER(GatherKey), C.c_int, C.c_void_p, C.c_int, C.c_int, C.c_void_p]),
@@ -261,6 +276,7 @@
                                                   C.c_void_p, C.c_void_p, C.c_int, C.c_void_p]),
     'asac_struct_size': (C.c_int64, [C.c_char_p]),
     'asac_policy_sample_q_forward_ok': (C.c_int, [C.POINTER(PiQJob)]),
+    'asac_policy_sample_q_forward_jobs_ok': (C.c_int, [C.POINTER(PiQJob), C.POINTER(MlpJob), C.c_int]),
     'asac_policy_sample_q_forward': (C.c_int, [C.POINTER(PiQJob), C.POINTER(MlpJob), C.c_int, C.POINTER(Sidecar), C.c_int,
                                                C.c_void_p]),
     'asac_policy_step_fused_ok': (C.c_int, [C.POINTER(MlpDesc), C.c_void_p, C.c_int64, C.POINTER(MlpDesc), C.c_void_p,
@@ -687,6 +703,19 @@
     return sc
 
 
+def sidecar_window_gather_w(keys, ids, batch, prev_n, post_n, capacity, index_ring, p, tree, beta_state, beta_increment,
+                            is_weights_out, min_p_out) -> Sidecar:
+    import torch
+    plan = torch.empty(int(load().asac_window_gather_plan_bytes()), dtype=torch.uint8, device=ids.device)
+    blocks = C.c_int(0)
+    _check(load().asac_window_gather_plan_w(keys, len(keys), _p(ids), batch, prev_n, post_n, capacity, _p(index_ring), _p(p),
+                                            _p(tree), _p(beta_state), float(beta_increment), _p(is_weights_out),
+                                            _p(min_p_out), _p(plan), C.byref(blocks)), 'asac_window_gather_plan_w')
+    sc = Sidecar(kind=SIDECAR_WINDOW_GATHER_W, gather_plan=_p(plan), gather_blocks=blocks.value)
+    sc._keep = (plan, keys, ids, index_ring, p, tree, beta_state, is_weights_out, min_p_out)
+    return sc
+
+
 @_profiled
 def gather_rows(keys, ids, capacity):
     _check(load().asac_gather_rows(keys, len(keys), _p(ids), ids.numel(), capacity, _stream()), 'asac_gather_rows')
@@ -1061,8 +1090,39 @@
     return j
 
 
-def policy_sample_q_forward_ok(job: PiQJob) -> bool:
-    return bool(load().asac_policy_sample_q_forward_ok(C.byref(job)))
+def ring_key(spec) -> RingKey | None:
+    src = spec.get('src')
+    if (src is None or src.dtype != torch.float32 or spec.get('convert', CVT_NONE) != CVT_NONE or spec.get('derive', 0)
+            or spec['pad_mode'] not in (PAD_KEEP, PAD_WORD, PAD_ROW) or int(spec['row_bytes']) % 4):
+        return None
+    k = RingKey()
+    k.src, k.row_bytes, k.pad_mode = src.data_ptr(), int(spec['row_bytes']), int(spec['pad_mode'])
+    k.pad_word = int(spec.get('pad_word', 0)) & 0xffffffff
+    if spec['pad_mode'] == PAD_ROW:
+        k.pad_row = spec['pad_row'].data_ptr()
+    return k
+
+
+def pi_q_ring_rows(job: PiQJob, ids, index_ring, capacity, prev_n, L, j0, x0_key: RingKey, action_key: RingKey | None = None,
+                   x_j0=-1, x_action_offset=0) -> PiQJob:
+    assert ids.dtype == torch.int64 and index_ring.dtype == torch.int32
+    out = PiQJob()
+    C.memmove(C.byref(out), C.byref(job), C.sizeof(PiQJob))
+    r = out.ring
+    r.ids, r.index_ring = ids.data_ptr(), index_ring.data_ptr()
+    r.capacity, r.prev_n, r.L, r.j0, r.x_j0, r.x_action_offset = capacity, prev_n, L, j0, x_j0, x_action_offset
+    r.x0 = x0_key
+    if action_key is not None:
+        r.action = action_key
+    return out
+
+
+def policy_sample_q_forward_ok(job: PiQJob, extra_jobs=None) -> bool:
+    if extra_jobs is None:
+        return bool(load().asac_policy_sample_q_forward_ok(C.byref(job)))
+    extra_jobs = list(extra_jobs)
+    arr = (MlpJob * len(extra_jobs))(*extra_jobs) if extra_jobs else None
+    return bool(load().asac_policy_sample_q_forward_jobs_ok(C.byref(job), arr, len(extra_jobs)))
 
 
 @_profiled
@@ -1772,7 +1832,7 @@
 def step_prologue_sample_partial(polyak, zero, seed, step_counter, uniform_out, normal_out, subsets_out, ensemble, tree,
                                  capacity, batch, slot_ids, leaf_out, p_out, ids_out, min_p_out):
     target_flat, source_flat, tau = polyak if polyak is not None else (None, None, 0.0)
-    assert uniform_out.numel() == batch and uniform_out.dtype == torch.float64 and 256 < batch <= PROLOGUE_SAMPLE_MAX_BATCH
+    assert uniform_out.numel() == batch and uniform_out.dtype == torch.float64 and 0 < batch <= PROLOGUE_SAMPLE_MAX_BATCH
     assert min_p_out.numel() >= 528 and min_p_out.dtype == torch.float32
     assert zero is None or (zero.is_contiguous() and zero.dtype == torch.float32)
     nn_ = 0 if normal_out is None else normal_out.numel()
diff --git a/include/asac_hip.h b/include/asac_hip.h
--- a/include/asac_hip.h
+++ b/include/asac_hip.h
@@ -7,7 +7,7 @@
 extern "C" {
 #endif
 
-#define ASAC_ABI_VERSION 88
+#define ASAC_ABI_VERSION 89
 #define ASAC_MAX_GATHER_KEYS 16
 #define ASAC_MAX_ENSEMBLE 16
 #define ASAC_MAX_ACTION 64
@@ -86,6 +86,11 @@
 int asac_window_gather_plan(const asac_gather_key_t* keys_host, int n_keys, const int64_t* ids, int batch, int prev_n,
                             int post_n, int capacity, const int32_t* index_ring, void* plan_dev, int* blocks_out);
 
+int asac_window_gather_plan_w(const asac_gather_key_t* keys_host, int n_keys, const int64_t* ids, int batch, int prev_n,
+                              int post_n, int capacity, const int32_t* index_ring, const float* p, const float* tree,
+                              double* beta_state, double beta_increment, float* is_weights_out, float* min_p_out,
+                              void* plan_dev, int* blocks_out);
+
 int asac_gather_rows(const asac_gather_key_t* keys_host, int n_keys, const int64_t* ids, int n_rows, int capacity,
                      void* stream);
 
@@ -132,6 +137,7 @@
 #define ASAC_SIDECAR_SCATTER_ELECT 2
 #define ASAC_SIDECAR_SCATTER_WRITE 3
 #define ASAC_SIDECAR_WINDOW_GATHER 4
+#define ASAC_SIDECAR_WINDOW_GATHER_W 5
 #define ASAC_MAX_SIDECARS 4
 typedef struct {
     int32_t kind;
@@ -285,6 +291,23 @@
                                    const asac_sidecar_t* sidecars_host, int n_sidecars, void* stream);
 
 typedef struct {
+    const void* src;
+    const void* pad_row;
+    int32_t row_bytes;
+    int32_t pad_mode;
+    uint32_t pad_word;
+    int32_t reserved_;
+} asac_ring_key_t;
+typedef struct {
+    const int64_t* ids;
+    const int32_t* index_ring;
+    int32_t capacity, prev_n, L;
+    int32_t j0;
+    int32_t x_j0;
+    int32_t x_action_offset;
+    asac_ring_key_t x0, action;
+} asac_ring_rows_t;
+typedef struct {
     asac_mlp_job_t pi;
     asac_squash_job_t sample;
     const float* eps2;
@@ -293,8 +316,10 @@
     float* a2_out;
     float* logp2_out;
     asac_mlp_job_t q;
+    asac_ring_rows_t ring;
 } asac_pi_q_job_t;
 int asac_policy_sample_q_forward_ok(const asac_pi_q_job_t* job);
+int asac_policy_sample_q_forward_jobs_ok(const asac_pi_q_job_t* job, const asac_mlp_job_t* extra_jobs, int n_extra);
 int asac_policy_sample_q_forward(const asac_pi_q_job_t* job, const asac_mlp_job_t* extra_jobs, int n_extra,
                                  const asac_sidecar_t* sidecars_host, int n_sidecars, void* stream);
 
```
